# cita-cloud/consensus_overlord

Hardware: AMD Instinct MI355X
Metric: BLS12-381 vote verifications/sec (batch 4096) at 1/2/4/8 MI355X vs host blst (higher is better)
Workload: dtype u32; 1 GPU; config3: 4096 distinct-message precommit votes per GPU, RLC batch verify; batch_per_gpu=4096, global_batch=4096, parallelism=single GPU

## Files before the change

### consensus_overlord_amd/csrc/bls/fp.hpp

```cpp
#pragma once
#include <stdint.h>

#if defined(__HIPCC__)
#include <hip/hip_runtime.h>
#define OVH_HD __host__ __device__ __forceinline__
#define OVH_HDNI __host__ __device__ inline __attribute__((noinline))
#else
#define OVH_HD inline
#define OVH_HDNI inline
#endif

#include "consts.hpp"
#if defined(__HIP_DEVICE_COMPILE__)
#include "fp_mul_gfx950.hpp"
#include "fp_mul28.hpp"
#include "fp_mul28_gfx950.hpp"
#endif

namespace ovh {

#if defined(OVH_COUNT_MULS) && !defined(__HIP_DEVICE_COMPILE__)
extern unsigned long long g_fp_mul_count;
#define OVH_COUNT_MUL() (++::ovh::g_fp_mul_count)
#else
// ... 39 lines not shown
  for (int i = 0; i < 12; ++i) r.v[i] = 0;
}

OVH_HD void fp_one(Fp& r) { fp_load(r, ONE_M); }

OVH_HD bool fp_is_zero(const Fp& a) {
  uint32_t acc = 0;
#pragma unroll
  for (int i = 0; i < 12; ++i) acc |= a.v[i];
  return acc == 0;
}

OVH_HD bool fp_eq(const Fp& a, const Fp& b) {
  uint32_t acc = 0;
#pragma unroll
  for (int i = 0; i < 12; ++i) acc |= a.v[i] ^ b.v[i];
  return acc == 0;
}

OVH_HD bool fp_is_one(const Fp& a) { return fp_eq(a, fp_const(ONE_M)); }

OVH_HD void fp_select(Fp& r, bool cond, const Fp& a, const Fp& b) {
#pragma unroll
  for (int i = 0; i < 12; ++i) r.v[i] = cond ? b.v[i] : a.v[i];
}

OVH_HD void fp_add(Fp& r, const Fp& a, const Fp& b) {
  uint32_t s[12], d[12], c = 0, br = 0;
#pragma unroll
  for (int i = 0; i < 12; ++i) s[i] = addc32(a.v[i], b.v[i], c, &c);
#pragma unroll
  for (int i = 0; i < 12; ++i) d[i] = subc32(s[i], P_LIMBS[i], br, &br);
#pragma unroll
  for (int i = 0; i < 12; ++i) r.v[i] = br ? s[i] : d[i];
}

OVH_HD void fp_sub(Fp& r, const Fp& a, const Fp& b) {
  uint32_t d[12], br = 0, c = 0;
#pragma unroll
  for (int i = 0; i < 12; ++i) d[i] = subc32(a.v[i], b.v[i], br, &br);
  const uint32_t mask = 0u - br;
#pragma unroll
  for (int i = 0; i < 12; ++i) r.v[i] = addc32(d[i], P_LIMBS[i] & mask, c, &c);
}

OVH_HD void fp_dbl(Fp& r, const Fp& a) { fp_add(r, a, a); }

OVH_HD void fp_neg(Fp& r, const Fp& a) {
  Fp z;
  fp_zero(z);
  fp_sub(r, z, a);
}

OVH_HD void fp_mul(Fp& r, const Fp& a, const Fp& b) {
#if defined(__HIP_DEVICE_COMPILE__) && defined(OVH_FPMUL32)
  fp_mul_gfx950(r.v, a.v, b.v);
#elif defined(__HIP_DEVICE_COMPILE__)
  fp_mul28_gfx950(r.v, a.v, b.v);
#else
  OVH_COUNT_MUL();
  uint32_t t[12];
#pragma unroll
  for (int j = 0; j < 12; ++j) t[j] = 0;
#pragma unroll
  for (int i = 0; i < 12; ++i) {
    const uint32_t bi = b.v[i];
    uint64_t c = (uint64_t)a.v[0] * bi + t[0];
    t[0] = (uint32_t)c;
    const uint32_t m = t[0] * P_INV32;
    uint64_t c2 = (uint64_t)m * P_LIMBS[0] + t[0];
#pragma unroll
    for (int j = 1; j < 12; ++j) {
      c = (uint64_t)a.v[j] * bi + t[j] + (c >> 32);
      c2 = (uint64_t)m * P_LIMBS[j] + (uint32_t)c + (c2 >> 32);
      t[j - 1] = (uint32_t)c2;
    }
    t[11] = (uint32_t)(c >> 32) + (uint32_t)(c2 >> 32);
  }
  uint32_t d[12], br = 0;
#pragma unroll
  for (int i = 0; i < 12; ++i) d[i] = subc32(t[i], P_LIMBS[i], br, &br);
#pragma unroll
  for (int i = 0; i < 12; ++i) r.v[i] = br ? t[i] : d[i];
#endif
}

OVH_HD void fp_sqr(Fp& r, const Fp& a) { fp_mul(r, a, a); }

OVH_HD void fp_mul_small(Fp& r, const Fp& a, uint32_t k) {
  Fp acc, base = a;
  fp_zero(acc);
  while (k) {
    if (k & 1) fp_add(acc, acc, base);
    fp_add(base, base, base);
    k >>= 1;
  }
  r = acc;
}

OVH_HDNI void fp_pow(Fp& r, const Fp& a, const uint32_t* e) {
  Fp acc;
  fp_one(acc);
  bool started = false;
#pragma unroll 1
  for (int i = 11; i >= 0; --i) {
    const uint32_t w = e[i];
#pragma unroll 1
    for (int b = 31; b >= 0; --b) {
      if (started) fp_sqr(acc, acc);
      if ((w >> b) & 1) {
        if (started) {
          fp_mul(acc, acc, a);
        } else {
          acc = a;
          started = true;
        }
      }
    }
  }
  r = acc;
}

namespace inv {
constexpr int NL = 13;
constexpr int32_t M30 = 0x3FFFFFFF;
constexpr int32_t PL[NL] = {0x3fffaaab, 0x27fbffff, 0x153ffffb, 0x2affffac, 0x30f6241e, 0x034a83da, 0x112bf673,
                            0x12e13ce1, 0x2cd76477, 0x1ed90d2e, 0x29a4b1ba, 0x3a8e5ff9, 0x001a0111};
constexpr uint32_t PINV30 = 0x30003;
struct Trans {
  int32_t u, v, q, r;
};

OVH_HD int ctz32(uint32_t x) { return __builtin_ctz(x); }

OVH_HD uint32_t neg_inv32(uint32_t f) {
  uint32_t x = f;
  x *= 2u - f * x;
  x *= 2u - f * x;
  x *= 2u - f * x;
  x *= 2u - f * x;
  return 0u - x;
}

OVH_HD int32_t divsteps30(int32_t eta, uint32_t f, uint32_t g, Trans& t) {
  uint32_t u = 1, v = 0, q = 0, r = 1, finv = neg_inv32(f);
  int i = 30;
#pragma unroll 1
  for (;;) {
    const int z = ctz32(g | (0xFFFFFFFFu << i));
    g >>= z;
    u <<= z;
    v <<= z;
    eta -= z;
    i -= z;
    if (i == 0) break;
    if (eta < 0) {
      eta = -eta;
      uint32_t x = f;
      f = g;
      g = 0u - x;
      x = u;
      u = q;
      q = 0u - x;
      x = v;
      v = r;
      r = 0u - x;
// ... 208 lines not shown
```

### consensus_overlord_amd/csrc/bls/fp_mul28.hpp

```cpp
#pragma once
#include <stdint.h>

#include "consts.hpp"

namespace ovh {

constexpr uint32_t M28 = 0x0FFFFFFFu;
constexpr uint32_t P28[14] = {0xfffaaabu, 0xfefffffu, 0x3ffffb9u, 0xfffeb15u, 0x6241eabu, 0xa0f6b0fu, 0xf6730d2u,
                              0xf38512bu, 0x4774b84u, 0x4bacd76u, 0xba7b643u, 0xe69a4b1u, 0x1ea397fu, 0x001a011u};
constexpr uint32_t PINV28 = 0xffcfffdu;

template <int SH>
__device__ __forceinline__ void split28(uint32_t* x, const uint32_t* a) {
#if defined(OVH_UBENCH_NOSPLIT)
#pragma unroll
  for (int k = 0; k < 14; ++k) x[k] = a[k % 12];
  return;
#endif
#pragma unroll
  for (int k = 0; k < 14; ++k) {
    const int lo = 28 * k - SH;
    uint32_t v;
    if (lo < 0) {
      v = a[0] << (-lo);
    } else {
      const int w = lo >> 5, s = lo & 31;
      v = a[w] >> s;
      if (s > 4 && w + 1 < 12) v |= a[w + 1] << (32 - s);
    }
    x[k] = v & M28;
  }
}

__device__ __forceinline__ void join28_reduce(uint32_t* r, const uint32_t* t) {
#if defined(OVH_UBENCH_NOSPLIT)
#pragma unroll
  for (int j = 0; j < 12; ++j) r[j] = t[j];
  return;
#endif
  uint32_t u[12];
#pragma unroll
  for (int j = 0; j < 12; ++j) {
    const int k = (32 * j) / 28, s = (32 * j) % 28;
    uint32_t v = (t[k] >> s) | (t[k + 1] << (28 - s));
    if (s > 24 && k + 2 < 14) v |= t[k + 2] << (56 - s);
    u[j] = v;
  }
  uint32_t d[12], br = 0;
#pragma unroll
  for (int j = 0; j < 12; ++j) d[j] = __builtin_subc(u[j], P_LIMBS[j], br, &br);
#pragma unroll
  for (int j = 0; j < 12; ++j) r[j] = br ? u[j] : d[j];
}

__device__ __forceinline__ void fp_mul28(uint32_t* r, const uint32_t* a, const uint32_t* b) {
  uint32_t x[14], y[14], m[14], t[14];
  split28<8>(x, a);
  split28<0>(y, b);
  uint64_t acc = 0;
#pragma unroll
  for (int k = 0; k < 27; ++k) {
#pragma unroll
    for (int i = 0; i < 14; ++i)
      if (k - i >= 0 && k - i < 14) acc += (uint64_t)x[i] * y[k - i];
#pragma unroll
    for (int i = 0; i < 14; ++i)
      if (i < k && k - i < 14) acc += (uint64_t)m[i] * P28[k - i];
    if (k < 14) {
      m[k] = ((uint32_t)acc * PINV28) & M28;
      acc += (uint64_t)m[k] * P28[0];
    } else {
      t[k - 14] = (uint32_t)acc & M28;
    }
    acc >>= 28;
  }
  t[13] = (uint32_t)acc;
  join28_reduce(r, t);
}

}
```

### consensus_overlord_amd/csrc/bls/fp_mul28_gfx950.hpp

```cpp
#pragma once
#include <stdint.h>
#include "fp_mul28.hpp"
namespace ovh {
__device__ __forceinline__ void fp_mul28_gfx950_1acc(uint32_t* __restrict__ r, const uint32_t* __restrict__ a,
                                             const uint32_t* __restrict__ b) {
  uint32_t x[14], y[14], m[14], t[14];
  split28<8>(x, a);
  split28<0>(y, b);
  asm volatile(
      "v_mad_u64_u32 v[252:253], vcc, %[x0], %[y0], 0\n\tv_mul_lo_u32 %[m0], v252, %[pinv]\n\tv_and_b32_e32 %[m0], %[mask], %[m0]\n\tv_mad_u64_u32 v[252:253], vcc, %[m0], %[p0], v[252:253]\n\tv_lshrrev_b64 v[252:253], 28, v[252:253]\n\tv_mad_u64_u32 v[252:253], vcc, %[x0], %[y1], v[252:253]\n\tv_mad_u64_u32 v[252:253], vcc, %[x1], %[y0], v[252:253]\n\tv_mad_u64_u32 v[252:253], vcc, %[m0], %[p1], v[252:253]\n\t"
      "v_mul_lo_u32 %[m1], v252, %[pinv]\n\tv_and_b32_e32 %[m1], %[mask], %[m1]\n\tv_mad_u64_u32 v[252:253], vcc, %[m1], %[p0], v[252:253]\n\tv_lshrrev_b64 v[252:253], 28, v[252:253]\n\tv_mad_u64_u32 v[252:253], vcc, %[x0], %[y2], v[252:253]\n\tv_mad_u64_u32 v[252:253], vcc, %[x1], %[y1], v[252:253]\n\tv_mad_u64_u32 v[252:253], vcc, %[x2], %[y0], v[252:253]\n\tv_mad_u64_u32 v[252:253], vcc, %[m0], %[p2], v[252:253]\n\t"
      "v_mad_u64_u32 v[252:253], vcc, %[m1], %[p1], v[252:253]\n\tv_mul_lo_u32 %[m2], v252, %[pinv]\n\tv_and_b32_e32 %[m2], %[mask], %[m2]\n\tv_mad_u64_u32 v[252:253], vcc, %[m2], %[p0], v[252:253]\n\tv_lshrrev_b64 v[252:253], 28, v[252:253]\n\tv_mad_u64_u32 v[252:253], vcc, %[x0], %[y3], v[252:253]\n\tv_mad_u64_u32 v[252:253], vcc, %[x1], %[y2], v[252:253]\n\tv_mad_u64_u32 v[252:253], vcc, %[x2], %[y1], v[252:253]\n\t"
      "v_mad_u64_u32 v[252:253], vcc, %[x3], %[y0], v[252:253]\n\tv_mad_u64_u32 v[252:253], vcc, %[m0], %[p3], v[252:253]\n\tv_mad_u64_u32 v[252:253], vcc, %[m1], %[p2], v[252:253]\n\tv_mad_u64_u32 v[252:253], vcc, %[m2], %[p1], v[252:253]\n\tv_mul_lo_u32 %[m3], v252, %[pinv]\n\tv_and_b32_e32 %[m3], %[mask], %[m3]\n\tv_mad_u64_u32 v[252:253], vcc, %[m3], %[p0], v[252:253]\n\tv_lshrrev_b64 v[252:253], 28, v[252:253]\n\t"
      "v_mad_u64_u32 v[252:253], vcc, %[x0], %[y4], v[252:253]\n\tv_mad_u64_u32 v[252:253], vcc, %[x1], %[y3], v[252:253]\n\tv_mad_u64_u32 v[252:253], vcc, %[x2], %[y2], v[252:253]\n\tv_mad_u64_u32 v[252:253], vcc, %[x3], %[y1], v[252:253]\n\tv_mad_u64_u32 v[252:253], vcc, %[x4], %[y0], v[252:253]\n\tv_mad_u64_u32 v[252:253], vcc, %[m0], %[p4], v[252:253]\n\tv_mad_u64_u32 v[252:253], vcc, %[m1], %[p3], v[252:253]\n\tv_mad_u64_u32 v[252:253], vcc, %[m2], %[p2], v[252:253]\n\t"
      "v_mad_u64_u32 v[252:253], vcc, %[m3], %[p1], v[252:253]\n\tv_mul_lo_u32 %[m4], v252, %[pinv]\n\tv_and_b32_e32 %[m4], %[mask], %[m4]\n\tv_mad_u64_u32 v[252:253], vcc, %[m4], %[p0], v[252:253]\n\tv_lshrrev_b64 v[252:253], 28, v[252:253]\n\tv_mad_u64_u32 v[252:253], vcc, %[x0], %[y5], v[252:253]\n\tv_mad_u64_u32 v[252:253], vcc, %[x1], %[y4], v[252:253]\n\tv_mad_u64_u32 v[252:253], vcc, %[x2], %[y3], v[252:253]\n\t"
      "v_mad_u64_u32 v[252:253], vcc, %[x3], %[y2], v[252:253]\n\tv_mad_u64_u32 v[252:253], vcc, %[x4], %[y1], v[252:253]\n\tv_mad_u64_u32 v[252:253], vcc, %[x5], %[y0], v[252:253]\n\tv_mad_u64_u32 v[252:253], vcc, %[m0], %[p5], v[252:253]\n\tv_mad_u64_u32 v[252:253], vcc, %[m1], %[p4], v[252:253]\n\tv_mad_u64_u32 v[252:253], vcc, %[m2], %[p3], v[252:253]\n\tv_mad_u64_u32 v[252:253], vcc, %[m3], %[p2], v[252:253]\n\tv_mad_u64_u32 v[252:253], vcc, %[m4], %[p1], v[252:253]\n\t"
      "v_mul_lo_u32 %[m5], v252, %[pinv]\n\tv_and_b32_e32 %[m5], %[mask], %[m5]\n\tv_mad_u64_u32 v[252:253], vcc, %[m5], %[p0], v[252:253]\n\tv_lshrrev_b64 v[252:253], 28, v[252:253]\n\tv_mad_u64_u32 v[252:253], vcc, %[x0], %[y6], v[252:253]\n\tv_mad_u64_u32 v[252:253], vcc, %[x1], %[y5], v[252:253]\n\tv_mad_u64_u32 v[252:253], vcc, %[x2], %[y4], v[252:253]\n\tv_mad_u64_u32 v[252:253], vcc, %[x3], %[y3], v[252:253]\n\t"
      "v_mad_u64_u32 v[252:253], vcc, %[x4], %[y2], v[252:253]\n\tv_mad_u64_u32 v[252:253], vcc, %[x5], %[y1], v[252:253]\n\tv_mad_u64_u32 v[252:253], vcc, %[x6], %[y0], v[252:253]\n\tv_mad_u64_u32 v[252:253], vcc, %[m0], %[p6], v[252:253]\n\tv_mad_u64_u32 v[252:253], vcc, %[m1], %[p5], v[252:253]\n\tv_mad_u64_u32 v[252:253], vcc, %[m2], %[p4], v[252:253]\n\tv_mad_u64_u32 v[252:253], vcc, %[m3], %[p3], v[252:253]\n\tv_mad_u64_u32 v[252:253], vcc, %[m4], %[p2], v[252:253]\n\t"
      "v_mad_u64_u32 v[252:253], vcc, %[m5], %[p1], v[252:253]\n\tv_mul_lo_u32 %[m6], v252, %[pinv]\n\tv_and_b32_e32 %[m6], %[mask], %[m6]\n\tv_mad_u64_u32 v[252:253], vcc, %[m6], %[p0], v[252:253]\n\tv_lshrrev_b64 v[252:253], 28, v[252:253]\n\tv_mad_u64_u32 v[252:253], vcc, %[x0], %[y7], v[252:253]\n\tv_mad_u64_u32 v[252:253], vcc, %[x1], %[y6], v[252:253]\n\tv_mad_u64_u32 v[252:253], vcc, %[x2], %[y5], v[252:253]\n\t"
      "v_mad_u64_u32 v[252:253], vcc, %[x3], %[y4], v[252:253]\n\tv_mad_u64_u32 v[252:253], vcc, %[x4], %[y3], v[252:253]\n\tv_mad_u64_u32 v[252:253], vcc, %[x5], %[y2], v[252:253]\n\tv_mad_u64_u32 v[252:253], vcc, %[x6], %[y1], v[252:253]\n\tv_mad_u64_u32 v[252:253], vcc, %[x7], %[y0], v[252:253]\n\tv_mad_u64_u32 v[252:253], vcc, %[m0], %[p7], v[252:253]\n\tv_mad_u64_u32 v[252:253], vcc, %[m1], %[p6], v[252:253]\n\tv_mad_u64_u32 v[252:253], vcc, %[m2], %[p5], v[252:253]\n\t"
      "v_mad_u64_u32 v[252:253], vcc, %[m3], %[p4], v[252:253]\n\tv_mad_u64_u32 v[252:253], vcc, %[m4], %[p3], v[252:253]\n\tv_mad_u64_u32 v[252:253], vcc, %[m5], %[p2], v[252:253]\n\tv_mad_u64_u32 v[252:253], vcc, %[m6], %[p1], v[252:253]\n\tv_mul_lo_u32 %[m7], v252, %[pinv]\n\tv_and_b32_e32 %[m7], %[mask], %[m7]\n\tv_mad_u64_u32 v[252:253], vcc, %[m7], %[p0], v[252:253]\n\tv_lshrrev_b64 v[252:253], 28, v[252:253]\n\t"
      "v_mad_u64_u32 v[252:253], vcc, %[x0], %[y8], v[252:253]\n\tv_mad_u64_u32 v[252:253], vcc, %[x1], %[y7], v[252:253]\n\tv_mad_u64_u32 v[252:253], vcc, %[x2], %[y6], v[252:253]\n\tv_mad_u64_u32 v[252:253], vcc, %[x3], %[y5], v[252:253]\n\tv_mad_u64_u32 v[252:253], vcc, %[x4], %[y4], v[252:253]\n\tv_mad_u64_u32 v[252:253], vcc, %[x5], %[y3], v[252:253]\n\tv_mad_u64_u32 v[252:253], vcc, %[x6], %[y2], v[252:253]\n\tv_mad_u64_u32 v[252:253], vcc, %[x7], %[y1], v[252:253]\n\t"
      "v_mad_u64_u32 v[252:253], vcc, %[x8], %[y0], v[252:253]\n\tv_mad_u64_u32 v[252:253], vcc, %[m0], %[p8], v[252:253]\n\tv_mad_u64_u32 v[252:253], vcc, %[m1], %[p7], v[252:253]\n\tv_mad_u64_u32 v[252:253], vcc, %[m2], %[p6], v[252:253]\n\tv_mad_u64_u32 v[252:253], vcc, %[m3], %[p5], v[252:253]\n\tv_mad_u64_u32 v[252:253], vcc, %[m4], %[p4], v[252:253]\n\tv_mad_u64_u32 v[252:253], vcc, %[m5], %[p3], v[252:253]\n\tv_mad_u64_u32 v[252:253], vcc, %[m6], %[p2], v[252:253]\n\t"
      "v_mad_u64_u32 v[252:253], vcc, %[m7], %[p1], v[252:253]\n\tv_mul_lo_u32 %[m8], v252, %[pinv]\n\tv_and_b32_e32 %[m8], %[mask], %[m8]\n\tv_mad_u64_u32 v[252:253], vcc, %[m8], %[p0], v[252:253]\n\tv_lshrrev_b64 v[252:253], 28, v[252:253]\n\tv_mad_u64_u32 v[252:253], vcc, %[x0], %[y9], v[252:253]\n\tv_mad_u64_u32 v[252:253], vcc, %[x1], %[y8], v[252:253]\n\tv_mad_u64_u32 v[252:253], vcc, %[x2], %[y7], v[252:253]\n\t"
// ... 39 lines not shown
      "v_mad_u64_u32 v[252:253], vcc, %[x10], %[y13], v[252:253]\n\tv_mad_u64_u32 v[252:253], vcc, %[x11], %[y12], v[252:253]\n\tv_mad_u64_u32 v[252:253], vcc, %[x12], %[y11], v[252:253]\n\tv_mad_u64_u32 v[252:253], vcc, %[x13], %[y10], v[252:253]\n\tv_mad_u64_u32 v[252:253], vcc, %[m10], %[p13], v[252:253]\n\tv_mad_u64_u32 v[252:253], vcc, %[m11], %[p12], v[252:253]\n\tv_mad_u64_u32 v[252:253], vcc, %[m12], %[p11], v[252:253]\n\tv_mad_u64_u32 v[252:253], vcc, %[m13], %[p10], v[252:253]\n\t"
      "v_and_b32_e32 %[t9], %[mask], v252\n\tv_lshrrev_b64 v[252:253], 28, v[252:253]\n\tv_mad_u64_u32 v[252:253], vcc, %[x11], %[y13], v[252:253]\n\tv_mad_u64_u32 v[252:253], vcc, %[x12], %[y12], v[252:253]\n\tv_mad_u64_u32 v[252:253], vcc, %[x13], %[y11], v[252:253]\n\tv_mad_u64_u32 v[252:253], vcc, %[m11], %[p13], v[252:253]\n\tv_mad_u64_u32 v[252:253], vcc, %[m12], %[p12], v[252:253]\n\tv_mad_u64_u32 v[252:253], vcc, %[m13], %[p11], v[252:253]\n\t"
      "v_and_b32_e32 %[t10], %[mask], v252\n\tv_lshrrev_b64 v[252:253], 28, v[252:253]\n\tv_mad_u64_u32 v[252:253], vcc, %[x12], %[y13], v[252:253]\n\tv_mad_u64_u32 v[252:253], vcc, %[x13], %[y12], v[252:253]\n\tv_mad_u64_u32 v[252:253], vcc, %[m12], %[p13], v[252:253]\n\tv_mad_u64_u32 v[252:253], vcc, %[m13], %[p12], v[252:253]\n\tv_and_b32_e32 %[t11], %[mask], v252\n\tv_lshrrev_b64 v[252:253], 28, v[252:253]\n\t"
      "v_mad_u64_u32 v[252:253], vcc, %[x13], %[y13], v[252:253]\n\tv_mad_u64_u32 v[252:253], vcc, %[m13], %[p13], v[252:253]\n\tv_and_b32_e32 %[t12], %[mask], v252\n\tv_lshrrev_b64 v[252:253], 28, v[252:253]\n\tv_mov_b32 %[t13], v252\n\t"
      : [m0] "=&v"(m[0]), [m1] "=&v"(m[1]), [m2] "=&v"(m[2]), [m3] "=&v"(m[3]), [m4] "=&v"(m[4]), [m5] "=&v"(m[5]), [m6] "=&v"(m[6]), [m7] "=&v"(m[7]), [m8] "=&v"(m[8]), [m9] "=&v"(m[9]), [m10] "=&v"(m[10]), [m11] "=&v"(m[11]), [m12] "=&v"(m[12]), [m13] "=&v"(m[13]), [t0] "=&v"(t[0]), [t1] "=&v"(t[1]), [t2] "=&v"(t[2]), [t3] "=&v"(t[3]), [t4] "=&v"(t[4]), [t5] "=&v"(t[5]), [t6] "=&v"(t[6]), [t7] "=&v"(t[7]), [t8] "=&v"(t[8]), [t9] "=&v"(t[9]), [t10] "=&v"(t[10]), [t11] "=&v"(t[11]), [t12] "=&v"(t[12]), [t13] "=&v"(t[13])
      : [x0] "v"(x[0]), [x1] "v"(x[1]), [x2] "v"(x[2]), [x3] "v"(x[3]), [x4] "v"(x[4]), [x5] "v"(x[5]), [x6] "v"(x[6]), [x7] "v"(x[7]), [x8] "v"(x[8]), [x9] "v"(x[9]), [x10] "v"(x[10]), [x11] "v"(x[11]), [x12] "v"(x[12]), [x13] "v"(x[13]), [y0] "v"(y[0]), [y1] "v"(y[1]), [y2] "v"(y[2]), [y3] "v"(y[3]), [y4] "v"(y[4]), [y5] "v"(y[5]), [y6] "v"(y[6]), [y7] "v"(y[7]), [y8] "v"(y[8]), [y9] "v"(y[9]), [y10] "v"(y[10]), [y11] "v"(y[11]), [y12] "v"(y[12]), [y13] "v"(y[13]), [p0] "s"(P28[0]), [p1] "s"(P28[1]), [p2] "s"(P28[2]), [p3] "s"(P28[3]), [p4] "s"(P28[4]), [p5] "s"(P28[5]), [p6] "s"(P28[6]), [p7] "s"(P28[7]), [p8] "s"(P28[8]), [p9] "s"(P28[9]), [p10] "s"(P28[10]), [p11] "s"(P28[11]), [p12] "s"(P28[12]), [p13] "s"(P28[13]), [pinv] "s"(PINV28), [mask] "v"(M28)
      : "vcc", "v252", "v253");
  (void)m;
  join28_reduce(r, t);
}
__device__ __forceinline__ void fp_mul28_gfx950_2acc(uint32_t* __restrict__ r, const uint32_t* __restrict__ a,
                                             const uint32_t* __restrict__ b) {
  uint32_t x[14], y[14], m[14], t[14];
  split28<8>(x, a);
  split28<0>(y, b);
  asm volatile(
      "v_mad_u64_u32 v[252:253], vcc, %[x0], %[y0], 0\n\tv_mul_lo_u32 %[m0], v252, %[pinv]\n\tv_mad_u64_u32 v[250:251], vcc, %[x0], %[y1], 0\n\tv_and_b32_e32 %[m0], %[mask], %[m0]\n\tv_mad_u64_u32 v[250:251], vcc, %[x1], %[y0], v[250:251]\n\tv_mad_u64_u32 v[252:253], vcc, %[m0], %[p0], v[252:253]\n\tv_lshrrev_b64 v[252:253], 28, v[252:253]\n\tv_mad_u64_u32 v[252:253], vcc, %[m0], %[p1], v[252:253]\n\t"
      "v_lshl_add_u64 v[252:253], v[250:251], 0, v[252:253]\n\tv_mul_lo_u32 %[m1], v252, %[pinv]\n\tv_mad_u64_u32 v[250:251], vcc, %[x0], %[y2], 0\n\tv_and_b32_e32 %[m1], %[mask], %[m1]\n\tv_mad_u64_u32 v[250:251], vcc, %[x1], %[y1], v[250:251]\n\tv_mad_u64_u32 v[252:253], vcc, %[m1], %[p0], v[252:253]\n\tv_mad_u64_u32 v[250:251], vcc, %[x2], %[y0], v[250:251]\n\tv_lshrrev_b64 v[252:253], 28, v[252:253]\n\t"
      "v_mad_u64_u32 v[250:251], vcc, %[m0], %[p2], v[250:251]\n\tv_mad_u64_u32 v[252:253], vcc, %[m1], %[p1], v[252:253]\n\tv_lshl_add_u64 v[252:253], v[250:251], 0, v[252:253]\n\tv_mul_lo_u32 %[m2], v252, %[pinv]\n\tv_mad_u64_u32 v[250:251], vcc, %[x0], %[y3], 0\n\tv_and_b32_e32 %[m2], %[mask], %[m2]\n\tv_mad_u64_u32 v[250:251], vcc, %[x1], %[y2], v[250:251]\n\tv_mad_u64_u32 v[252:253], vcc, %[m2], %[p0], v[252:253]\n\t"
      "v_mad_u64_u32 v[250:251], vcc, %[x2], %[y1], v[250:251]\n\tv_lshrrev_b64 v[252:253], 28, v[252:253]\n\tv_mad_u64_u32 v[250:251], vcc, %[x3], %[y0], v[250:251]\n\tv_mad_u64_u32 v[252:253], vcc, %[m0], %[p3], v[252:253]\n\tv_mad_u64_u32 v[250:251], vcc, %[m1], %[p2], v[250:251]\n\tv_mad_u64_u32 v[252:253], vcc, %[m2], %[p1], v[252:253]\n\tv_lshl_add_u64 v[252:253], v[250:251], 0, v[252:253]\n\tv_mul_lo_u32 %[m3], v252, %[pinv]\n\t"
      "v_mad_u64_u32 v[250:251], vcc, %[x0], %[y4], 0\n\tv_and_b32_e32 %[m3], %[mask], %[m3]\n\tv_mad_u64_u32 v[250:251], vcc, %[x1], %[y3], v[250:251]\n\tv_mad_u64_u32 v[252:253], vcc, %[m3], %[p0], v[252:253]\n\tv_mad_u64_u32 v[250:251], vcc, %[x2], %[y2], v[250:251]\n\tv_lshrrev_b64 v[252:253], 28, v[252:253]\n\tv_mad_u64_u32 v[250:251], vcc, %[x3], %[y1], v[250:251]\n\tv_mad_u64_u32 v[252:253], vcc, %[x4], %[y0], v[252:253]\n\t"
      "v_mad_u64_u32 v[250:251], vcc, %[m0], %[p4], v[250:251]\n\tv_mad_u64_u32 v[252:253], vcc, %[m1], %[p3], v[252:253]\n\tv_mad_u64_u32 v[250:251], vcc, %[m2], %[p2], v[250:251]\n\tv_mad_u64_u32 v[252:253], vcc, %[m3], %[p1], v[252:253]\n\tv_lshl_add_u64 v[252:253], v[250:251], 0, v[252:253]\n\tv_mul_lo_u32 %[m4], v252, %[pinv]\n\tv_mad_u64_u32 v[250:251], vcc, %[x0], %[y5], 0\n\tv_and_b32_e32 %[m4], %[mask], %[m4]\n\t"
      "v_mad_u64_u32 v[250:251], vcc, %[x1], %[y4], v[250:251]\n\tv_mad_u64_u32 v[252:253], vcc, %[m4], %[p0], v[252:253]\n\tv_mad_u64_u32 v[250:251], vcc, %[x2], %[y3], v[250:251]\n\tv_lshrrev_b64 v[252:253], 28, v[252:253]\n\tv_mad_u64_u32 v[250:251], vcc, %[x3], %[y2], v[250:251]\n\tv_mad_u64_u32 v[252:253], vcc, %[x4], %[y1], v[252:253]\n\tv_mad_u64_u32 v[250:251], vcc, %[x5], %[y0], v[250:251]\n\tv_mad_u64_u32 v[252:253], vcc, %[m0], %[p5], v[252:253]\n\t"
      "v_mad_u64_u32 v[250:251], vcc, %[m1], %[p4], v[250:251]\n\tv_mad_u64_u32 v[252:253], vcc, %[m2], %[p3], v[252:253]\n\tv_mad_u64_u32 v[250:251], vcc, %[m3], %[p2], v[250:251]\n\tv_mad_u64_u32 v[252:253], vcc, %[m4], %[p1], v[252:253]\n\tv_lshl_add_u64 v[252:253], v[250:251], 0, v[252:253]\n\tv_mul_lo_u32 %[m5], v252, %[pinv]\n\tv_mad_u64_u32 v[250:251], vcc, %[x0], %[y6], 0\n\tv_and_b32_e32 %[m5], %[mask], %[m5]\n\t"
      "v_mad_u64_u32 v[250:251], vcc, %[x1], %[y5], v[250:251]\n\tv_mad_u64_u32 v[252:253], vcc, %[m5], %[p0], v[252:253]\n\tv_mad_u64_u32 v[250:251], vcc, %[x2], %[y4], v[250:251]\n\tv_lshrrev_b64 v[252:253], 28, v[252:253]\n\tv_mad_u64_u32 v[250:251], vcc, %[x3], %[y3], v[250:251]\n\tv_mad_u64_u32 v[252:253], vcc, %[x4], %[y2], v[252:253]\n\tv_mad_u64_u32 v[250:251], vcc, %[x5], %[y1], v[250:251]\n\tv_mad_u64_u32 v[252:253], vcc, %[x6], %[y0], v[252:253]\n\t"
      "v_mad_u64_u32 v[250:251], vcc, %[m0], %[p6], v[250:251]\n\tv_mad_u64_u32 v[252:253], vcc, %[m1], %[p5], v[252:253]\n\tv_mad_u64_u32 v[250:251], vcc, %[m2], %[p4], v[250:251]\n\tv_mad_u64_u32 v[252:253], vcc, %[m3], %[p3], v[252:253]\n\tv_mad_u64_u32 v[250:251], vcc, %[m4], %[p2], v[250:251]\n\tv_mad_u64_u32 v[252:253], vcc, %[m5], %[p1], v[252:253]\n\tv_lshl_add_u64 v[252:253], v[250:251], 0, v[252:253]\n\tv_mul_lo_u32 %[m6], v252, %[pinv]\n\t"
      "v_mad_u64_u32 v[250:251], vcc, %[x0], %[y7], 0\n\tv_and_b32_e32 %[m6], %[mask], %[m6]\n\tv_mad_u64_u32 v[250:251], vcc, %[x1], %[y6], v[250:251]\n\tv_mad_u64_u32 v[252:253], vcc, %[m6], %[p0], v[252:253]\n\tv_mad_u64_u32 v[250:251], vcc, %[x2], %[y5], v[250:251]\n\tv_lshrrev_b64 v[252:253], 28, v[252:253]\n\tv_mad_u64_u32 v[250:251], vcc, %[x3], %[y4], v[250:251]\n\tv_mad_u64_u32 v[252:253], vcc, %[x4], %[y3], v[252:253]\n\t"
      "v_mad_u64_u32 v[250:251], vcc, %[x5], %[y2], v[250:251]\n\tv_mad_u64_u32 v[252:253], vcc, %[x6], %[y1], v[252:253]\n\tv_mad_u64_u32 v[250:251], vcc, %[x7], %[y0], v[250:251]\n\tv_mad_u64_u32 v[252:253], vcc, %[m0], %[p7], v[252:253]\n\tv_mad_u64_u32 v[250:251], vcc, %[m1], %[p6], v[250:251]\n\tv_mad_u64_u32 v[252:253], vcc, %[m2], %[p5], v[252:253]\n\tv_mad_u64_u32 v[250:251], vcc, %[m3], %[p4], v[250:251]\n\tv_mad_u64_u32 v[252:253], vcc, %[m4], %[p3], v[252:253]\n\t"
      "v_mad_u64_u32 v[250:251], vcc, %[m5], %[p2], v[250:251]\n\tv_mad_u64_u32 v[252:253], vcc, %[m6], %[p1], v[252:253]\n\tv_lshl_add_u64 v[252:253], v[250:251], 0, v[252:253]\n\tv_mul_lo_u32 %[m7], v252, %[pinv]\n\tv_mad_u64_u32 v[250:251], vcc, %[x0], %[y8], 0\n\tv_and_b32_e32 %[m7], %[mask], %[m7]\n\tv_mad_u64_u32 v[250:251], vcc, %[x1], %[y7], v[250:251]\n\tv_mad_u64_u32 v[252:253], vcc, %[m7], %[p0], v[252:253]\n\t"
      "v_mad_u64_u32 v[250:251], vcc, %[x2], %[y6], v[250:251]\n\tv_lshrrev_b64 v[252:253], 28, v[252:253]\n\tv_mad_u64_u32 v[250:251], vcc, %[x3], %[y5], v[250:251]\n\tv_mad_u64_u32 v[252:253], vcc, %[x4], %[y4], v[252:253]\n\tv_mad_u64_u32 v[250:251], vcc, %[x5], %[y3], v[250:251]\n\tv_mad_u64_u32 v[252:253], vcc, %[x6], %[y2], v[252:253]\n\tv_mad_u64_u32 v[250:251], vcc, %[x7], %[y1], v[250:251]\n\tv_mad_u64_u32 v[252:253], vcc, %[x8], %[y0], v[252:253]\n\t"
      "v_mad_u64_u32 v[250:251], vcc, %[m0], %[p8], v[250:251]\n\tv_mad_u64_u32 v[252:253], vcc, %[m1], %[p7], v[252:253]\n\tv_mad_u64_u32 v[250:251], vcc, %[m2], %[p6], v[250:251]\n\tv_mad_u64_u32 v[252:253], vcc, %[m3], %[p5], v[252:253]\n\tv_mad_u64_u32 v[250:251], vcc, %[m4], %[p4], v[250:251]\n\tv_mad_u64_u32 v[252:253], vcc, %[m5], %[p3], v[252:253]\n\tv_mad_u64_u32 v[250:251], vcc, %[m6], %[p2], v[250:251]\n\tv_mad_u64_u32 v[252:253], vcc, %[m7], %[p1], v[252:253]\n\t"
      "v_lshl_add_u64 v[252:253], v[250:251], 0, v[252:253]\n\tv_mul_lo_u32 %[m8], v252, %[pinv]\n\tv_mad_u64_u32 v[250:251], vcc, %[x0], %[y9], 0\n\tv_and_b32_e32 %[m8], %[mask], %[m8]\n\tv_mad_u64_u32 v[250:251], vcc, %[x1], %[y8], v[250:251]\n\tv_mad_u64_u32 v[252:253], vcc, %[m8], %[p0], v[252:253]\n\tv_mad_u64_u32 v[250:251], vcc, %[x2], %[y7], v[250:251]\n\tv_lshrrev_b64 v[252:253], 28, v[252:253]\n\t"
      "v_mad_u64_u32 v[250:251], vcc, %[x3], %[y6], v[250:251]\n\tv_mad_u64_u32 v[252:253], vcc, %[x4], %[y5], v[252:253]\n\tv_mad_u64_u32 v[250:251], vcc, %[x5], %[y4], v[250:251]\n\tv_mad_u64_u32 v[252:253], vcc, %[x6], %[y3], v[252:253]\n\tv_mad_u64_u32 v[250:251], vcc, %[x7], %[y2], v[250:251]\n\tv_mad_u64_u32 v[252:253], vcc, %[x8], %[y1], v[252:253]\n\tv_mad_u64_u32 v[250:251], vcc, %[x9], %[y0], v[250:251]\n\tv_mad_u64_u32 v[252:253], vcc, %[m0], %[p9], v[252:253]\n\t"
      "v_mad_u64_u32 v[250:251], vcc, %[m1], %[p8], v[250:251]\n\tv_mad_u64_u32 v[252:253], vcc, %[m2], %[p7], v[252:253]\n\tv_mad_u64_u32 v[250:251], vcc, %[m3], %[p6], v[250:251]\n\tv_mad_u64_u32 v[252:253], vcc, %[m4], %[p5], v[252:253]\n\tv_mad_u64_u32 v[250:251], vcc, %[m5], %[p4], v[250:251]\n\tv_mad_u64_u32 v[252:253], vcc, %[m6], %[p3], v[252:253]\n\tv_mad_u64_u32 v[250:251], vcc, %[m7], %[p2], v[250:251]\n\tv_mad_u64_u32 v[252:253], vcc, %[m8], %[p1], v[252:253]\n\t"
      "v_lshl_add_u64 v[252:253], v[250:251], 0, v[252:253]\n\tv_mul_lo_u32 %[m9], v252, %[pinv]\n\tv_mad_u64_u32 v[250:251], vcc, %[x0], %[y10], 0\n\tv_and_b32_e32 %[m9], %[mask], %[m9]\n\tv_mad_u64_u32 v[250:251], vcc, %[x1], %[y9], v[250:251]\n\tv_mad_u64_u32 v[252:253], vcc, %[m9], %[p0], v[252:253]\n\tv_mad_u64_u32 v[250:251], vcc, %[x2], %[y8], v[250:251]\n\tv_lshrrev_b64 v[252:253], 28, v[252:253]\n\t"
      "v_mad_u64_u32 v[250:251], vcc, %[x3], %[y7], v[250:251]\n\tv_mad_u64_u32 v[252:253], vcc, %[x4], %[y6], v[252:253]\n\tv_mad_u64_u32 v[250:251], vcc, %[x5], %[y5], v[250:251]\n\tv_mad_u64_u32 v[252:253], vcc, %[x6], %[y4], v[252:253]\n\tv_mad_u64_u32 v[250:251], vcc, %[x7], %[y3], v[250:251]\n\tv_mad_u64_u32 v[252:253], vcc, %[x8], %[y2], v[252:253]\n\tv_mad_u64_u32 v[250:251], vcc, %[x9], %[y1], v[250:251]\n\tv_mad_u64_u32 v[252:253], vcc, %[x10], %[y0], v[252:253]\n\t"
      "v_mad_u64_u32 v[250:251], vcc, %[m0], %[p10], v[250:251]\n\tv_mad_u64_u32 v[252:253], vcc, %[m1], %[p9], v[252:253]\n\tv_mad_u64_u32 v[250:251], vcc, %[m2], %[p8], v[250:251]\n\tv_mad_u64_u32 v[252:253], vcc, %[m3], %[p7], v[252:253]\n\tv_mad_u64_u32 v[250:251], vcc, %[m4], %[p6], v[250:251]\n\tv_mad_u64_u32 v[252:253], vcc, %[m5], %[p5], v[252:253]\n\tv_mad_u64_u32 v[250:251], vcc, %[m6], %[p4], v[250:251]\n\tv_mad_u64_u32 v[252:253], vcc, %[m7], %[p3], v[252:253]\n\t"
      "v_mad_u64_u32 v[250:251], vcc, %[m8], %[p2], v[250:251]\n\tv_mad_u64_u32 v[252:253], vcc, %[m9], %[p1], v[252:253]\n\tv_lshl_add_u64 v[252:253], v[250:251], 0, v[252:253]\n\tv_mul_lo_u32 %[m10], v252, %[pinv]\n\tv_mad_u64_u32 v[250:251], vcc, %[x0], %[y11], 0\n\tv_and_b32_e32 %[m10], %[mask], %[m10]\n\tv_mad_u64_u32 v[250:251], vcc, %[x1], %[y10], v[250:251]\n\tv_mad_u64_u32 v[252:253], vcc, %[m10], %[p0], v[252:253]\n\t"
      "v_mad_u64_u32 v[250:251], vcc, %[x2], %[y9], v[250:251]\n\tv_lshrrev_b64 v[252:253], 28, v[252:253]\n\tv_mad_u64_u32 v[250:251], vcc, %[x3], %[y8], v[250:251]\n\tv_mad_u64_u32 v[252:253], vcc, %[x4], %[y7], v[252:253]\n\tv_mad_u64_u32 v[250:251], vcc, %[x5], %[y6], v[250:251]\n\tv_mad_u64_u32 v[252:253], vcc, %[x6], %[y5], v[252:253]\n\tv_mad_u64_u32 v[250:251], vcc, %[x7], %[y4], v[250:251]\n\tv_mad_u64_u32 v[252:253], vcc, %[x8], %[y3], v[252:253]\n\t"
      "v_mad_u64_u32 v[250:251], vcc, %[x9], %[y2], v[250:251]\n\tv_mad_u64_u32 v[252:253], vcc, %[x10], %[y1], v[252:253]\n\tv_mad_u64_u32 v[250:251], vcc, %[x11], %[y0], v[250:251]\n\tv_mad_u64_u32 v[252:253], vcc, %[m0], %[p11], v[252:253]\n\tv_mad_u64_u32 v[250:251], vcc, %[m1], %[p10], v[250:251]\n\tv_mad_u64_u32 v[252:253], vcc, %[m2], %[p9], v[252:253]\n\tv_mad_u64_u32 v[250:251], vcc, %[m3], %[p8], v[250:251]\n\tv_mad_u64_u32 v[252:253], vcc, %[m4], %[p7], v[252:253]\n\t"
      "v_mad_u64_u32 v[250:251], vcc, %[m5], %[p6], v[250:251]\n\tv_mad_u64_u32 v[252:253], vcc, %[m6], %[p5], v[252:253]\n\tv_mad_u64_u32 v[250:251], vcc, %[m7], %[p4], v[250:251]\n\tv_mad_u64_u32 v[252:253], vcc, %[m8], %[p3], v[252:253]\n\tv_mad_u64_u32 v[250:251], vcc, %[m9], %[p2], v[250:251]\n\tv_mad_u64_u32 v[252:253], vcc, %[m10], %[p1], v[252:253]\n\tv_lshl_add_u64 v[252:253], v[250:251], 0, v[252:253]\n\tv_mul_lo_u32 %[m11], v252, %[pinv]\n\t"
      "v_mad_u64_u32 v[250:251], vcc, %[x0], %[y12], 0\n\tv_and_b32_e32 %[m11], %[mask], %[m11]\n\tv_mad_u64_u32 v[250:251], vcc, %[x1], %[y11], v[250:251]\n\tv_mad_u64_u32 v[252:253], vcc, %[m11], %[p0], v[252:253]\n\tv_mad_u64_u32 v[250:251], vcc, %[x2], %[y10], v[250:251]\n\tv_lshrrev_b64 v[252:253], 28, v[252:253]\n\tv_mad_u64_u32 v[250:251], vcc, %[x3], %[y9], v[250:251]\n\tv_mad_u64_u32 v[252:253], vcc, %[x4], %[y8], v[252:253]\n\t"
      "v_mad_u64_u32 v[250:251], vcc, %[x5], %[y7], v[250:251]\n\tv_mad_u64_u32 v[252:253], vcc, %[x6], %[y6], v[252:253]\n\tv_mad_u64_u32 v[250:251], vcc, %[x7], %[y5], v[250:251]\n\tv_mad_u64_u32 v[252:253], vcc, %[x8], %[y4], v[252:253]\n\tv_mad_u64_u32 v[250:251], vcc, %[x9], %[y3], v[250:251]\n\tv_mad_u64_u32 v[252:253], vcc, %[x10], %[y2], v[252:253]\n\tv_mad_u64_u32 v[250:251], vcc, %[x11], %[y1], v[250:251]\n\tv_mad_u64_u32 v[252:253], vcc, %[x12], %[y0], v[252:253]\n\t"
      "v_mad_u64_u32 v[250:251], vcc, %[m0], %[p12], v[250:251]\n\tv_mad_u64_u32 v[252:253], vcc, %[m1], %[p11], v[252:253]\n\tv_mad_u64_u32 v[250:251], vcc, %[m2], %[p10], v[250:251]\n\tv_mad_u64_u32 v[252:253], vcc, %[m3], %[p9], v[252:253]\n\tv_mad_u64_u32 v[250:251], vcc, %[m4], %[p8], v[250:251]\n\tv_mad_u64_u32 v[252:253], vcc, %[m5], %[p7], v[252:253]\n\tv_mad_u64_u32 v[250:251], vcc, %[m6], %[p6], v[250:251]\n\tv_mad_u64_u32 v[252:253], vcc, %[m7], %[p5], v[252:253]\n\t"
      "v_mad_u64_u32 v[250:251], vcc, %[m8], %[p4], v[250:251]\n\tv_mad_u64_u32 v[252:253], vcc, %[m9], %[p3], v[252:253]\n\tv_mad_u64_u32 v[250:251], vcc, %[m10], %[p2], v[250:251]\n\tv_mad_u64_u32 v[252:253], vcc, %[m11], %[p1], v[252:253]\n\tv_lshl_add_u64 v[252:253], v[250:251], 0, v[252:253]\n\tv_mul_lo_u32 %[m12], v252, %[pinv]\n\tv_mad_u64_u32 v[250:251], vcc, %[x0], %[y13], 0\n\tv_and_b32_e32 %[m12], %[mask], %[m12]\n\t"
      "v_mad_u64_u32 v[250:251], vcc, %[x1], %[y12], v[250:251]\n\tv_mad_u64_u32 v[252:253], vcc, %[m12], %[p0], v[252:253]\n\tv_mad_u64_u32 v[250:251], vcc, %[x2], %[y11], v[250:251]\n\tv_lshrrev_b64 v[252:253], 28, v[252:253]\n\tv_mad_u64_u32 v[250:251], vcc, %[x3], %[y10], v[250:251]\n\tv_mad_u64_u32 v[252:253], vcc, %[x4], %[y9], v[252:253]\n\tv_mad_u64_u32 v[250:251], vcc, %[x5], %[y8], v[250:251]\n\tv_mad_u64_u32 v[252:253], vcc, %[x6], %[y7], v[252:253]\n\t"
      "v_mad_u64_u32 v[250:251], vcc, %[x7], %[y6], v[250:251]\n\tv_mad_u64_u32 v[252:253], vcc, %[x8], %[y5], v[252:253]\n\tv_mad_u64_u32 v[250:251], vcc, %[x9], %[y4], v[250:251]\n\tv_mad_u64_u32 v[252:253], vcc, %[x10], %[y3], v[252:253]\n\tv_mad_u64_u32 v[250:251], vcc, %[x11], %[y2], v[250:251]\n\tv_mad_u64_u32 v[252:253], vcc, %[x12], %[y1], v[252:253]\n\tv_mad_u64_u32 v[250:251], vcc, %[x13], %[y0], v[250:251]\n\tv_mad_u64_u32 v[252:253], vcc, %[m0], %[p13], v[252:253]\n\t"
      "v_mad_u64_u32 v[250:251], vcc, %[m1], %[p12], v[250:251]\n\tv_mad_u64_u32 v[252:253], vcc, %[m2], %[p11], v[252:253]\n\tv_mad_u64_u32 v[250:251], vcc, %[m3], %[p10], v[250:251]\n\tv_mad_u64_u32 v[252:253], vcc, %[m4], %[p9], v[252:253]\n\tv_mad_u64_u32 v[250:251], vcc, %[m5], %[p8], v[250:251]\n\tv_mad_u64_u32 v[252:253], vcc, %[m6], %[p7], v[252:253]\n\tv_mad_u64_u32 v[250:251], vcc, %[m7], %[p6], v[250:251]\n\tv_mad_u64_u32 v[252:253], vcc, %[m8], %[p5], v[252:253]\n\t"
      "v_mad_u64_u32 v[250:251], vcc, %[m9], %[p4], v[250:251]\n\tv_mad_u64_u32 v[252:253], vcc, %[m10], %[p3], v[252:253]\n\tv_mad_u64_u32 v[250:251], vcc, %[m11], %[p2], v[250:251]\n\tv_mad_u64_u32 v[252:253], vcc, %[m12], %[p1], v[252:253]\n\tv_lshl_add_u64 v[252:253], v[250:251], 0, v[252:253]\n\tv_mul_lo_u32 %[m13], v252, %[pinv]\n\tv_mad_u64_u32 v[250:251], vcc, %[x1], %[y13], 0\n\tv_and_b32_e32 %[m13], %[mask], %[m13]\n\t"
      "v_mad_u64_u32 v[250:251], vcc, %[x2], %[y12], v[250:251]\n\tv_mad_u64_u32 v[252:253], vcc, %[m13], %[p0], v[252:253]\n\tv_mad_u64_u32 v[250:251], vcc, %[x3], %[y11], v[250:251]\n\tv_lshrrev_b64 v[252:253], 28, v[252:253]\n\tv_mad_u64_u32 v[250:251], vcc, %[x4], %[y10], v[250:251]\n\tv_mad_u64_u32 v[252:253], vcc, %[x5], %[y9], v[252:253]\n\tv_mad_u64_u32 v[250:251], vcc, %[x6], %[y8], v[250:251]\n\tv_mad_u64_u32 v[252:253], vcc, %[x7], %[y7], v[252:253]\n\t"
      "v_mad_u64_u32 v[250:251], vcc, %[x8], %[y6], v[250:251]\n\tv_mad_u64_u32 v[252:253], vcc, %[x9], %[y5], v[252:253]\n\tv_mad_u64_u32 v[250:251], vcc, %[x10], %[y4], v[250:251]\n\tv_mad_u64_u32 v[252:253], vcc, %[x11], %[y3], v[252:253]\n\tv_mad_u64_u32 v[250:251], vcc, %[x12], %[y2], v[250:251]\n\tv_mad_u64_u32 v[252:253], vcc, %[x13], %[y1], v[252:253]\n\tv_mad_u64_u32 v[250:251], vcc, %[m1], %[p13], v[250:251]\n\tv_mad_u64_u32 v[252:253], vcc, %[m2], %[p12], v[252:253]\n\t"
      "v_mad_u64_u32 v[250:251], vcc, %[m3], %[p11], v[250:251]\n\tv_mad_u64_u32 v[252:253], vcc, %[m4], %[p10], v[252:253]\n\tv_mad_u64_u32 v[250:251], vcc, %[m5], %[p9], v[250:251]\n\tv_mad_u64_u32 v[252:253], vcc, %[m6], %[p8], v[252:253]\n\tv_mad_u64_u32 v[250:251], vcc, %[m7], %[p7], v[250:251]\n\tv_mad_u64_u32 v[252:253], vcc, %[m8], %[p6], v[252:253]\n\tv_mad_u64_u32 v[250:251], vcc, %[m9], %[p5], v[250:251]\n\tv_mad_u64_u32 v[252:253], vcc, %[m10], %[p4], v[252:253]\n\t"
      "v_mad_u64_u32 v[250:251], vcc, %[m11], %[p3], v[250:251]\n\tv_mad_u64_u32 v[252:253], vcc, %[m12], %[p2], v[252:253]\n\tv_mad_u64_u32 v[250:251], vcc, %[m13], %[p1], v[250:251]\n\tv_lshl_add_u64 v[252:253], v[250:251], 0, v[252:253]\n\tv_and_b32_e32 %[t0], %[mask], v252\n\tv_mad_u64_u32 v[250:251], vcc, %[x2], %[y13], 0\n\tv_lshrrev_b64 v[252:253], 28, v[252:253]\n\tv_mad_u64_u32 v[250:251], vcc, %[x3], %[y12], v[250:251]\n\t"
      "v_mad_u64_u32 v[252:253], vcc, %[x4], %[y11], v[252:253]\n\tv_mad_u64_u32 v[250:251], vcc, %[x5], %[y10], v[250:251]\n\tv_mad_u64_u32 v[252:253], vcc, %[x6], %[y9], v[252:253]\n\tv_mad_u64_u32 v[250:251], vcc, %[x7], %[y8], v[250:251]\n\tv_mad_u64_u32 v[252:253], vcc, %[x8], %[y7], v[252:253]\n\tv_mad_u64_u32 v[250:251], vcc, %[x9], %[y6], v[250:251]\n\tv_mad_u64_u32 v[252:253], vcc, %[x10], %[y5], v[252:253]\n\tv_mad_u64_u32 v[250:251], vcc, %[x11], %[y4], v[250:251]\n\t"
      "v_mad_u64_u32 v[252:253], vcc, %[x12], %[y3], v[252:253]\n\tv_mad_u64_u32 v[250:251], vcc, %[x13], %[y2], v[250:251]\n\tv_mad_u64_u32 v[252:253], vcc, %[m2], %[p13], v[252:253]\n\tv_mad_u64_u32 v[250:251], vcc, %[m3], %[p12], v[250:251]\n\tv_mad_u64_u32 v[252:253], vcc, %[m4], %[p11], v[252:253]\n\tv_mad_u64_u32 v[250:251], vcc, %[m5], %[p10], v[250:251]\n\tv_mad_u64_u32 v[252:253], vcc, %[m6], %[p9], v[252:253]\n\tv_mad_u64_u32 v[250:251], vcc, %[m7], %[p8], v[250:251]\n\t"
      "v_mad_u64_u32 v[252:253], vcc, %[m8], %[p7], v[252:253]\n\tv_mad_u64_u32 v[250:251], vcc, %[m9], %[p6], v[250:251]\n\tv_mad_u64_u32 v[252:253], vcc, %[m10], %[p5], v[252:253]\n\tv_mad_u64_u32 v[250:251], vcc, %[m11], %[p4], v[250:251]\n\tv_mad_u64_u32 v[252:253], vcc, %[m12], %[p3], v[252:253]\n\tv_mad_u64_u32 v[250:251], vcc, %[m13], %[p2], v[250:251]\n\tv_lshl_add_u64 v[252:253], v[250:251], 0, v[252:253]\n\tv_and_b32_e32 %[t1], %[mask], v252\n\t"
      "v_mad_u64_u32 v[250:251], vcc, %[x3], %[y13], 0\n\tv_lshrrev_b64 v[252:253], 28, v[252:253]\n\tv_mad_u64_u32 v[250:251], vcc, %[x4], %[y12], v[250:251]\n\tv_mad_u64_u32 v[252:253], vcc, %[x5], %[y11], v[252:253]\n\tv_mad_u64_u32 v[250:251], vcc, %[x6], %[y10], v[250:251]\n\tv_mad_u64_u32 v[252:253], vcc, %[x7], %[y9], v[252:253]\n\tv_mad_u64_u32 v[250:251], vcc, %[x8], %[y8], v[250:251]\n\tv_mad_u64_u32 v[252:253], vcc, %[x9], %[y7], v[252:253]\n\t"
      "v_mad_u64_u32 v[250:251], vcc, %[x10], %[y6], v[250:251]\n\tv_mad_u64_u32 v[252:253], vcc, %[x11], %[y5], v[252:253]\n\tv_mad_u64_u32 v[250:251], vcc, %[x12], %[y4], v[250:251]\n\tv_mad_u64_u32 v[252:253], vcc, %[x13], %[y3], v[252:253]\n\tv_mad_u64_u32 v[250:251], vcc, %[m3], %[p13], v[250:251]\n\tv_mad_u64_u32 v[252:253], vcc, %[m4], %[p12], v[252:253]\n\tv_mad_u64_u32 v[250:251], vcc, %[m5], %[p11], v[250:251]\n\tv_mad_u64_u32 v[252:253], vcc, %[m6], %[p10], v[252:253]\n\t"
      "v_mad_u64_u32 v[250:251], vcc, %[m7], %[p9], v[250:251]\n\tv_mad_u64_u32 v[252:253], vcc, %[m8], %[p8], v[252:253]\n\tv_mad_u64_u32 v[250:251], vcc, %[m9], %[p7], v[250:251]\n\tv_mad_u64_u32 v[252:253], vcc, %[m10], %[p6], v[252:253]\n\tv_mad_u64_u32 v[250:251], vcc, %[m11], %[p5], v[250:251]\n\tv_mad_u64_u32 v[252:253], vcc, %[m12], %[p4], v[252:253]\n\tv_mad_u64_u32 v[250:251], vcc, %[m13], %[p3], v[250:251]\n\tv_lshl_add_u64 v[252:253], v[250:251], 0, v[252:253]\n\t"
      "v_and_b32_e32 %[t2], %[mask], v252\n\tv_mad_u64_u32 v[250:251], vcc, %[x4], %[y13], 0\n\tv_lshrrev_b64 v[252:253], 28, v[252:253]\n\tv_mad_u64_u32 v[250:251], vcc, %[x5], %[y12], v[250:251]\n\tv_mad_u64_u32 v[252:253], vcc, %[x6], %[y11], v[252:253]\n\tv_mad_u64_u32 v[250:251], vcc, %[x7], %[y10], v[250:251]\n\tv_mad_u64_u32 v[252:253], vcc, %[x8], %[y9], v[252:253]\n\tv_mad_u64_u32 v[250:251], vcc, %[x9], %[y8], v[250:251]\n\t"
      "v_mad_u64_u32 v[252:253], vcc, %[x10], %[y7], v[252:253]\n\tv_mad_u64_u32 v[250:251], vcc, %[x11], %[y6], v[250:251]\n\tv_mad_u64_u32 v[252:253], vcc, %[x12], %[y5], v[252:253]\n\tv_mad_u64_u32 v[250:251], vcc, %[x13], %[y4], v[250:251]\n\tv_mad_u64_u32 v[252:253], vcc, %[m4], %[p13], v[252:253]\n\tv_mad_u64_u32 v[250:251], vcc, %[m5], %[p12], v[250:251]\n\tv_mad_u64_u32 v[252:253], vcc, %[m6], %[p11], v[252:253]\n\tv_mad_u64_u32 v[250:251], vcc, %[m7], %[p10], v[250:251]\n\t"
      "v_mad_u64_u32 v[252:253], vcc, %[m8], %[p9], v[252:253]\n\tv_mad_u64_u32 v[250:251], vcc, %[m9], %[p8], v[250:251]\n\tv_mad_u64_u32 v[252:253], vcc, %[m10], %[p7], v[252:253]\n\tv_mad_u64_u32 v[250:251], vcc, %[m11], %[p6], v[250:251]\n\tv_mad_u64_u32 v[252:253], vcc, %[m12], %[p5], v[252:253]\n\tv_mad_u64_u32 v[250:251], vcc, %[m13], %[p4], v[250:251]\n\tv_lshl_add_u64 v[252:253], v[250:251], 0, v[252:253]\n\tv_and_b32_e32 %[t3], %[mask], v252\n\t"
      "v_mad_u64_u32 v[250:251], vcc, %[x5], %[y13], 0\n\tv_lshrrev_b64 v[252:253], 28, v[252:253]\n\tv_mad_u64_u32 v[250:251], vcc, %[x6], %[y12], v[250:251]\n\tv_mad_u64_u32 v[252:253], vcc, %[x7], %[y11], v[252:253]\n\tv_mad_u64_u32 v[250:251], vcc, %[x8], %[y10], v[250:251]\n\tv_mad_u64_u32 v[252:253], vcc, %[x9], %[y9], v[252:253]\n\tv_mad_u64_u32 v[250:251], vcc, %[x10], %[y8], v[250:251]\n\tv_mad_u64_u32 v[252:253], vcc, %[x11], %[y7], v[252:253]\n\t"
      "v_mad_u64_u32 v[250:251], vcc, %[x12], %[y6], v[250:251]\n\tv_mad_u64_u32 v[252:253], vcc, %[x13], %[y5], v[252:253]\n\tv_mad_u64_u32 v[250:251], vcc, %[m5], %[p13], v[250:251]\n\tv_mad_u64_u32 v[252:253], vcc, %[m6], %[p12], v[252:253]\n\tv_mad_u64_u32 v[250:251], vcc, %[m7], %[p11], v[250:251]\n\tv_mad_u64_u32 v[252:253], vcc, %[m8], %[p10], v[252:253]\n\tv_mad_u64_u32 v[250:251], vcc, %[m9], %[p9], v[250:251]\n\tv_mad_u64_u32 v[252:253], vcc, %[m10], %[p8], v[252:253]\n\t"
      "v_mad_u64_u32 v[250:251], vcc, %[m11], %[p7], v[250:251]\n\tv_mad_u64_u32 v[252:253], vcc, %[m12], %[p6], v[252:253]\n\tv_mad_u64_u32 v[250:251], vcc, %[m13], %[p5], v[250:251]\n\tv_lshl_add_u64 v[252:253], v[250:251], 0, v[252:253]\n\tv_and_b32_e32 %[t4], %[mask], v252\n\tv_mad_u64_u32 v[250:251], vcc, %[x6], %[y13], 0\n\tv_lshrrev_b64 v[252:253], 28, v[252:253]\n\tv_mad_u64_u32 v[250:251], vcc, %[x7], %[y12], v[250:251]\n\t"
      "v_mad_u64_u32 v[252:253], vcc, %[x8], %[y11], v[252:253]\n\tv_mad_u64_u32 v[250:251], vcc, %[x9], %[y10], v[250:251]\n\tv_mad_u64_u32 v[252:253], vcc, %[x10], %[y9], v[252:253]\n\tv_mad_u64_u32 v[250:251], vcc, %[x11], %[y8], v[250:251]\n\tv_mad_u64_u32 v[252:253], vcc, %[x12], %[y7], v[252:253]\n\tv_mad_u64_u32 v[250:251], vcc, %[x13], %[y6], v[250:251]\n\tv_mad_u64_u32 v[252:253], vcc, %[m6], %[p13], v[252:253]\n\tv_mad_u64_u32 v[250:251], vcc, %[m7], %[p12], v[250:251]\n\t"
      "v_mad_u64_u32 v[252:253], vcc, %[m8], %[p11], v[252:253]\n\tv_mad_u64_u32 v[250:251], vcc, %[m9], %[p10], v[250:251]\n\tv_mad_u64_u32 v[252:253], vcc, %[m10], %[p9], v[252:253]\n\tv_mad_u64_u32 v[250:251], vcc, %[m11], %[p8], v[250:251]\n\tv_mad_u64_u32 v[252:253], vcc, %[m12], %[p7], v[252:253]\n\tv_mad_u64_u32 v[250:251], vcc, %[m13], %[p6], v[250:251]\n\tv_lshl_add_u64 v[252:253], v[250:251], 0, v[252:253]\n\tv_and_b32_e32 %[t5], %[mask], v252\n\t"
      "v_mad_u64_u32 v[250:251], vcc, %[x7], %[y13], 0\n\tv_lshrrev_b64 v[252:253], 28, v[252:253]\n\tv_mad_u64_u32 v[250:251], vcc, %[x8], %[y12], v[250:251]\n\tv_mad_u64_u32 v[252:253], vcc, %[x9], %[y11], v[252:253]\n\tv_mad_u64_u32 v[250:251], vcc, %[x10], %[y10], v[250:251]\n\tv_mad_u64_u32 v[252:253], vcc, %[x11], %[y9], v[252:253]\n\tv_mad_u64_u32 v[250:251], vcc, %[x12], %[y8], v[250:251]\n\tv_mad_u64_u32 v[252:253], vcc, %[x13], %[y7], v[252:253]\n\t"
      "v_mad_u64_u32 v[250:251], vcc, %[m7], %[p13], v[250:251]\n\tv_mad_u64_u32 v[252:253], vcc, %[m8], %[p12], v[252:253]\n\tv_mad_u64_u32 v[250:251], vcc, %[m9], %[p11], v[250:251]\n\tv_mad_u64_u32 v[252:253], vcc, %[m10], %[p10], v[252:253]\n\tv_mad_u64_u32 v[250:251], vcc, %[m11], %[p9], v[250:251]\n\tv_mad_u64_u32 v[252:253], vcc, %[m12], %[p8], v[252:253]\n\tv_mad_u64_u32 v[250:251], vcc, %[m13], %[p7], v[250:251]\n\tv_lshl_add_u64 v[252:253], v[250:251], 0, v[252:253]\n\t"
      "v_and_b32_e32 %[t6], %[mask], v252\n\tv_mad_u64_u32 v[250:251], vcc, %[x8], %[y13], 0\n\tv_lshrrev_b64 v[252:253], 28, v[252:253]\n\tv_mad_u64_u32 v[250:251], vcc, %[x9], %[y12], v[250:251]\n\tv_mad_u64_u32 v[252:253], vcc, %[x10], %[y11], v[252:253]\n\tv_mad_u64_u32 v[250:251], vcc, %[x11], %[y10], v[250:251]\n\tv_mad_u64_u32 v[252:253], vcc, %[x12], %[y9], v[252:253]\n\tv_mad_u64_u32 v[250:251], vcc, %[x13], %[y8], v[250:251]\n\t"
      "v_mad_u64_u32 v[252:253], vcc, %[m8], %[p13], v[252:253]\n\tv_mad_u64_u32 v[250:251], vcc, %[m9], %[p12], v[250:251]\n\tv_mad_u64_u32 v[252:253], vcc, %[m10], %[p11], v[252:253]\n\tv_mad_u64_u32 v[250:251], vcc, %[m11], %[p10], v[250:251]\n\tv_mad_u64_u32 v[252:253], vcc, %[m12], %[p9], v[252:253]\n\tv_mad_u64_u32 v[250:251], vcc, %[m13], %[p8], v[250:251]\n\tv_lshl_add_u64 v[252:253], v[250:251], 0, v[252:253]\n\tv_and_b32_e32 %[t7], %[mask], v252\n\t"
      "v_mad_u64_u32 v[250:251], vcc, %[x9], %[y13], 0\n\tv_lshrrev_b64 v[252:253], 28, v[252:253]\n\tv_mad_u64_u32 v[250:251], vcc, %[x10], %[y12], v[250:251]\n\tv_mad_u64_u32 v[252:253], vcc, %[x11], %[y11], v[252:253]\n\tv_mad_u64_u32 v[250:251], vcc, %[x12], %[y10], v[250:251]\n\tv_mad_u64_u32 v[252:253], vcc, %[x13], %[y9], v[252:253]\n\tv_mad_u64_u32 v[250:251], vcc, %[m9], %[p13], v[250:251]\n\tv_mad_u64_u32 v[252:253], vcc, %[m10], %[p12], v[252:253]\n\t"
      "v_mad_u64_u32 v[250:251], vcc, %[m11], %[p11], v[250:251]\n\tv_mad_u64_u32 v[252:253], vcc, %[m12], %[p10], v[252:253]\n\tv_mad_u64_u32 v[250:251], vcc, %[m13], %[p9], v[250:251]\n\tv_lshl_add_u64 v[252:253], v[250:251], 0, v[252:253]\n\tv_and_b32_e32 %[t8], %[mask], v252\n\tv_mad_u64_u32 v[250:251], vcc, %[x10], %[y13], 0\n\tv_lshrrev_b64 v[252:253], 28, v[252:253]\n\tv_mad_u64_u32 v[250:251], vcc, %[x11], %[y12], v[250:251]\n\t"
      "v_mad_u64_u32 v[252:253], vcc, %[x12], %[y11], v[252:253]\n\tv_mad_u64_u32 v[250:251], vcc, %[x13], %[y10], v[250:251]\n\tv_mad_u64_u32 v[252:253], vcc, %[m10], %[p13], v[252:253]\n\tv_mad_u64_u32 v[250:251], vcc, %[m11], %[p12], v[250:251]\n\tv_mad_u64_u32 v[252:253], vcc, %[m12], %[p11], v[252:253]\n\tv_mad_u64_u32 v[250:251], vcc, %[m13], %[p10], v[250:251]\n\tv_lshl_add_u64 v[252:253], v[250:251], 0, v[252:253]\n\tv_and_b32_e32 %[t9], %[mask], v252\n\t"
      "v_mad_u64_u32 v[250:251], vcc, %[x11], %[y13], 0\n\tv_lshrrev_b64 v[252:253], 28, v[252:253]\n\tv_mad_u64_u32 v[250:251], vcc, %[x12], %[y12], v[250:251]\n\tv_mad_u64_u32 v[252:253], vcc, %[x13], %[y11], v[252:253]\n\tv_mad_u64_u32 v[250:251], vcc, %[m11], %[p13], v[250:251]\n\tv_mad_u64_u32 v[252:253], vcc, %[m12], %[p12], v[252:253]\n\tv_mad_u64_u32 v[250:251], vcc, %[m13], %[p11], v[250:251]\n\tv_lshl_add_u64 v[252:253], v[250:251], 0, v[252:253]\n\t"
      "v_and_b32_e32 %[t10], %[mask], v252\n\tv_mad_u64_u32 v[250:251], vcc, %[x12], %[y13], 0\n\tv_lshrrev_b64 v[252:253], 28, v[252:253]\n\tv_mad_u64_u32 v[250:251], vcc, %[x13], %[y12], v[250:251]\n\tv_mad_u64_u32 v[252:253], vcc, %[m12], %[p13], v[252:253]\n\tv_mad_u64_u32 v[250:251], vcc, %[m13], %[p12], v[250:251]\n\tv_lshl_add_u64 v[252:253], v[250:251], 0, v[252:253]\n\tv_and_b32_e32 %[t11], %[mask], v252\n\t"
      "v_mad_u64_u32 v[250:251], vcc, %[x13], %[y13], 0\n\tv_lshrrev_b64 v[252:253], 28, v[252:253]\n\tv_mad_u64_u32 v[250:251], vcc, %[m13], %[p13], v[250:251]\n\tv_lshl_add_u64 v[252:253], v[250:251], 0, v[252:253]\n\tv_and_b32_e32 %[t12], %[mask], v252\n\tv_lshrrev_b64 v[252:253], 28, v[252:253]\n\tv_mov_b32 %[t13], v252\n\t"
      : [m0] "=&v"(m[0]), [m1] "=&v"(m[1]), [m2] "=&v"(m[2]), [m3] "=&v"(m[3]), [m4] "=&v"(m[4]), [m5] "=&v"(m[5]), [m6] "=&v"(m[6]), [m7] "=&v"(m[7]), [m8] "=&v"(m[8]), [m9] "=&v"(m[9]), [m10] "=&v"(m[10]), [m11] "=&v"(m[11]), [m12] "=&v"(m[12]), [m13] "=&v"(m[13]), [t0] "=&v"(t[0]), [t1] "=&v"(t[1]), [t2] "=&v"(t[2]), [t3] "=&v"(t[3]), [t4] "=&v"(t[4]), [t5] "=&v"(t[5]), [t6] "=&v"(t[6]), [t7] "=&v"(t[7]), [t8] "=&v"(t[8]), [t9] "=&v"(t[9]), [t10] "=&v"(t[10]), [t11] "=&v"(t[11]), [t12] "=&v"(t[12]), [t13] "=&v"(t[13])
      : [x0] "v"(x[0]), [x1] "v"(x[1]), [x2] "v"(x[2]), [x3] "v"(x[3]), [x4] "v"(x[4]), [x5] "v"(x[5]), [x6] "v"(x[6]), [x7] "v"(x[7]), [x8] "v"(x[8]), [x9] "v"(x[9]), [x10] "v"(x[10]), [x11] "v"(x[11]), [x12] "v"(x[12]), [x13] "v"(x[13]), [y0] "v"(y[0]), [y1] "v"(y[1]), [y2] "v"(y[2]), [y3] "v"(y[3]), [y4] "v"(y[4]), [y5] "v"(y[5]), [y6] "v"(y[6]), [y7] "v"(y[7]), [y8] "v"(y[8]), [y9] "v"(y[9]), [y10] "v"(y[10]), [y11] "v"(y[11]), [y12] "v"(y[12]), [y13] "v"(y[13]), [p0] "s"(P28[0]), [p1] "s"(P28[1]), [p2] "s"(P28[2]), [p3] "s"(P28[3]), [p4] "s"(P28[4]), [p5] "s"(P28[5]), [p6] "s"(P28[6]), [p7] "s"(P28[7]), [p8] "s"(P28[8]), [p9] "s"(P28[9]), [p10] "s"(P28[10]), [p11] "s"(P28[11]), [p12] "s"(P28[12]), [p13] "s"(P28[13]), [pinv] "s"(PINV28), [mask] "v"(M28)
      : "vcc", "v250", "v251", "v252", "v253");
  (void)m;
  join28_reduce(r, t);
}
#if defined(OVH_FPMUL28_2ACC)
__device__ __forceinline__ void fp_mul28_gfx950(uint32_t* r, const uint32_t* a, const uint32_t* b) {
  fp_mul28_gfx950_2acc(r, a, b);
}
#else
__device__ __forceinline__ void fp_mul28_gfx950(uint32_t* r, const uint32_t* a, const uint32_t* b) {
  fp_mul28_gfx950_1acc(r, a, b);
}
#endif
}
```

### consensus_overlord_amd/csrc/fpvm.hpp

```cpp
#pragma once
#include "bls/fp.hpp"

#if defined(__HIPCC__)
#define VM_FN __device__ __forceinline__
#else
#define VM_FN inline
struct uint4 {
  uint32_t x, y, z, w;
};
inline uint4 make_uint4(uint32_t a, uint32_t b, uint32_t c, uint32_t d) { return uint4{a, b, c, d}; }
#endif

namespace ovh {
namespace vm {

enum : uint32_t {
  OP_NOP = 0, OP_MULS = 1, OP_SGN0 = 2, OP_LEX = 3, OP_INV = 4, OP_LIN = 5, OP_SEL = 6, OP_EQ = 7,
  OP_AND = 8, OP_OR = 9, OP_XOR = 10, OP_ST = 11, OP_SELB = 12,
};

constexpr uint32_t PREFETCH = 6;

struct Out {
  uint32_t* base;
// ... 105 lines not shown

VM_FN void canon(Fp& r, const Fp& a) {
  uint32_t d[12], br = 0;
#pragma unroll
  for (int j = 0; j < 12; ++j) d[j] = subc32(a.v[j], P_LIMBS[j], br, &br);
#pragma unroll
  for (int j = 0; j < 12; ++j) r.v[j] = br ? a.v[j] : d[j];
}

constexpr uint32_t NP_LIMBS[12] = {
    0u - P_LIMBS[0], ~P_LIMBS[1], ~P_LIMBS[2], ~P_LIMBS[3], ~P_LIMBS[4], ~P_LIMBS[5],
    ~P_LIMBS[6], ~P_LIMBS[7], ~P_LIMBS[8], ~P_LIMBS[9], ~P_LIMBS[10], ~P_LIMBS[11]};
static_assert(P_LIMBS[0] != 0, "NP_LIMBS: no borrow out of limb 0");

VM_FN uint32_t quot_est(uint32_t t) {
  constexpr float QS = (float)((1.0 - 0x1p-20) / (double)((P_LIMBS[11] >> 7) + 1));
  return (uint32_t)((float)t * QS);
}

VM_FN void scale_reduce(Fp& r, const uint32_t* s, uint32_t k) {
  const uint32_t q = quot_est(k * (uint32_t)((((uint64_t)s[12] << 32) | s[11]) >> 7));
  uint64_t acc = 0;
#pragma unroll
  for (int j = 0; j < 12; ++j) {
    acc = (uint64_t)k * s[j] + (acc >> 32);
    acc = (uint64_t)q * NP_LIMBS[j] + acc;
    r.v[j] = (uint32_t)acc;
  }
}

constexpr uint32_t P2P1_LIMBS[12] = {
    P2_LIMBS[0] + 1, P2_LIMBS[1], P2_LIMBS[2], P2_LIMBS[3], P2_LIMBS[4], P2_LIMBS[5],
    P2_LIMBS[6], P2_LIMBS[7], P2_LIMBS[8], P2_LIMBS[9], P2_LIMBS[10], P2_LIMBS[11]};

VM_FN void lin_mad(Fp& r, const Fp& A, const Fp& B, const Fp& C, const Fp& D, int ca, int cb, int cc, int cd) {
  const Fp* X[4] = {&A, &B, &C, &D};
  const int cf[4] = {ca, cb, cc, cd};
  uint64_t acc[12];
#pragma unroll
  for (int j = 0; j < 12; ++j) acc[j] = 0;
  uint32_t nw = 0;
#pragma unroll
  for (int t = 0; t < 4; ++t) {
    const uint32_t a = cf[t] < 0 ? (uint32_t)(-cf[t]) : (uint32_t)cf[t];
    const uint32_t m = cf[t] < 0 ? ~0u : 0u;
    nw += a & m;
#pragma unroll
    for (int j = 0; j < 12; ++j) acc[j] = (uint64_t)a * (X[t]->v[j] ^ m) + acc[j];
  }
#pragma unroll
  for (int j = 0; j < 12; ++j) acc[j] = (uint64_t)nw * P2P1_LIMBS[j] + acc[j];
  const int64_t top = (int64_t)(acc[11] >> 7) - ((int64_t)nw << 25);
  const uint32_t q = top > 0 ? quot_est((uint32_t)top) : 0u;
  uint64_t cy = 0;
#pragma unroll
  for (int j = 0; j < 12; ++j) {
    const uint64_t v = (uint64_t)q * NP_LIMBS[j] + (acc[j] + cy);
    r.v[j] = (uint32_t)v;
    cy = v >> 32;
  }
}

VM_FN void pre_add2(Fp& x, const Fp& A, const Fp& B, Fp& y, const Fp& C, const Fp& D, bool ny, bool any_neg) {
  uint32_t c1 = 0, c2 = 0;
  if (any_neg) {
    uint32_t nd[12], b2 = 0;
#pragma unroll
    for (int j = 0; j < 13; ++j) {
      if (j < 12) {
        nd[j] = subc32(P2_LIMBS[j], D.v[j], b2, &b2);
        x.v[j] = addc32(A.v[j], B.v[j], c1, &c1);
      }
      if (j >= 1) y.v[j - 1] = addc32(C.v[j - 1], ny ? nd[j - 1] : D.v[j - 1], c2, &c2);
    }
  } else {
#pragma unroll
    for (int j = 0; j < 12; ++j) {
      x.v[j] = addc32(A.v[j], B.v[j], c1, &c1);
      y.v[j] = addc32(C.v[j], D.v[j], c2, &c2);
    }
  }
}

constexpr uint32_t H_MUL = 1u << 22, H_MULNEG = 1u << 23, H_FLAG = 1u << 24, H_LIN = 1u << 25,
                   H_LINNEG = 1u << 26, H_ACC = 1u << 27, H_RARE = 1u << 28, H_SELB = 1u << 29,
                   H_LINNEG2 = 1u << 30, H_LINNEG3 = 1u << 31;
constexpr uint32_t H_ANY = H_MUL | H_LIN | H_ACC | H_RARE;

template <bool XB, bool XC>
VM_FN void lin_chain_neg(uint32_t* s, const Fp& A, const Fp& B, const Fp& C, const Fp& D, uint32_t mb, uint32_t mc,
                         uint32_t md, const Fp& K) {
  uint32_t u[12], v[12], w[12], c1 = 0, c2 = 0, c3 = 0, c4 = 0;
#pragma unroll
  for (int j = 0; j < 14; ++j) {
    if (j < 12) {
      u[j] = addc32(A.v[j], XB ? B.v[j] ^ mb : B.v[j], c1, &c1);
      v[j] = addc32(XC ? C.v[j] ^ mc : C.v[j], D.v[j] ^ md, c2, &c2);
    }
    if (j >= 1 && j <= 12) w[j - 1] = addc32(u[j - 1], v[j - 1], c3, &c3);
    if (j >= 2) s[j - 2] = addc32(w[j - 2], K.v[j - 2], c4, &c4);
  }
}

VM_FN void lin_sum(uint32_t* s, const Fp& A, const Fp& B, const Fp& C, const Fp& D, uint32_t mb, uint32_t mc,
                   uint32_t md, uint32_t hdr, const uint32_t* __restrict__ cst) {
  if (hdr & H_LINNEG) {
    const uint32_t n = (mb & 1u) + (mc & 1u) + (md & 1u);
    Fp K;
    ld_slot(K, nullptr, cst, CONST_BASE + KTAB + n);
    if (hdr & H_LINNEG3) {
      lin_chain_neg<true, true>(s, A, B, C, D, mb, mc, md, K);
    } else if (hdr & H_LINNEG2) {
#if defined(__HIP_DEVICE_COMPILE__)
      __asm__ volatile("");
#endif
      lin_chain_neg<false, true>(s, A, B, C, D, mb, mc, md, K);
    } else {
#if defined(__HIP_DEVICE_COMPILE__)
      __asm__ volatile("");
#endif
      lin_chain_neg<false, false>(s, A, B, C, D, mb, mc, md, K);
    }
  } else {
    uint32_t u[12], v[12], c1 = 0, c2 = 0, c3 = 0;
#pragma unroll
    for (int j = 0; j < 13; ++j) {
      if (j < 12) {
        u[j] = addc32(A.v[j], B.v[j], c1, &c1);
        v[j] = addc32(C.v[j], D.v[j], c2, &c2);
      }
      if (j >= 1) s[j - 1] = addc32(u[j - 1], v[j - 1], c3, &c3);
    }
  }
  s[12] = 0;
}

VM_FN void fp_inv(Fp& r, const Fp& a, const Fp& r3) { fp_inv_divsteps(r, a, r3); }

#if defined(__HIPCC__)
VM_FN uint32_t uniform(uint32_t w0) { return __builtin_amdgcn_readfirstlane(w0); }
#else
inline uint32_t uniform(uint32_t w0) { return w0; }
#endif

VM_FN uint32_t sign_mask(uint32_t w, int bit) { return (uint32_t)((int32_t)(w << (31 - bit)) >> 31); }
VM_FN int coef5(uint32_t w, int lo) { return ((int)(w << (27 - lo))) >> 27; }

template <bool INV = true>
VM_FN void exec(const uint4 in, bool active, uint32_t* __restrict__ slots, const uint32_t* __restrict__ cst,
                uint64_t scalar, const Out& out) {
  const uint32_t hdr = uniform(in.x);
  if (!(hdr & H_ANY)) return;
  const uint32_t op = active ? (in.x & 31) : (uint32_t)OP_NOP;
  uint32_t ra = in.y & 0xFFFF, rb = in.y >> 16, rc = in.z & 0xFFFF;
  bool selb = false;
  if (hdr & H_SELB) {
#if defined(__HIP_DEVICE_COMPILE__)
    __asm__ volatile("");
#endif
    selb = op == OP_SELB;
    const bool bit = ((scalar >> ((in.x >> 16) & 63)) & 1) != 0;
    ra = selb ? (bit ? rc : rb) : ra;
    rb = selb ? CONST_BASE + KZERO : rb;
    rc = selb ? CONST_BASE + KZERO : rc;
  }
  Fp A, B, C, D;
  ld_slots4(A, B, C, D, slots, cst, ra, rb, rc, in.z >> 16);
  const uint32_t dst = (in.x >> 5) & 0x7FF;
  const bool force_acc = (in.w & (1u << 24)) != 0;
  if (hdr & H_MUL) {
    const bool is_mul = op == OP_MULS || op == OP_SGN0 || op == OP_LEX || op == OP_EQ;
    Fp x, y, m;
    pre_add2(x, A, B, y, C, D, sign_mask(in.w, 19) != 0, (hdr & H_MULNEG) != 0);
    fp_mul(m, x, y);
    if (hdr & H_FLAG) {
      const bool flag = is_mul && op != OP_MULS;
      uint32_t f = 0;
      if (op == OP_SGN0) f = m.v[0] & 1u;
      if (op == OP_LEX) f = limbs_gt(m.v, HALF_P) ? 1u : 0u;
      if (op == OP_EQ) f = fp_is_zero(m) ? 1u : 0u;
#pragma unroll
      for (int j = 0; j < 12; ++j) m.v[j] = flag ? (j == 0 ? f : 0u) : m.v[j];
    }
    if (is_mul) st_slot(slots, dst, m);
  }
  if (hdr & H_LIN) {
    uint32_t s[13];
    lin_sum(s, A, B, C, D, sign_mask(in.w, 9), sign_mask(in.w, 14), sign_mask(in.w, 19), hdr, cst);
    const uint32_t k = (in.w >> 20) & 15;
    Fp l;
    scale_reduce(l, s, k > 1 ? k : 1u);
    if ((op == OP_LIN && !force_acc) || selb) st_slot(slots, dst, l);
  }
  if (hdr & H_ACC) {
    Fp l;
    lin_mad(l, A, B, C, D, coef5(in.w, 0), coef5(in.w, 5), coef5(in.w, 10), coef5(in.w, 15));
    if (op == OP_LIN && force_acc) st_slot(slots, dst, l);
  }
  if (hdr & H_RARE) {
    const bool rare = op != OP_NOP && op != OP_LIN && !selb && op != OP_MULS && op != OP_SGN0 && op != OP_LEX &&
                      op != OP_EQ;
    const uint32_t imm = (in.x >> 16) & 63;
    Fp z = A;
    if (op == OP_ST) {
      canon(z, A);
      uint32_t* b = out.base + (size_t)imm * 12 * out.cap + out.unit;
#pragma unroll
      for (int k = 0; k < 12; ++k) b[(size_t)k * out.cap] = z.v[k];
    } else if (op == OP_SEL) {
      z = A.v[0] ? C : B;
    } else if (op >= OP_AND && op <= OP_XOR) {
      set_flag(z, op == OP_AND ? (A.v[0] & C.v[0]) : op == OP_OR ? (A.v[0] | C.v[0]) : (A.v[0] ^ C.v[0]));
    } else if (INV && op == OP_INV) {
      Fp a;
      canon(a, A);
      fp_inv(z, a, C);
    }
    if (rare && op != OP_ST) st_slot(slots, dst, z);
  }
#if defined(__HIP_DEVICE_COMPILE__)
  __asm__ volatile("" ::"v"(A.v[11]), "v"(B.v[11]), "v"(C.v[11]), "v"(D.v[11]));
#endif
}

#if defined(__HIPCC__)
constexpr uint32_t SIDE_VALID = 1u << 31, SIDE_FILL = 1u << 30;

__device__ __forceinline__ void side_spill(uint32_t sw, uint32_t* __restrict__ slots, uint32_t* __restrict__ scr) {
  if ((sw & (SIDE_VALID | SIDE_FILL)) == SIDE_VALID) {
    const u32x4* s = reinterpret_cast<const u32x4*>(slots + (sw & 0x7FF) * 12);
    const u32x4 a = s[0], b = s[1], c = s[2];
    u32x4* d = reinterpret_cast<u32x4*>(scr + ((sw >> 11) & 0xFFF) * 12);
    d[0] = a;
    d[1] = b;
    d[2] = c;
  }
}

#ifndef OVH_VM_UNROLL
#define OVH_VM_UNROLL 1
#endif

template <bool SIDE = false, bool INV = true, int UNROLL = OVH_VM_UNROLL>
__device__ __forceinline__ void run(const uint4* __restrict__ code, uint32_t nphases, uint32_t W, uint32_t lane,
                                    bool active, uint32_t* __restrict__ slots, const uint32_t* __restrict__ cst,
                                    uint64_t scalar, const Out& out, uint64_t* __restrict__ trace = nullptr,
                                    const uint32_t* __restrict__ side = nullptr, uint32_t* __restrict__ scr = nullptr) {
  static_assert(PREFETCH >= 5, "the unrolled loops below read up to 4 phases past the end");
  static_assert(UNROLL == 1 || UNROLL == 3, "loop shapes: 1 (rotated by moves) or 3 (unrolled over the rings)");
  if constexpr (SIDE) {
    uint4 qa = code[lane], qb, qc;
    uint32_t sa = side[lane], sb = side[W + lane], sc;
    if constexpr (UNROLL == 3) qb = code[W + lane];
    if (!active) sa = sb = 0;
    __builtin_amdgcn_s_waitcnt(0x0F70);
    auto step = [&](const uint4& q, uint4& q2, const uint32_t s, const uint32_t sn, uint32_t& s2,
                    const uint32_t ph) __attribute__((always_inline)) {
      constexpr uint32_t QD = UNROLL == 3 ? 2 : 1;
      const bool fill = (sn & (SIDE_VALID | SIDE_FILL)) == (SIDE_VALID | SIDE_FILL);
      u32x4 f0, f1, f2;
      if (fill) {
        const u32x4* src = reinterpret_cast<const u32x4*>(scr + ((sn >> 11) & 0xFFF) * 12);
        f0 = __builtin_nontemporal_load(src);
        f1 = __builtin_nontemporal_load(src + 1);
        f2 = __builtin_nontemporal_load(src + 2);
      }
      q2 = code[(size_t)(ph + QD) * W + lane];
      s2 = active ? side[(size_t)(ph + 2) * W + lane] : 0u;
      exec<INV>(q, active, slots, cst, scalar, out);
      side_spill(s, slots, scr);
      if (fill) {
        u32x4* d = reinterpret_cast<u32x4*>(slots + (sn & 0x7FF) * 12);
        d[0] = f0;
        d[1] = f1;
        d[2] = f2;
      }
    };
    if constexpr (UNROLL == 3) {
#pragma unroll 1
      for (uint32_t ph = 0; ph < nphases; ph += 3) {
        step(qa, qc, sa, sb, sc, ph);
        step(qb, qa, sb, sc, sa, ph + 1);
        step(qc, qb, sc, sa, sb, ph + 2);
      }
    } else {
#pragma unroll 1
      for (uint32_t ph = 0; ph < nphases; ++ph) {
        step(qa, qb, sa, sb, sc, ph);
        qa = qb;
        sa = sb;
        sb = sc;
      }
    }
    __asm__ volatile("s_waitcnt lgkmcnt(0)\n\ts_barrier" ::: "memory");
    return;
  }
  if (trace && threadIdx.x == 0) trace[0] = wall_clock64();
  uint4 qa = code[lane], qb, qc;
  if constexpr (UNROLL == 3) qb = code[W + lane];
  __builtin_amdgcn_s_waitcnt(0x0F70);
  auto step = [&](const uint4& q, uint4& q2, const uint32_t ph) __attribute__((always_inline)) {
    q2 = code[(size_t)(ph + (UNROLL == 3 ? 2 : 1)) * W + lane];
    exec<INV>(q, active, slots, cst, scalar, out);
    if (trace && ph < nphases) {
      __asm__ volatile("s_waitcnt lgkmcnt(0)" ::: "memory");
      if (threadIdx.x == 0) trace[ph + 1] = wall_clock64();
    }
  };
  if constexpr (UNROLL == 3) {
#pragma unroll 1
    for (uint32_t ph = 0; ph < nphases; ph += 3) {
      step(qa, qc, ph);
      step(qb, qa, ph + 1);
      step(qc, qb, ph + 2);
    }
  } else {
#pragma unroll 1
    for (uint32_t ph = 0; ph < nphases; ++ph) {
      step(qa, qb, ph);
      qa = qb;
    }
  }
  __asm__ volatile("s_waitcnt lgkmcnt(0)\n\ts_barrier" ::: "memory");
}

#endif

}
}
```

### consensus_overlord_amd/csrc/ovhip.hip

```cpp
#include <hip/hip_runtime.h>

#include <errno.h>
#include <stdlib.h>
#include <sys/random.h>
#include <sys/types.h>

#include <algorithm>
#include <atomic>
#include <deque>
#include <mutex>
#include <new>
#include <string>
#include <string.h>
#include <unordered_map>
#include <vector>

#include "../../include/ovhip.h"
#include "bls/verify.hpp"
#include "fpvm.hpp"
#include "keygen.hpp"
#include "proof.hpp"
#include "qc_round_groups.hpp"
#include "qc_segments.hpp"
#include "rlp.hpp"
#include "sm3.hpp"
#include "sm3_bulk.hpp"
#ifdef OVH_VM_PROGS
#include OVH_VM_PROGS
#else
#include <vm_progs.inc>
#endif
static_assert(VM_KZERO == ovh::vm::KZERO && VM_KTAB == ovh::vm::KTAB, "fixed constants (tools/fpvm/gen.py)");
#define VM_ASSERT_NO_INV(P) static_assert(!VM_##P##_HAS_INV, #P " has an inv op: it needs vm::run<SIDE, true>")
#define VM_ASSERT_INV(P) static_assert(VM_##P##_HAS_INV, #P " has no inv op: bind it to vm::run<SIDE, false>")
VM_ASSERT_NO_INV(MADD); VM_ASSERT_NO_INV(PADD); VM_ASSERT_NO_INV(G1PADD);
VM_ASSERT_NO_INV(HDBL1); VM_ASSERT_NO_INV(HDBL2); VM_ASSERT_NO_INV(HDBL4); VM_ASSERT_NO_INV(HDBL8); VM_ASSERT_NO_INV(HDBL16);
VM_ASSERT_NO_INV(VOTE1); VM_ASSERT_NO_INV(VOTE_T1); VM_ASSERT_NO_INV(VOTE1H); VM_ASSERT_NO_INV(VOTE_T1H);
VM_ASSERT_NO_INV(VOTEW); VM_ASSERT_NO_INV(VOTEW_T);
VM_ASSERT_NO_INV(VSAME); VM_ASSERT_NO_INV(VSAME_T); VM_ASSERT_NO_INV(VSAME8); VM_ASSERT_NO_INV(VSAME8_T);

using namespace ovh;

#define WG 64

#include "ovhip/common.hpp"

#include "ovhip/pool.hpp"

template <int SLICES>
__global__ __launch_bounds__(64) void k_vm_fold(uint32_t m, VmDev prog, const uint32_t* __restrict__ cst_g, Slab inF,
                                                Slab inS, Slab out, const int32_t* __restrict__ codes,
                                                const int32_t* __restrict__ gate = nullptr) {
  if (gate && *gate == 1) return;
  __builtin_amdgcn_s_setprio(2);
  const uint32_t slice = threadIdx.x / VM_FOLD_W, lane = threadIdx.x % VM_FOLD_W;
  const uint32_t sl = slice < SLICES ? slice : 0;
  auto [cst, slots] = vm_lds(cst_g, sl * FOLD_STRIDE_W);
  const uint32_t t = blockIdx.x * SLICES + slice;
  const bool active = slice < SLICES && 4 * t < m;
  fold_unit(t, m, prog, cst, slots, lane, active, inF, inS, out, codes);
}

__global__ __launch_bounds__(64) void k_vm_final(uint32_t m, VmDev prog, const uint32_t* __restrict__ cst_g, Slab inF,
                                                 Slab inS, Slab xS, int32_t* __restrict__ result) {
  __builtin_amdgcn_s_setprio(3);
  auto [cst, slots] = vm_lds(cst_g);
  const uint32_t lane = threadIdx.x;
  for (uint32_t k = lane; k < 4 * PART_PLANES; k += 64) {
    const uint32_t q = k / PART_PLANES, j = k % PART_PLANES;
    Fp v;
    if (q == 0 && j >= 12 && xS.p) {
      xS.ld(v, j - 12, 0);
    } else if (q < m) {
      if (j < 12) inF.ld(v, j, q);
      else inS.ld(v, j - 12, q);
    } else if (j == 0 || j == 12 + 2) {
      fp_one(v);
    } else {
      fp_zero(v);
    }
    slot_put(slots, VM_FINAL_IN[k], v.v);
  }
  __syncthreads();
  VM_ASSERT_INV(FINAL);
  vm::run<false, true, 3>(prog.code, VM_FINAL_NPHASES, VM_FINAL_W, lane, true, slots, cst, 0, vm::Out{nullptr, 0, 0},
                          blockIdx.x == 0 ? prog.trace : nullptr);
  if (lane == 0) *result = slot_flag_get(slots, VM_FINAL_OUT[0]) ? 1 : 0;
}

static_assert(VM_VOTEW_NIN == VM_VOTE1_NIN && VM_VOTEW_T_NIN == VM_VOTE_T1_NIN && VM_VOTEW_W == 64 &&
                  VM_VOTEW_T_W == 64 && VM_VOTE1_W == 64 && VM_VOTE_T1_W == 64,
              "one-vote-per-wave programs share the vote1 / vote_t1 layouts");
static_assert(VM_VOTE1H_IN_H0 == VM_VOTE1_IN_U00 && VM_VOTE_T1H_IN_H0 == VM_VOTE_T1_IN_U00 &&
                  VM_VOTE1H_OUT_SIG_GRP == VM_VOTE1_OUT_SIG_GRP && VM_VOTE_T1H_OUT_SIG_GRP == VM_VOTE_T1_OUT_SIG_GRP,
              "vote1h / vote_t1h share vote1 / vote_t1's layouts, H in place of the u's");
template <bool TABLE, bool HIN = false>
__device__ __forceinline__ void vote_wave(const VmDev& prog, uint32_t nph, uint32_t ns, const uint16_t* IN,
                                          const uint16_t* OUT, const uint32_t* __restrict__ cst_g,
                                          const uint8_t* __restrict__ pk_bytes, PkSrc pk, uint32_t e,
                                          const uint8_t* __restrict__ sig, Slab s, uint32_t i, uint64_t scalar,
                                          int32_t* __restrict__ code, Slab hc = Slab{nullptr, 0}, uint32_t he = 0,
                                          const uint32_t* __restrict__ hinf_in = nullptr,
                                          uint32_t* __restrict__ hinf_out = nullptr) {
  auto [cst, slots] = vm_lds(cst_g);
  uint32_t* hdr = slots + ns * 12;
  const uint32_t lane = threadIdx.x;
  if (lane == 0) {
    uint32_t x1[12], x0[12], bad, inf, sort, xz;
    parse_hdr(sig, 96, x1, x0, bad, inf, sort, xz);
    if constexpr (TABLE) {
      slot_put(slots, IN[VM_VOTE_T1_IN_SIG_X1], x1);
      slot_put(slots, IN[VM_VOTE_T1_IN_SIG_X0], x0);
      slot_flag(slots, IN[VM_VOTE_T1_IN_SIG_SORT], sort);
    } else {
      slot_put(slots, IN[VM_VOTE1_IN_SIG_X1], x1);
      slot_put(slots, IN[VM_VOTE1_IN_SIG_X0], x0);
      slot_flag(slots, IN[VM_VOTE1_IN_SIG_SORT], sort);
// ... 1301 lines not shown
    size_t d, lo, cnt;
    std::vector<uint32_t> perm;
  };
  std::vector<Dev> dev;
};

#define NFIN_STREAMS 4u
struct ovh_ctx {
  int device = 0;
  uint32_t flags = 0;
  hipStream_t stream = nullptr;
  hipStream_t fstream[NFIN_STREAMS] = {};
  uint32_t nfin = NFIN_STREAMS;
  hipStream_t xstream = nullptr;
  hipStream_t vstream[3] = {};
  hipStream_t hstream[4] = {};
  hipStream_t pool_st[3] = {};
  uint64_t* pool_q = nullptr;
  void* pool_desc = nullptr;
  uint32_t* pool_scr = nullptr;
  uint32_t pool_wgs = 0;
  uint32_t pool_grid0 = 0;
  uint32_t ncu = 256;
  uint32_t pool_rsv = 0;
  uint32_t pool_ncu = 256;
  uint64_t pool_seq = 0;
  uint32_t* pool_err = nullptr;
  uint64_t* plog = nullptr;
  uint64_t plog_seq[OVH_BATCH_SLOTS] = {};
  uint64_t plog_grids = 0;
  hipStream_t fs[OVH_BATCH_SLOTS] = {};
  hipEvent_t ev_front[OVH_BATCH_SLOTS] = {}, ev_back[OVH_BATCH_SLOTS] = {};
  hipEvent_t ev_x[4] = {};
  uint32_t* state_slot[OVH_BATCH_SLOTS] = {};
  uint32_t* red_slot[OVH_BATCH_SLOTS] = {};
  uint32_t *state_all = nullptr, *red_all = nullptr;
  uint8_t* pstage_all = nullptr;
  size_t state_w = 0, red_w = 0, pstage_b = 0;
  int32_t* grp_ok[OVH_BATCH_SLOTS] = {};
  uint32_t slot_n[OVH_BATCH_SLOTS] = {};
  uint32_t* fin = nullptr;
  uint32_t pipe_k = 0;
  int last_slot = 0;
  uint32_t small_max = SMALL_MAX;
  XmdTemplates xmd;
  std::mutex mu;
  uint32_t cap = 0, red_cap = 0;
  uint8_t* in_buf = nullptr;
  size_t in_cap = 0;
  uint32_t* scr = nullptr;
  int32_t *scr_pk = nullptr, *scr_sig = nullptr;
  uint32_t scr_cap = 0;
  uint32_t* comb = nullptr;
  uint32_t comb_cap = 0;
  uint32_t* part_out = nullptr;
  int32_t* result = nullptr;
  uint32_t last_n = 0;
  uint64_t test_seed = 0, test_base = 0;
  ValidatorTable tab;
  std::vector<QcRound> rounds;
  uint64_t round_next = 1;
  uint32_t* rsig = nullptr;
  uint32_t rsig_cap = 0;
  uint32_t* qc_buf = nullptr;
  uint32_t qc_cap = 0;
  uint32_t* qt_buf = nullptr;
  uint32_t qt_cap = 0;
  VerdictCache cache;
  std::vector<ovh_ctx*> sub;
  std::atomic<uint32_t> rr{0};
  std::vector<uint8_t> peer;
  std::vector<int> fin_devs;
  uint8_t* gather = nullptr;
  uint32_t* mfin = nullptr;
  uint32_t* msm_buf[OVH_BATCH_SLOTS] = {};
  uint64_t slot_seed[OVH_BATCH_SLOTS] = {}, slot_base[OVH_BATCH_SLOTS] = {};
  uint8_t* hst_h[OVH_BATCH_SLOTS] = {};
  uint8_t* hst_d[OVH_BATCH_SLOTS] = {};
  size_t hst_cap[OVH_BATCH_SLOTS] = {};
  hipEvent_t ev_m[OVH_BATCH_SLOTS][4] = {};
  uint8_t* mg = nullptr;
  std::deque<HostBatch> hq;
  uint64_t hb_k = 0;
  VmDev vm_vote{}, vm_vote_t{}, vm_fold{}, vm_final{}, vm_rs{}, vm_sigchk{}, vm_pkchk{}, vm_vote1{}, vm_vote_t1{},
      vm_signg0{}, vm_signg1{}, vm_pkgen{}, vm_vote1h{}, vm_vote_t1h{}, vm_qcpre{}, vm_qcmil{}, vm_votew{}, vm_votew_t{},
      vm_votewh{}, vm_votewh_t{}, vm_signg0h{}, vm_final1{}, vm_vsame{}, vm_vsame_t{}, vm_vsame8{}, vm_vsame8_t{},
      vm_h2g{}, vm_gfin{}, vm_g1grp{}, vm_pkdec{}, vm_gmil{}, vm_g1padd{}, vm_madd{}, vm_padd{}, vm_hdbl[5]{};
  uint32_t* vm_consts = nullptr;
  std::vector<void*> vm_bufs;
  uint32_t* gslab[OVH_BATCH_SLOTS] = {};
  uint32_t gcap[OVH_BATCH_SLOTS] = {};
  int samemsg = 1;
  uint32_t shard_span = 0;
  uint32_t shard_streams = 2;
  uint8_t* pstage[OVH_BATCH_SLOTS] = {};
  uint64_t sm_batches = 0, sm_votes = 0, sm_hashes = 0;
  uint32_t* sm1_plan = nullptr;
  size_t sm1_n = 0;
  std::vector<uint32_t> sm1_lo;
  uint8_t* sm1_hash = nullptr;
  uint32_t* hc_planes = nullptr;
  uint32_t* hc_inf = nullptr;
  std::unordered_map<std::string, uint32_t> hc_index;
  std::vector<std::string> hc_keys;
  uint32_t hc_next = 0;
  uint64_t hc_hits = 0, hc_misses = 0;
  hipStream_t prime_st = nullptr;
  uint32_t* prime_slab = nullptr;
  hipEvent_t prime_ev0 = nullptr, prime_ev = nullptr;
  bool prime_pending = false;
  uint64_t prime_enq = 0, prime_skip = 0, prime_signs = 0, prime_parts = 0;
  bool prime_sign = true, prime_batch = true;
  uint32_t clk_wgs = 0;
  bool clk_table = false;
  std::vector<uint32_t> blind_h;
  hipEvent_t ev0[OVH_NSTAGES] = {}, ev1[OVH_NSTAGES] = {};
  static constexpr uint32_t VEV_CAP = 256;
  hipEvent_t vev0[VEV_CAP] = {}, vev1[VEV_CAP] = {};
  uint32_t vev_n = 0;
  uint32_t ev_mask = 0;
};

#define HIPCHK(x)                                  \
  do {                                             \
    if ((x) != hipSuccess) return OVH_ERR_DEVICE;  \
  } while (0)
#define CHK(x)                \
  do {                              \
    const int e_ = (x);             \
    if (e_) return e_;              \
  } while (0)

static const char* const STAGE_NAMES[OVH_NSTAGES] = {"hash_to_field", "vote", "fold", "final", "bisect", "msm"};

constexpr size_t lds_bytes(uint32_t units, uint32_t stride_w, uint32_t extra_w = 0) {
  return ((size_t)SLOT_BASE_W + (size_t)units * stride_w + extra_w) * 4;
}
static constexpr size_t LDS_VOTE = lds_bytes(VM_SLICES, VOTE_STRIDE_W);
static constexpr size_t LDS_VOTE_T = lds_bytes(VM_SLICES, VOTE_T_STRIDE_W);
static constexpr size_t LDS_FOLD = lds_bytes(VM_FOLD_UNITS, FOLD_STRIDE_W);
static constexpr size_t LDS_FINAL = lds_bytes(1, VM_FINAL_NSLOTS * 12);
static_assert(VM_VOTE_W * VM_SLICES == 64 && VM_VOTE_T_W * VM_SLICES == 64 && VM_FOLD_W * VM_FOLD_UNITS == 64 &&
                  VM_FINAL_W == 64, "VM slice widths");
static constexpr size_t LDS_FOLD1 = lds_bytes(1, FOLD_STRIDE_W);
static constexpr size_t LDS_RS = lds_bytes(64 / VM_RS_W, RS_STRIDE_W);
constexpr uint32_t cmax(uint32_t a, uint32_t b) { return a > b ? a : b; }
static constexpr uint32_t MSM8_STRIDE_W = align128w(cmax(VM_MADD_NSLOTS, VM_PADD_NSLOTS) * 12);
static constexpr uint32_t HDBL_STRIDE_W =
    align128w(cmax(cmax(cmax(VM_HDBL1_NSLOTS, VM_HDBL2_NSLOTS), cmax(VM_HDBL4_NSLOTS, VM_HDBL8_NSLOTS)), VM_HDBL16_NSLOTS) * 12);
static constexpr size_t LDS_MSM8 = lds_bytes(64 / VM_MADD_W, MSM8_STRIDE_W);
static constexpr size_t LDS_HDBL = lds_bytes(64 / VM_HDBL1_W, HDBL_STRIDE_W);
static_assert(VM_MADD_W == VM_PADD_W && VM_HDBL1_W == VM_HDBL2_W && VM_HDBL1_W == VM_HDBL4_W && VM_HDBL1_W == VM_HDBL8_W &&
                  VM_HDBL1_W == VM_HDBL16_W && VM_MADD_NIN == 10 && VM_PADD_NIN == 12 && VM_HDBL1_NIN == 12,
              "MSM program shapes (tools/fpvm/progs.py)");
static constexpr size_t LDS_SIGCHK = lds_bytes(64 / VM_SIGCHK_W, SIGCHK_STRIDE_W);
static constexpr uint32_t VOTE1_NSLOTS = cmax(VM_VOTE1_NSLOTS, VM_VOTE_T1_NSLOTS);
static constexpr size_t LDS_VOTE1 = lds_bytes(1, VOTE1_NSLOTS * 12, 4);
static constexpr uint32_t VOTE1H_NSLOTS = cmax(VM_VOTE1H_NSLOTS, VM_VOTE_T1H_NSLOTS);
static constexpr size_t LDS_VOTE1H = lds_bytes(1, VOTE1H_NSLOTS * 12, 4);
static constexpr uint32_t VOTEW_NSLOTS = cmax(VM_VOTEW_NSLOTS, VM_VOTEW_T_NSLOTS);
static constexpr size_t LDS_VOTEW = lds_bytes(1, VOTEW_NSLOTS * 12, 4);
static constexpr uint32_t VOTEWH_NSLOTS = cmax(VM_VOTEWH_NSLOTS, VM_VOTEWH_T_NSLOTS);
static constexpr size_t LDS_VOTEWH = lds_bytes(1, VOTEWH_NSLOTS * 12, 4);
static constexpr size_t LDS_QCPRE = lds_bytes(1, VM_QCPRE_NSLOTS * 12, 4);
static constexpr size_t LDS_QCMIL = lds_bytes(1, VM_QCMIL_NSLOTS * 12);
static constexpr size_t LDS_FINAL1 = lds_bytes(1, VM_FINAL1_NSLOTS * 12);
static constexpr size_t LDS_SIGNG = lds_bytes(64 / VM_SIGNG0_W, SIGNG_STRIDE_W);
static_assert(LDS_SIGNG <= 80 * 1024, "signg LDS (raised limit, ovh_create)");
static constexpr size_t LDS_PKGEN = lds_bytes(64 / VM_PKGEN_W, PKGEN_STRIDE_W);
static constexpr size_t LDS_PKCHK = lds_bytes(64 / VM_PKCHK_W, PKCHK_STRIDE_W);
static constexpr uint32_t G1PADD_STRIDE_W = align128w(VM_G1PADD_NSLOTS * 12);
static constexpr size_t LDS_G1PADD = lds_bytes(64 / VM_G1PADD_W, G1PADD_STRIDE_W);
static_assert(LDS_RS <= 64 * 1024 && LDS_MSM8 <= 64 * 1024 && LDS_HDBL <= 64 * 1024 && LDS_SIGCHK <= 64 * 1024 &&
                  LDS_PKCHK <= 64 * 1024 && LDS_G1PADD <= 64 * 1024 && LDS_PKGEN <= 64 * 1024 &&
                  LDS_VOTE1 <= 64 * 1024 && LDS_FINAL1 <= 64 * 1024 && LDS_VOTEW <= 64 * 1024 && LDS_QCPRE <= 64 * 1024 && LDS_VOTE1H <= 64 * 1024 &&
                  LDS_QCMIL <= 64 * 1024 && VM_G1PADD_NIN == 6,
              "default LDS limit");
static_assert(LDS_VOTE <= 160 * 1024 && LDS_VOTE_T <= 160 * 1024 && LDS_FINAL <= 160 * 1024, "VM LDS budget");
static constexpr size_t LDS_VSAME = lds_bytes(VM_SLICES, VSAME_STRIDE_W);
static constexpr size_t LDS_VSAME8 = lds_bytes(8, VSAME8_STRIDE_W);
static_assert(LDS_VSAME8 <= 64 * 1024, "vsame8 LDS (default limit)");
static constexpr size_t LDS_H2G = lds_bytes(VM_SLICES, H2G_STRIDE_W);
static constexpr size_t LDS_GMIL = lds_bytes(1, VM_GMIL_NSLOTS * 12);
static_assert(LDS_VSAME <= 64 * 1024 && LDS_H2G <= 64 * 1024 && LDS_GMIL + 16 <= 64 * 1024, "same-message LDS");
static constexpr size_t LDS_PKDEC = lds_bytes(64 / VM_PKDEC_W, PKDEC_STRIDE_W);
static_assert(LDS_PKDEC <= 64 * 1024 && VM_PKDEC_NIN == 2, "pkdec LDS / shape");
static constexpr size_t LDS_G1GRP = lds_bytes(1, G1GRP_STRIDE_W);
static_assert(LDS_G1GRP <= 64 * 1024 && VM_G1GRP_NIN == 3, "g1grp LDS / shape");
static constexpr size_t LDS_GFIN = lds_bytes(1, VM_GFIN_NSLOTS * 12);
static_assert(LDS_GFIN + 16 <= 64 * 1024, "gfin LDS");
constexpr size_t lds_granule(size_t b) { return (b + 1023) / 1024 * 1024; }
static constexpr size_t LDS_POOL = LDS_VOTE > LDS_VOTE_T ? LDS_VOTE : LDS_VOTE_T;
static_assert(8 * lds_granule(LDS_POOL) <= 160 * 1024, "eight pool workgroups per CU");
static_assert(4 * lds_granule(LDS_VOTEW) <= 160 * 1024, "four votew workgroups per CU: a small batch is one round");
static constexpr uint32_t VOTEWH_PER_CU = (uint32_t)(160 * 1024 / lds_granule(LDS_VOTEWH));
static constexpr uint32_t VOTEWH_MAX = 256 * VOTEWH_PER_CU < SMALL_MAX ? 256 * VOTEWH_PER_CU : SMALL_MAX;
static_assert(LDS_VOTEWH <= 64 * 1024 && VOTEWH_PER_CU >= 4, "votewh LDS (default limit; four per CU: 1,024 waves)");
static_assert(VOTE_NSCR <= 4096 && VM_VOTE_NSLOTS <= 2048 && VM_VOTE_T_NSLOTS <= 2048,
              "side words: 12-bit scratch entries, 11-bit slots (fpvm.hpp side_spill)");
#ifndef POOL_HOLES_PER_8CU
#define POOL_HOLES_PER_8CU 8u
#endif
#define POOL_MAX_WGS 4096u
static_assert(FOLD_STRIDE_W <= VM_SLICES * VOTE_STRIDE_W && FOLD_STRIDE_W <= VM_SLICES * VOTE_T_STRIDE_W,
              "fused fold reuses the vote slots");

struct VmProg {
  const uint32_t* code;
  uint32_t nphases, W, NW;
  const uint16_t* in; uint32_t nin; const uint16_t* out; uint32_t nout;
  const uint32_t* side;
};
#define VM_PROG(P, ...) \
  VmProg { VM_##P##_CODE, VM_##P##_NPHASES, VM_##P##_W, VM_##P##_NW, VM_##P##_IN, VM_##P##_NIN, VM_##P##_OUT, VM_##P##_NOUT, __VA_ARGS__ }
#if VM_VOTE_NSCR == 0
#define VM_VOTE_SIDE nullptr
#endif
#if VM_VOTE_T_NSCR == 0
#define VM_VOTE_T_SIDE nullptr
#endif
struct VmRow {
  VmDev* (*dev)(ovh_ctx*);
  VmProg prog;
};
#define VM_ROW(member, ...) \
  VmRow { [](ovh_ctx* c) { return &c->member; }, VM_PROG(__VA_ARGS__) }
static const VmRow VM_TABLE[] = {
    VM_ROW(vm_vote, VOTE, VM_VOTE_SIDE),
    VM_ROW(vm_vote_t, VOTE_T, VM_VOTE_T_SIDE),
    VM_ROW(vm_fold, FOLD),
    VM_ROW(vm_final, FINAL),
    VM_ROW(vm_rs, RS),
    VM_ROW(vm_sigchk, SIGCHK),
    VM_ROW(vm_pkchk, PKCHK),
    VM_ROW(vm_vote1, VOTE1),
    VM_ROW(vm_vote_t1, VOTE_T1),
    VM_ROW(vm_signg0, SIGNG0),
    VM_ROW(vm_signg1, SIGNG1),
    VM_ROW(vm_pkgen, PKGEN),
    VM_ROW(vm_vote1h, VOTE1H),
    VM_ROW(vm_vote_t1h, VOTE_T1H),
    VM_ROW(vm_qcpre, QCPRE),
    VM_ROW(vm_qcmil, QCMIL),
    VM_ROW(vm_votew, VOTEW),
    VM_ROW(vm_votew_t, VOTEW_T),
    VM_ROW(vm_votewh, VOTEWH),
    VM_ROW(vm_votewh_t, VOTEWH_T),
    VM_ROW(vm_signg0h, SIGNG0H),
    VM_ROW(vm_final1, FINAL1),
    VM_ROW(vm_vsame, VSAME),
    VM_ROW(vm_vsame_t, VSAME_T),
    VM_ROW(vm_vsame8, VSAME8),
    VM_ROW(vm_vsame8_t, VSAME8_T),
    VM_ROW(vm_h2g, H2G),
    VM_ROW(vm_gfin, GFIN),
    VM_ROW(vm_g1grp, G1GRP),
    VM_ROW(vm_pkdec, PKDEC),
    VM_ROW(vm_gmil, GMIL),
    VM_ROW(vm_g1padd, G1PADD),
    VM_ROW(vm_madd, MADD),
    VM_ROW(vm_padd, PADD),
    VM_ROW(vm_hdbl[0], HDBL1),
    VM_ROW(vm_hdbl[1], HDBL2),
    VM_ROW(vm_hdbl[2], HDBL4),
    VM_ROW(vm_hdbl[3], HDBL8),
    VM_ROW(vm_hdbl[4], HDBL16),
};
static_assert(VM_RS_NOUT == 0 && VM_GMIL_NOUT == 0, "rs / gmil: no slot outputs (tools/fpvm/progs.py)");

static int vm_upload(ovh_ctx* c, VmDev& d, const VmProg& p) {
  const size_t words = (size_t)p.nphases * p.W * p.NW, pad = (size_t)vm::PREFETCH * p.W * p.NW;
  void *dc = nullptr, *di = nullptr, *dout = nullptr;
  HIPCHK(hipMalloc(&dc, (words + pad) * 4));
  c->vm_bufs.push_back(dc);
  HIPCHK(hipMemcpy(dc, p.code, words * 4, hipMemcpyHostToDevice));
  HIPCHK(hipMemset((uint32_t*)dc + words, 0, pad * 4));
  HIPCHK(hipMalloc(&di, p.nin * 2 + 2));
  c->vm_bufs.push_back(di);
  HIPCHK(hipMemcpy(di, p.in, p.nin * 2, hipMemcpyHostToDevice));
  HIPCHK(hipMalloc(&dout, p.nout * 2 + 2));
  c->vm_bufs.push_back(dout);
  HIPCHK(hipMemcpy(dout, p.out, p.nout * 2, hipMemcpyHostToDevice));
  d.code = (const uint4*)dc;
  d.nphases = p.nphases;
  d.in = (const uint16_t*)di;
  d.out = (const uint16_t*)dout;
  d.trace = nullptr;
  d.clk = nullptr;
  d.side = nullptr;
  if (p.side) {
    const size_t sw = (size_t)p.nphases * p.W;
    void* ds = nullptr;
    HIPCHK(hipMalloc(&ds, (sw + (size_t)vm::PREFETCH * p.W) * 4));
    c->vm_bufs.push_back(ds);
    HIPCHK(hipMemcpy(ds, p.side, sw * 4, hipMemcpyHostToDevice));
    HIPCHK(hipMemset((uint32_t*)ds + sw, 0, (size_t)vm::PREFETCH * p.W * 4));
    d.side = (const uint32_t*)ds;
  }
  if ((c->flags & OVH_FLAG_VM_CLOCK) && (p.code == VM_VOTE_CODE || p.code == VM_VOTE_T_CODE)) {
    void* dk = nullptr;
    HIPCHK(hipMalloc(&dk, (size_t)2 * VM_CLOCK_WGS * 8));
    c->vm_bufs.push_back(dk);
    HIPCHK(hipMemset(dk, 0, (size_t)2 * VM_CLOCK_WGS * 8));
    d.clk = (uint64_t*)dk;
  }
  if (c->flags & OVH_FLAG_VM_TRACE) {
    void* dt = nullptr;
    HIPCHK(hipMalloc(&dt, ((size_t)p.nphases + 1) * 8));
    c->vm_bufs.push_back(dt);
    HIPCHK(hipMemset(dt, 0, ((size_t)p.nphases + 1) * 8));
    d.trace = (uint64_t*)dt;
  }
  return 0;
}

static int vm_init(ovh_ctx* c) {
  HIPCHK(hipMalloc(&c->vm_consts, sizeof(VM_CONST_WORDS)));
  HIPCHK(hipMemcpy(c->vm_consts, VM_CONST_WORDS, sizeof(VM_CONST_WORDS), hipMemcpyHostToDevice));
  for (const VmRow& r : VM_TABLE) CHK(vm_upload(c, *r.dev(c), r.prog));
  HIPCHK(hipFuncSetAttribute((const void*)k_vm_pool, hipFuncAttributeMaxDynamicSharedMemorySize, (int)LDS_POOL));
  HIPCHK(hipFuncSetAttribute((const void*)k_vm_signg, hipFuncAttributeMaxDynamicSharedMemorySize, (int)LDS_SIGNG));
  HIPCHK(hipFuncSetAttribute((const void*)k_vm_fold<VM_FOLD_UNITS>, hipFuncAttributeMaxDynamicSharedMemorySize,
                             (int)LDS_FOLD));
  HIPCHK(hipFuncSetAttribute((const void*)k_vm_fold<1>, hipFuncAttributeMaxDynamicSharedMemorySize, (int)LDS_FOLD1));
  for (const void* k : {(const void*)k_vm_final, (const void*)k_vm_group, (const void*)k_vm_votechk})
    HIPCHK(hipFuncSetAttribute(k, hipFuncAttributeMaxDynamicSharedMemorySize, (int)LDS_FINAL));
  return 0;
}

struct StageScope {
  ovh_ctx* c;
  int k;
  hipStream_t st;
  StageScope(ovh_ctx* c_, int k_, hipStream_t st_ = nullptr) : c(c_), k(k_), st(st_ ? st_ : c_->stream) {
    if (c->flags & OVH_FLAG_PROFILE) (void)hipEventRecord(c->ev0[k], st);
  }
  ~StageScope() {
    if (c->flags & OVH_FLAG_PROFILE) {
      (void)hipEventRecord(c->ev1[k], st);
      c->ev_mask |= 1u << k;
    }
  }
};

static const uint8_t DEFAULT_DST[] = "BLS_SIG_BLS12381G2_XMD:SHA-256_SSWU_RO_NUL_";

static uint32_t nblk(size_t n) { return (uint32_t)((n + WG - 1) / WG); }

static Slab region_F(ovh_ctx* c, int slot, int r) {
  return Slab{c->red_slot[slot] + (size_t)r * PART_PLANES * 12 * c->red_cap, c->red_cap};
}
static Slab region_S(ovh_ctx* c, int slot, int r) {
  return Slab{c->red_slot[slot] + (size_t)r * PART_PLANES * 12 * c->red_cap + (size_t)12 * 12 * c->red_cap,
              c->red_cap};
}

namespace {
struct ParkedStream {
  int device;
  int prio;
  hipStream_t s;
};
std::mutex g_park_mu;
std::vector<ParkedStream> g_parked;
}

static hipError_t stream_new(hipStream_t* s, int prio) {
  int dev = 0;
  const hipError_t e = hipGetDevice(&dev);
  if (e != hipSuccess) return e;
  {
    std::lock_guard<std::mutex> g(g_park_mu);
    for (size_t k = 0; k < g_parked.size(); ++k)
      if (g_parked[k].device == dev && g_parked[k].prio == prio) {
        *s = g_parked[k].s;
        g_parked.erase(g_parked.begin() + (ptrdiff_t)k);
        return hipSuccess;
      }
  }
  return hipStreamCreateWithPriority(s, hipStreamNonBlocking, prio);
}

static void stream_park(int device, hipStream_t s) {
  if (!s) return;
  (void)hipStreamSynchronize(s);
  int prio = 0;
  if (hipStreamGetPriority(s, &prio) != hipSuccess) return;
  std::lock_guard<std::mutex> g(g_park_mu);
  g_parked.push_back(ParkedStream{device, prio, s});
}

template <class F>
static void each_stream(const ovh_ctx* c, F f) {
  for (hipStream_t s : {c->stream, c->fstream[0], c->fstream[1], c->fstream[2], c->fstream[3], c->xstream, c->vstream[0],
                        c->vstream[1], c->vstream[2], c->pool_st[0], c->pool_st[1], c->pool_st[2], c->hstream[1],
                        c->hstream[2], c->hstream[3], c->prime_st})
    if (s) f(s);
}
static_assert(NFIN_STREAMS == 4, "each_stream names the final streams");

static int pool_failed(const ovh_ctx* c) {
// ... 130 lines not shown
    *base = c->test_base;
    return 0;
  }
  uint8_t b[8];
  size_t got = 0;
  while (got < sizeof b) {
    const ssize_t r = getrandom(b + got, sizeof b - got, 0);
    if (r < 0) {
      if (errno == EINTR) continue;
      return OVH_ERR_RNG;
    }
    got += (size_t)r;
  }
  memcpy(seed, b, 8);
  *base = 0;
  return 0;
}

struct KeySrc {
  const uint8_t* bytes;
  PkSrc pts;
};

static uint32_t groups_of(uint32_t n) { return (n + GROUP_VOTES - 1) / GROUP_VOTES; }

static int batch_front(ovh_ctx* c, int slot, uint32_t n, const uint8_t* d_sigs, const uint8_t* d_hashes, KeySrc key,
                       int32_t* d_codes, bool alone = false, bool launch = true, bool shard = false) {
  Slab s{c->state_slot[slot], c->cap};
  c->ev_mask = 0;
  uint64_t seed, base;
  CHK(draw_seed(c, &seed, &base));
  if (n == 1 && alone) base = UNIT_BASE;
  c->slot_seed[slot] = seed;
  c->slot_base[slot] = base;
  uint8_t* ps = c->pstage[slot];
  const bool table = key.bytes == nullptr;
  const uint64_t seq = c->pool_seq++;
  {
    StageScope p(c, ST_H2F, c->stream);
    const uint32_t bytes = n * (table ? 96u : 144u) + (table && key.pts.idx ? n * 4u : 0u);
    k_pool_stage<<<std::min(1024u, (bytes + 16 * WG - 1) / (16 * WG)), WG, 0, c->stream>>>(
        n, d_sigs, key.bytes, table ? key.pts.idx : nullptr, ps);
    k_h2f<<<nblk(n), WG, 0, c->stream>>>(n, d_hashes, c->xmd, s);
  }
  PoolBatch b{};
  b.n = n;
  b.nq = (n + VM_SLICES - 1) / VM_SLICES;
  b.table = table;
  b.has_idx = table && key.pts.idx;
  b.seed = seed;
  b.base = base;
  b.codes = d_codes;
  b.planes = key.pts.planes;
  b.flags = key.pts.flags;
  b.pcap = key.pts.cap;
  b.state = s.p;
  b.cap = s.cap;
  const Slab r0 = region_F(c, slot, 0);
  b.part0 = r0.p;
  b.part_cap = r0.cap;
  b.stage = ps;
  b.clk = table ? c->vm_vote_t.clk : c->vm_vote.clk;
  b.plog = c->plog ? c->plog + (size_t)(seq % PLOG_RING) * PLOG_WORDS : nullptr;
  c->plog_seq[slot] = seq;
  k_pool_publish<<<1, 64, 0, c->stream>>>(b, (uint32_t)slot, seq, c->pool_q, (PoolBatch*)c->pool_desc);
  if (b.plog) k_stamp<<<1, 64, 0, c->stream>>>(b.plog + PLOG_EV_PUB, seq);
  HIPCHK(hipEventRecord(c->ev_front[slot], c->stream));
  c->slot_n[slot] = n;
  c->last_n = n;
  const bool vev = (c->flags & OVH_FLAG_PROFILE) != 0;
  const uint32_t vk = c->vev_n % ovh_ctx::VEV_CAP;
  const uint32_t wgs = c->pool_wgs;
  PoolArgs pa;
  pa.only = ~0ull;
  pa.nsimd = 4 * c->pool_ncu;
  pa.skip_cu = c->pool_rsv / 8;
  shard = shard && !c->pool_rsv;
  pa.q = c->pool_q;
  pa.descs = (const PoolBatch*)c->pool_desc;
  pa.pv_code = c->vm_vote.code;
  pa.pv_side = c->vm_vote.side;
  pa.pt_code = c->vm_vote_t.code;
  pa.pt_side = c->vm_vote_t.side;
  pa.fold_code = c->vm_fold.code;
  pa.cst = c->vm_consts;
  for (uint32_t par = 0; launch && par < (shard ? c->shard_streams : 2u); ++par) {
    if (shard && par != (uint32_t)(seq % c->shard_streams)) continue;
    if (shard) pa.only = seq + c->shard_span;
    hipStream_t pst = c->pool_st[par];
    HIPCHK(hipStreamWaitEvent(pst, c->ev_front[slot], 0));
    if (par == 0 || shard) {
      if (c->flags & OVH_FLAG_PROFILE) HIPCHK(hipEventRecord(c->ev0[ST_VOTE], pst));
      if (vev) HIPCHK(hipEventRecord(c->vev0[vk], pst));
    }
    const uint32_t gw = shard ? 2 * wgs : par == 0 ? c->pool_grid0 : 2 * wgs - c->pool_grid0;
    pa.scr = c->pool_scr + (size_t)par * 2 * wgs * VM_SLICES * VOTE_NSCR * 12;
    pa.wlog = nullptr;
    if (c->plog) {
      uint64_t* g = c->plog + PLOG_GRID_BASE + (size_t)(c->plog_grids++ % PLOG_GRIDS) * (4 + PLOG_WGS * PLOG_WG_WORDS);
      k_grid_hdr<<<1, 64, 0, pst>>>(g, seq, par, gw);
      pa.wlog = g + 4;
    }
    k_vm_pool<<<gw, 64, LDS_POOL, pst>>>(pa);
    if (par == 1 || shard) {
      if (c->flags & OVH_FLAG_PROFILE) {
        HIPCHK(hipEventRecord(c->ev1[ST_VOTE], pst));
        c->ev_mask |= 1u << ST_VOTE;
      }
      if (vev) {
        HIPCHK(hipEventRecord(c->vev1[vk], pst));
        ++c->vev_n;
      }
    }
  }
  c->clk_table = table;
  c->clk_wgs = c->pool_wgs < VM_CLOCK_WGS ? c->pool_wgs : VM_CLOCK_WGS;
  HIPCHK(hipGetLastError());
  return 0;
}

static uint64_t pool_wait_ticks(uint32_t n) { return 100000000ull * 4 + (uint64_t)n * 100 * OVH_BATCH_SLOTS; }

static void plog_stamp(ovh_ctx* c, int slot, uint32_t ev, hipStream_t st) {
  if (c->plog)
    k_stamp<<<1, 64, 0, st>>>(c->plog + (size_t)(c->plog_seq[slot] % PLOG_RING) * PLOG_WORDS + ev, ~0ull);
}

static int pool_join(ovh_ctx* c, int slot, hipStream_t st, int* reg, uint32_t* m) {
  const uint32_t n = c->slot_n[slot], nq = (n + VM_SLICES - 1) / VM_SLICES;
  k_pool_wait<<<1, 64, 0, st>>>(c->pool_q, (uint32_t)slot, nq, pool_wait_ticks(n), c->pool_err);
  plog_stamp(c, slot, PLOG_EV_DONE, st);
  *m = groups_of(n);
  *reg = 1;
  StageScope p(c, ST_FOLD, st);
  k_vm_fold<1><<<*m, 64, LDS_FOLD1, st>>>(nq, c->vm_fold, c->vm_consts, region_F(c, slot, 0), region_S(c, slot, 0),
                                           region_F(c, slot, 1), nullptr);
  return hipGetLastError() == hipSuccess ? 0 : OVH_ERR_DEVICE;
}


static int fold_down(ovh_ctx* c, int slot, hipStream_t st, int slices, int* reg, uint32_t* m, uint32_t until) {
  StageScope p(c, ST_FOLD, st);
  while (*m > until) {
    const uint32_t mo = (*m + 3) / 4;
    const int ro = *reg == 2 ? 3 : 2;
    if (slices == 1)
      k_vm_fold<1><<<mo, 64, LDS_FOLD1, st>>>(*m, c->vm_fold, c->vm_consts, region_F(c, slot, *reg),
                                              region_S(c, slot, *reg), region_F(c, slot, ro), nullptr);
    else
      k_vm_fold<VM_FOLD_UNITS><<<(mo + VM_FOLD_UNITS - 1) / VM_FOLD_UNITS, 64, LDS_FOLD, st>>>(
          *m, c->vm_fold, c->vm_consts, region_F(c, slot, *reg), region_S(c, slot, *reg), region_F(c, slot, ro),
          nullptr);
    *reg = ro;
    *m = mo;
  }
  return hipGetLastError() == hipSuccess ? 0 : OVH_ERR_DEVICE;
}

enum { RES_WORDS = 32 };
enum { RES_BATCH = 4, RES_COMBINE = RES_BATCH + OVH_BATCH_SLOTS, RES_SYNC = RES_COMBINE + OVH_BATCH_SLOTS, RES_MULTI };
static_assert(RES_MULTI + 1 + OVH_BATCH_SLOTS <= RES_WORDS, "verdict words fit c->result");

static void enqueue_final(ovh_ctx* c, hipStream_t st, Slab F, Slab S, uint32_t m, int32_t* d_res,
                          Slab xS = Slab{nullptr, 0}) {
  StageScope p(c, ST_FINAL, st);
  k_vm_final<<<1, 64, LDS_FINAL, st>>>(m, c->vm_final, c->vm_consts, F, S, xS, d_res);
}

// ... 3263 lines not shown
```

### consensus_overlord_amd/csrc/ovhip/pool.hpp

```cpp

#define POOL_SEQR 16u
#define POOL_QW 16u
enum : uint32_t {
  PQ_CUR = 0,
  PQ_NPUB = POOL_QW,
  PQ_SLOTOF = 2 * POOL_QW,
  PQ_NANN = 3 * POOL_QW,
  PQ_DONE = 4 * POOL_QW,
  PQ_CLAIM = PQ_DONE + OVH_BATCH_SLOTS * POOL_QW,
  PQ_INFL = PQ_CLAIM + OVH_BATCH_SLOTS * POOL_QW,
  PQ_OCC = PQ_INFL + POOL_QW,
};
constexpr uint32_t POOL_OCC_N = 4096;
constexpr uint32_t PQ_WORDS = PQ_OCC + POOL_OCC_N / 2;
static_assert(POOL_SEQR > OVH_BATCH_SLOTS && POOL_SEQR / 2 <= POOL_QW, "pool queue layout");
#define POOL_IDLE_TICKS 2000ull
#define POOL_WAIT_TICKS 2000000ull

__device__ __forceinline__ uint32_t simd_key() {
  const uint32_t hw = __builtin_amdgcn_s_getreg((31 << 11) | 4);
  const uint32_t xcc = __builtin_amdgcn_s_getreg((3 << 11) | 20);
  return (xcc & 7u) << 9 | ((hw >> 13) & 3u) << 7 | ((hw >> 12) & 1u) << 6 | ((hw >> 8) & 15u) << 2 |
         ((hw >> 4) & 3u);
}
// ... 139 lines not shown
      continue;
    }
    const uint32_t slot = __builtin_amdgcn_readfirstlane(
        __hip_atomic_load(pq_slot_of(q) + s % POOL_SEQR, __ATOMIC_RELAXED, __HIP_MEMORY_SCOPE_AGENT));
    bool held = false;
    if (np == s + 1) {
      hw |= 1u;
      bool busy;
      if (tdef && __builtin_amdgcn_readfirstlane(__hip_atomic_load(occ, __ATOMIC_RELAXED, __HIP_MEMORY_SCOPE_AGENT))) {
        busy = true;
      } else {
        busy = lane0_fetch_add32(occ, 1u) != 0;
        held = true;
      }
      if (busy) {
        hw |= 2u;
        const uint64_t cw = qldu(pq_claim(q, slot));
        const uint32_t nq = __builtin_amdgcn_readfirstlane(
            __hip_atomic_load(&descs[slot].nq, __ATOMIC_RELAXED, __HIP_MEMORY_SCOPE_AGENT));
        const uint64_t infl = qldu(q + PQ_INFL);
        const uint32_t taken = (uint32_t)cw;
        if ((cw >> 32) == s && taken < nq && (uint64_t)(nq - taken) + infl <= nsimd + nsimd / 16) {
          const uint64_t now = wclock();
          if (!tdef) tdef = now;
          if (now - tdef < POOL_SPREAD_TICKS) {
            hw |= 4u;
            if (held) (void)lane0_fetch_add32(occ, ~0u);
            __builtin_amdgcn_s_sleep(32);
            continue;
          }
        }
        hw |= 8u;
      }
    }
    if (!held) (void)lane0_fetch_add32(occ, 1u);
    const uint64_t old = lane0_fetch_add(pq_claim(q, slot), 1ull);
    const uint64_t seq = old >> 32;
    const uint32_t idx = (uint32_t)old;
    const uint64_t tw = wclock();
    while (qldu(q + PQ_NPUB) <= seq && wclock() - tw < 100000000ull) __builtin_amdgcn_s_sleep(2);
    const uint32_t nq = __builtin_amdgcn_readfirstlane(
        __hip_atomic_load(&descs[slot].nq, __ATOMIC_RELAXED, __HIP_MEMORY_SCOPE_AGENT));
    asm volatile("s_waitcnt vmcnt(0)" ::: "memory");
    const uint64_t dseq = qldu(&descs[slot].seq);
    const bool mine = dseq == seq && idx < nq;
    if (seq != s || !mine) lane0_cas(q + PQ_CUR, s, s + 1);
    if (mine) {
      (void)lane0_fetch_add(q + PQ_INFL, 1ull);
      *slot_out = slot;
      *quad_out = idx;
      *how = hw;
      return 1;
    }
    (void)lane0_fetch_add32(occ, ~0u);
    tdef = 0;
    t0 = wclock();
  }
  return 0;
}

template <typename T>
__device__ __forceinline__ T dget(const T* p) {
  return __hip_atomic_load(p, __ATOMIC_RELAXED, __HIP_MEMORY_SCOPE_AGENT);
}
template <typename T>
__device__ __forceinline__ T* dgetp(T* const* p) {
  return reinterpret_cast<T*>(__hip_atomic_load(reinterpret_cast<const uint64_t*>(p), __ATOMIC_RELAXED,
                                                __HIP_MEMORY_SCOPE_AGENT));
}
__device__ __forceinline__ uint32_t uni(uint32_t v) { return __builtin_amdgcn_readfirstlane(v); }
__device__ __forceinline__ uint64_t uni64(uint64_t v) {
  return ((uint64_t)uni((uint32_t)(v >> 32)) << 32) | uni((uint32_t)v);
}
template <typename T>
__device__ __forceinline__ T* unip(T* p) {
  return reinterpret_cast<T*>(uni64(reinterpret_cast<uint64_t>(p)));
}

#ifndef OVH_POOL_UNROLL
#define OVH_POOL_UNROLL 3
#endif
__device__ __forceinline__ void vote_quad(const PoolArgs& a, uint32_t slot_in, uint32_t quad_in, uint32_t* lds,
                                          const bool TABLE) {
  VM_ASSERT_NO_INV(VOTE);
  VM_ASSERT_NO_INV(VOTE_T);
  const uint32_t NSLOTS = TABLE ? VM_VOTE_T_NSLOTS : VM_VOTE_NSLOTS;
  const uint32_t STRIDE = TABLE ? VOTE_T_STRIDE_W : VOTE_STRIDE_W;
  const uint32_t NPH = TABLE ? VM_VOTE_T_NPHASES : VM_VOTE_NPHASES;
  const uint16_t* IN = TABLE ? VM_VOTE_T_IN : VM_VOTE_IN;
  const uint16_t* OUT = TABLE ? VM_VOTE_T_OUT : VM_VOTE_OUT;
  uint32_t* cst = lds;
  const uint32_t slice = threadIdx.x / VM_VOTE_W, lane = threadIdx.x % VM_VOTE_W;
  uint32_t* slots = lds + SLOT_BASE_W + slice * STRIDE;
  uint32_t* hdr = slots + NSLOTS * 12;
  uint32_t* park = lds + SLOT_BASE_W + 2 * STRIDE + NSLOTS * 12 + 2;
  {
    const PoolBatch* bd = a.descs + slot_in;
    const uint32_t i = (quad_in & 0x0FFFFFFFu) * VM_SLICES + slice;
    const uint32_t n = uni(dget(&bd->n));
    const bool active = i < n;
    const uint8_t* sigs = unip(dgetp(&bd->stage));
    const Slab s{unip(dgetp(&bd->state)), uni(dget(&bd->cap))};
    if (active) {
      if (lane == 0) {
        uint32_t x1[12], x0[12], bad, inf, sort, xz;
        parse_hdr(sigs + (size_t)i * 96, 96, x1, x0, bad, inf, sort, xz);
        slot_put(slots, IN[TABLE ? VM_VOTE_T_IN_SIG_X1 : VM_VOTE_IN_SIG_X1], x1);
        slot_put(slots, IN[TABLE ? VM_VOTE_T_IN_SIG_X0 : VM_VOTE_IN_SIG_X0], x0);
        slot_flag(slots, IN[TABLE ? VM_VOTE_T_IN_SIG_SORT : VM_VOTE_IN_SIG_SORT], sort);
        hdr[0] = bad | inf << 1 | xz << 2;
      } else if (lane >= 2 && lane < 6) {
        Fp u;
        s.ld(u, S_U + (lane - 2), i);
        slot_put(slots, IN[(TABLE ? VM_VOTE_T_IN_U00 : VM_VOTE_IN_U00) + (lane - 2)], u.v);
      }
    }
    if (threadIdx.x == 0) {
      park[0] = slot_in;
      park[1] = quad_in;
      if (dgetp(&bd->plog)) {
        uint32_t* h3 = lds + SLOT_BASE_W + 3 * STRIDE + NSLOTS * 12 + 2;
        const uint64_t t = __builtin_amdgcn_s_memrealtime();
        h3[0] = (uint32_t)t;
        h3[1] = (uint32_t)(t >> 32);
      }
    }
    __syncthreads();
    if (active) {
      if (TABLE) {
        const int32_t* idx = reinterpret_cast<const int32_t*>(sigs + (size_t)n * 144);
        const uint32_t e = uni(dget(&bd->has_idx)) ? (uint32_t)idx[i] : i;
        if (lane == 1) {
          hdr[1] = unip(dgetp(&bd->flags))[e];
        } else if (lane >= 6 && lane < 9) {
          Fp v;
          Slab{const_cast<uint32_t*>(unip(dgetp(&bd->planes))), uni(dget(&bd->pcap))}.ld(v, lane - 6, e);
          slot_put(slots, IN[VM_VOTE_T_IN_PK_X + (lane - 6)], v.v);
        }
      } else {
        if (lane == 1) {
          uint32_t x[12], bad, inf, sort, xz;
          parse_hdr(sigs + (size_t)n * 96 + (size_t)i * 48, 48, x, x, bad, inf, sort, xz);
          slot_put(slots, IN[VM_VOTE_IN_PK_X], x);
          slot_flag(slots, IN[VM_VOTE_IN_PK_SORT], sort);
          hdr[1] = bad | inf << 1 | xz << 2;
        }
      }
    }
    if (threadIdx.x == 0 && dgetp(&bd->clk)) {
      const uint64_t t0 = __builtin_amdgcn_s_memtime(), r0 = __builtin_amdgcn_s_memrealtime();
      uint32_t* h0 = lds + SLOT_BASE_W + NSLOTS * 12 + 2;
      uint32_t* h1 = lds + SLOT_BASE_W + STRIDE + NSLOTS * 12 + 2;
      h0[0] = (uint32_t)t0;
      h0[1] = (uint32_t)(t0 >> 32);
      h1[0] = (uint32_t)r0;
      h1[1] = (uint32_t)(r0 >> 32);
    }
    __syncthreads();
    const uint64_t scalar = vote_scalar(uni64(dget(&bd->seed)), uni64(dget(&bd->base)), i);
    vm::run<true, false, OVH_POOL_UNROLL>(
        TABLE ? a.pt_code : a.pv_code, NPH, VM_VOTE_W, lane, active, slots, cst, scalar, vm::Out{s.p, s.cap, i},
        nullptr, TABLE ? a.pt_side : a.pv_side,
        a.scr + (size_t)blockIdx.x * VM_SLICES * VOTE_NSCR * 12 + slice * VOTE_NSCR * 12);
  }
  const uint32_t slot = uni(park[0]), quad = uni(park[1]) & 0x0FFFFFFFu, how = uni(park[1]) >> 28;
  const PoolBatch* bd = a.descs + slot;
  const uint32_t i = quad * VM_SLICES + slice;
  const uint32_t n = uni(dget(&bd->n));
  int32_t* codes = unip(dgetp(&bd->codes));
  if (uint64_t* clk = dgetp(&bd->clk); clk && threadIdx.x == 0 && blockIdx.x < VM_CLOCK_WGS) {
    const uint32_t* h0 = lds + SLOT_BASE_W + NSLOTS * 12 + 2;
    const uint32_t* h1 = lds + SLOT_BASE_W + STRIDE + NSLOTS * 12 + 2;
    const uint64_t t0 = h0[0] | (uint64_t)h0[1] << 32, r0 = h1[0] | (uint64_t)h1[1] << 32;
    clk[2 * blockIdx.x] = __builtin_amdgcn_s_memtime() - t0;
    clk[2 * blockIdx.x + 1] = __builtin_amdgcn_s_memrealtime() - r0;
  }
  if (i < n && lane == 0) {
    const uint32_t sf = hdr[0], pf = hdr[1];
    const uint32_t sg_bad = sf & 1, sg_inf = (sf >> 1) & 1, sg_xz = (sf >> 2) & 1;
    const uint32_t sg_ok = slot_flag_get(slots, OUT[TABLE ? VM_VOTE_T_OUT_SIG_OK : VM_VOTE_OUT_SIG_OK]);
    const uint32_t sg_grp = slot_flag_get(slots, OUT[TABLE ? VM_VOTE_T_OUT_SIG_GRP : VM_VOTE_OUT_SIG_GRP]);
    const uint32_t h_inf = slot_flag_get(slots, OUT[TABLE ? VM_VOTE_T_OUT_H_INF : VM_VOTE_OUT_H_INF]);
    uint32_t pk_parse, pk_inf, pk_grp;
    if (TABLE) {
      pk_parse = pf & PKF_PARSE;
      pk_inf = pf & PKF_INF;
      pk_grp = !(pf & PKF_GRP);
    } else {
      const uint32_t pk_bad = pf & 1, pk_xz = (pf >> 2) & 1;
      pk_inf = (pf >> 1) & 1;
      const uint32_t pk_ok = slot_flag_get(slots, OUT[VM_VOTE_OUT_PK_OK]);
      pk_grp = slot_flag_get(slots, OUT[VM_VOTE_OUT_PK_GRP]);
      pk_parse = pk_bad || (!pk_inf && (!pk_ok || pk_xz));
    }
    int32_t c;
    if (pk_parse) c = OVH_ERR_PUBKEY;
    else if (sg_bad) c = BLST_BAD_ENCODING;
    else if (!sg_inf && !sg_ok) c = BLST_POINT_NOT_ON_CURVE;
    else if (!sg_inf && (sg_xz || !sg_grp)) c = BLST_POINT_NOT_IN_GROUP;
    else if (pk_inf) c = BLST_PK_IS_INFINITY;
    else if (!pk_grp) c = BLST_POINT_NOT_IN_GROUP;
    else if (h_inf || sg_inf) c = BLST_VERIFY_FAIL;
    else c = 0;
    codes[i] = c;
  }
  __threadfence();
  __syncthreads();
  uint64_t* const pl = threadIdx.x == 0 && quad < PLOG_QUADS ? dgetp(&bd->plog) : nullptr;
  uint64_t pl_start = 0;
  if (pl) {
    const uint32_t* h3 = lds + SLOT_BASE_W + 3 * STRIDE + NSLOTS * 12 + 2;
    pl_start = (uint64_t)h3[0] | (uint64_t)(h3[1] & 0xFFFFu) << 32;
  }
  const Slab s{unip(dgetp(&bd->state)), uni(dget(&bd->cap))};
  VmDev fold{};
  fold.code = a.fold_code;
  fold_unit<1>(quad, n, fold, cst, lds + SLOT_BASE_W, threadIdx.x % VM_FOLD_W, threadIdx.x < VM_FOLD_W,
            Slab{s.p + (size_t)S_F * 12 * s.cap, s.cap}, Slab{nullptr, 0},
            Slab{unip(dgetp(&bd->part0)), uni(dget(&bd->part_cap))}, codes);
  if (pl) {
    pl[16 + 2 * quad] = pl_start | (uint64_t)simd_key() << 48 | (uint64_t)how << 60;
    pl[16 + 2 * quad + 1] = __builtin_amdgcn_s_memrealtime();
  }
  __builtin_amdgcn_fence(__ATOMIC_RELEASE, "agent");
  asm volatile("s_waitcnt vmcnt(0)" ::: "memory");
  if (threadIdx.x == 0) {
    __hip_atomic_fetch_add(pq_done(a.q, slot), 1ull, __ATOMIC_RELAXED, __HIP_MEMORY_SCOPE_AGENT);
    __hip_atomic_fetch_add(a.q + PQ_INFL, ~0ull, __ATOMIC_RELAXED, __HIP_MEMORY_SCOPE_AGENT);
    __hip_atomic_fetch_add(pq_occ(a.q) + simd_key(), ~0u, __ATOMIC_RELAXED, __HIP_MEMORY_SCOPE_AGENT);
  }
}

__global__ __launch_bounds__(64, 2) void k_vm_pool(PoolArgs a) {
  __builtin_amdgcn_s_setprio(2);
  extern __shared__ uint4 lds4[];
  if (a.skip_cu && ((simd_key() >> 2) & 0x7Fu) < a.skip_cu) return;
  uint32_t* lds = reinterpret_cast<uint32_t*>(lds4);
  load_consts(lds, a.cst, VM_NCONST);
  const uint64_t t_in = __builtin_amdgcn_s_memrealtime();
  vote_stagger();
  uint32_t nquads = 0, why = 0;
#pragma unroll 1
  for (;; ++nquads) {
    uint32_t slot = 0, quad = 0, how = 0;
    if (!pool_claim(a.q, a.descs, &slot, &quad, &why, a.only, a.nsimd, &how)) break;
    slot = uni(slot);
    quad = uni(quad) | uni(how) << 28;
    __builtin_amdgcn_fence(__ATOMIC_ACQUIRE, "agent");
    vote_quad(a, slot, quad, lds, uni(dget(&a.descs[slot].table)) != 0);
  }
  if (a.wlog && threadIdx.x == 0 && blockIdx.x < PLOG_WGS) {
    uint64_t* w = a.wlog + (size_t)blockIdx.x * PLOG_WG_WORDS;
    w[0] = t_in;
    w[1] = __builtin_amdgcn_s_memrealtime();
    w[2] = nquads;
    w[3] = why;
  }
}

__global__ __launch_bounds__(64) void k_pool_wait(uint64_t* q, uint32_t slot, uint32_t nq, uint64_t ticks,
                                                  uint32_t* err) {
  if (threadIdx.x) return;
  const uint64_t t0 = wall_clock64();
  while (__hip_atomic_load(pq_done(q, slot), __ATOMIC_RELAXED, __HIP_MEMORY_SCOPE_AGENT) < nq) {
    if (wall_clock64() - t0 > ticks) {
      __hip_atomic_store(err, 1u, __ATOMIC_RELAXED, __HIP_MEMORY_SCOPE_SYSTEM);
      return;
    }
    __builtin_amdgcn_s_sleep(32);
  }
}

__global__ __launch_bounds__(WG) void k_pool_stage(uint32_t n, const uint8_t* __restrict__ sigs,
                                                   const uint8_t* __restrict__ pks, const int32_t* __restrict__ idx,
                                                   uint8_t* __restrict__ dst) {
  const size_t nb = (size_t)n * 96 + (pks ? (size_t)n * 48 : 0);
  uint8_t* di = dst + (size_t)n * 144;
  for (size_t k = (size_t)blockIdx.x * WG + threadIdx.x; k < nb + (idx ? (size_t)n * 4 : 0);
       k += (size_t)gridDim.x * WG) {
    if (k < (size_t)n * 96) dst[k] = sigs[k];
    else if (k < nb) dst[k] = pks[k - (size_t)n * 96];
    else di[k - nb] = reinterpret_cast<const uint8_t*>(idx)[k - nb];
  }
}
```

Measured before the change: 1.804 million verifications/s.

## Run pool vote programs in Montgomery radix 2^392 with a compact constant table

```diff
diff --git a/consensus_overlord_amd/csrc/bls/fp.hpp b/consensus_overlord_amd/csrc/bls/fp.hpp
--- a/consensus_overlord_amd/csrc/bls/fp.hpp
+++ b/consensus_overlord_amd/csrc/bls/fp.hpp
@@ -145,6 +145,45 @@
   for (int i = 0; i < 12; ++i) d[i] = subc32(t[i], P_LIMBS[i], br, &br);
 #pragma unroll
   for (int i = 0; i < 12; ++i) r.v[i] = br ? t[i] : d[i];
+#endif
+}
+
+OVH_HD void fp_mul_wide(Fp& r, const Fp& a, const Fp& b) {
+#if defined(__HIP_DEVICE_COMPILE__)
+#if defined(OVH_FPMUL28_2ACC) || defined(OVH_FPMUL_2ACC)
+#error "the wide product (radix 2^392) has the one-accumulator 14 x 28 form only"
+#endif
+  fp_mul28w_gfx950(r.v, a.v, b.v);
+#else
+  OVH_COUNT_MUL();
+  uint32_t t[13];
+#pragma unroll
+  for (int j = 0; j < 13; ++j) t[j] = 0;
+#pragma unroll
+  for (int i = 0; i < 12; ++i) {
+    const uint32_t bi = b.v[i];
+    uint64_t c = (uint64_t)a.v[0] * bi + t[0];
+    t[0] = (uint32_t)c;
+    const uint32_t m = t[0] * P_INV32;
+    uint64_t c2 = (uint64_t)m * P_LIMBS[0] + t[0];
+#pragma unroll
+    for (int j = 1; j < 12; ++j) {
+      c = (uint64_t)a.v[j] * bi + t[j] + (c >> 32);
+      c2 = (uint64_t)m * P_LIMBS[j] + (uint32_t)c + (c2 >> 32);
+      t[j - 1] = (uint32_t)c2;
+    }
+    t[11] = (uint32_t)(c >> 32) + (uint32_t)(c2 >> 32);
+  }
+  const uint32_t m8 = (t[0] * P_INV32) & 0xFFu;
+  uint64_t cy = 0;
+#pragma unroll
+  for (int j = 0; j < 12; ++j) {
+    cy = (uint64_t)m8 * P_LIMBS[j] + t[j] + (cy >> 32);
+    t[j] = (uint32_t)cy;
+  }
+  t[12] = (uint32_t)(cy >> 32);
+#pragma unroll
+  for (int j = 0; j < 12; ++j) r.v[j] = (t[j] >> 8) | (t[j + 1] << 24);
 #endif
 }
 
diff --git a/consensus_overlord_amd/csrc/bls/fp_mul28.hpp b/consensus_overlord_amd/csrc/bls/fp_mul28.hpp
--- a/consensus_overlord_amd/csrc/bls/fp_mul28.hpp
+++ b/consensus_overlord_amd/csrc/bls/fp_mul28.hpp
@@ -29,6 +29,23 @@
       if (s > 4 && w + 1 < 12) v |= a[w + 1] << (32 - s);
     }
     x[k] = v & M28;
+  }
+}
+
+__device__ __forceinline__ void join28(uint32_t* u, const uint32_t* t) {
+#if defined(OVH_UBENCH_NOSPLIT)
+#pragma unroll
+  for (int j = 0; j < 12; ++j) u[j] = t[j];
+  return;
+#endif
+#pragma unroll
+  for (int j = 0; j < 12; ++j) {
+    const int k = (32 * j) / 28, s = (32 * j) % 28;
+    static_assert(28 % 4 == 0, "s <= 24: no third limb");
+    const uint32_t lo = s ? t[k] >> s : t[k];
+    uint32_t v;
+    asm("v_lshl_or_b32 %0, %1, %2, %3" : "=v"(v) : "v"(t[k + 1]), "n"(28 - s), "v"(lo));
+    u[j] = v;
   }
 }
 
diff --git a/consensus_overlord_amd/csrc/bls/fp_mul28_gfx950.hpp b/consensus_overlord_amd/csrc/bls/fp_mul28_gfx950.hpp
--- a/consensus_overlord_amd/csrc/bls/fp_mul28_gfx950.hpp
+++ b/consensus_overlord_amd/csrc/bls/fp_mul28_gfx950.hpp
@@ -145,6 +145,76 @@
   (void)m;
   join28_reduce(r, t);
 }
+__device__ __forceinline__ void fp_mul28w_gfx950(uint32_t* __restrict__ r, const uint32_t* __restrict__ a,
+                                         const uint32_t* __restrict__ b) {
+  uint32_t x[14], y[14], m[14], t[14];
+  split28<0>(x, a);
+  split28<0>(y, b);
+  asm volatile(
+      "v_mad_u64_u32 v[252:253], vcc, %[x0], %[y0], 0\n\tv_mul_lo_u32 %[m0], v252, %[pinv]\n\tv_and_b32_e32 %[m0], %[mask], %[m0]\n\tv_mad_u64_u32 v[252:253], vcc, %[m0], %[p0], v[252:253]\n\tv_lshrrev_b64 v[252:253], 28, v[252:253]\n\tv_mad_u64_u32 v[252:253], vcc, %[x0], %[y1], v[252:253]\n\tv_mad_u64_u32 v[252:253], vcc, %[x1], %[y0], v[252:253]\n\tv_mad_u64_u32 v[252:253], vcc, %[m0], %[p1], v[252:253]\n\t"
+      "v_mul_lo_u32 %[m1], v252, %[pinv]\n\tv_and_b32_e32 %[m1], %[mask], %[m1]\n\tv_mad_u64_u32 v[252:253], vcc, %[m1], %[p0], v[252:253]\n\tv_lshrrev_b64 v[252:253], 28, v[252:253]\n\tv_mad_u64_u32 v[252:253], vcc, %[x0], %[y2], v[252:253]\n\tv_mad_u64_u32 v[252:253], vcc, %[x1], %[y1], v[252:253]\n\tv_mad_u64_u32 v[252:253], vcc, %[x2], %[y0], v[252:253]\n\tv_mad_u64_u32 v[252:253], vcc, %[m0], %[p2], v[252:253]\n\t"
+      "v_mad_u64_u32 v[252:253], vcc, %[m1], %[p1], v[252:253]\n\tv_mul_lo_u32 %[m2], v252, %[pinv]\n\tv_and_b32_e32 %[m2], %[mask], %[m2]\n\tv_mad_u64_u32 v[252:253], vcc, %[m2], %[p0], v[252:253]\n\tv_lshrrev_b64 v[252:253], 28, v[252:253]\n\tv_mad_u64_u32 v[252:253], vcc, %[x0], %[y3], v[252:253]\n\tv_mad_u64_u32 v[252:253], vcc, %[x1], %[y2], v[252:253]\n\tv_mad_u64_u32 v[252:253], vcc, %[x2], %[y1], v[252:253]\n\t"
+      "v_mad_u64_u32 v[252:253], vcc, %[x3], %[y0], v[252:253]\n\tv_mad_u64_u32 v[252:253], vcc, %[m0], %[p3], v[252:253]\n\tv_mad_u64_u32 v[252:253], vcc, %[m1], %[p2], v[252:253]\n\tv_mad_u64_u32 v[252:253], vcc, %[m2], %[p1], v[252:253]\n\tv_mul_lo_u32 %[m3], v252, %[pinv]\n\tv_and_b32_e32 %[m3], %[mask], %[m3]\n\tv_mad_u64_u32 v[252:253], vcc, %[m3], %[p0], v[252:253]\n\tv_lshrrev_b64 v[252:253], 28, v[252:253]\n\t"
+      "v_mad_u64_u32 v[252:253], vcc, %[x0], %[y4], v[252:253]\n\tv_mad_u64_u32 v[252:253], vcc, %[x1], %[y3], v[252:253]\n\tv_mad_u64_u32 v[252:253], vcc, %[x2], %[y2], v[252:253]\n\tv_mad_u64_u32 v[252:253], vcc, %[x3], %[y1], v[252:253]\n\tv_mad_u64_u32 v[252:253], vcc, %[x4], %[y0], v[252:253]\n\tv_mad_u64_u32 v[252:253], vcc, %[m0], %[p4], v[252:253]\n\tv_mad_u64_u32 v[252:253], vcc, %[m1], %[p3], v[252:253]\n\tv_mad_u64_u32 v[252:253], vcc, %[m2], %[p2], v[252:253]\n\t"
+      "v_mad_u64_u32 v[252:253], vcc, %[m3], %[p1], v[252:253]\n\tv_mul_lo_u32 %[m4], v252, %[pinv]\n\tv_and_b32_e32 %[m4], %[mask], %[m4]\n\tv_mad_u64_u32 v[252:253], vcc, %[m4], %[p0], v[252:253]\n\tv_lshrrev_b64 v[252:253], 28, v[252:253]\n\tv_mad_u64_u32 v[252:253], vcc, %[x0], %[y5], v[252:253]\n\tv_mad_u64_u32 v[252:253], vcc, %[x1], %[y4], v[252:253]\n\tv_mad_u64_u32 v[252:253], vcc, %[x2], %[y3], v[252:253]\n\t"
+      "v_mad_u64_u32 v[252:253], vcc, %[x3], %[y2], v[252:253]\n\tv_mad_u64_u32 v[252:253], vcc, %[x4], %[y1], v[252:253]\n\tv_mad_u64_u32 v[252:253], vcc, %[x5], %[y0], v[252:253]\n\tv_mad_u64_u32 v[252:253], vcc, %[m0], %[p5], v[252:253]\n\tv_mad_u64_u32 v[252:253], vcc, %[m1], %[p4], v[252:253]\n\tv_mad_u64_u32 v[252:253], vcc, %[m2], %[p3], v[252:253]\n\tv_mad_u64_u32 v[252:253], vcc, %[m3], %[p2], v[252:253]\n\tv_mad_u64_u32 v[252:253], vcc, %[m4], %[p1], v[252:253]\n\t"
+      "v_mul_lo_u32 %[m5], v252, %[pinv]\n\tv_and_b32_e32 %[m5], %[mask], %[m5]\n\tv_mad_u64_u32 v[252:253], vcc, %[m5], %[p0], v[252:253]\n\tv_lshrrev_b64 v[252:253], 28, v[252:253]\n\tv_mad_u64_u32 v[252:253], vcc, %[x0], %[y6], v[252:253]\n\tv_mad_u64_u32 v[252:253], vcc, %[x1], %[y5], v[252:253]\n\tv_mad_u64_u32 v[252:253], vcc, %[x2], %[y4], v[252:253]\n\tv_mad_u64_u32 v[252:253], vcc, %[x3], %[y3], v[252:253]\n\t"
+      "v_mad_u64_u32 v[252:253], vcc, %[x4], %[y2], v[252:253]\n\tv_mad_u64_u32 v[252:253], vcc, %[x5], %[y1], v[252:253]\n\tv_mad_u64_u32 v[252:253], vcc, %[x6], %[y0], v[252:253]\n\tv_mad_u64_u32 v[252:253], vcc, %[m0], %[p6], v[252:253]\n\tv_mad_u64_u32 v[252:253], vcc, %[m1], %[p5], v[252:253]\n\tv_mad_u64_u32 v[252:253], vcc, %[m2], %[p4], v[252:253]\n\tv_mad_u64_u32 v[252:253], vcc, %[m3], %[p3], v[252:253]\n\tv_mad_u64_u32 v[252:253], vcc, %[m4], %[p2], v[252:253]\n\t"
+      "v_mad_u64_u32 v[252:253], vcc, %[m5], %[p1], v[252:253]\n\tv_mul_lo_u32 %[m6], v252, %[pinv]\n\tv_and_b32_e32 %[m6], %[mask], %[m6]\n\tv_mad_u64_u32 v[252:253], vcc, %[m6], %[p0], v[252:253]\n\tv_lshrrev_b64 v[252:253], 28, v[252:253]\n\tv_mad_u64_u32 v[252:253], vcc, %[x0], %[y7], v[252:253]\n\tv_mad_u64_u32 v[252:253], vcc, %[x1], %[y6], v[252:253]\n\tv_mad_u64_u32 v[252:253], vcc, %[x2], %[y5], v[252:253]\n\t"
+      "v_mad_u64_u32 v[252:253], vcc, %[x3], %[y4], v[252:253]\n\tv_mad_u64_u32 v[252:253], vcc, %[x4], %[y3], v[252:253]\n\tv_mad_u64_u32 v[252:253], vcc, %[x5], %[y2], v[252:253]\n\tv_mad_u64_u32 v[252:253], vcc, %[x6], %[y1], v[252:253]\n\tv_mad_u64_u32 v[252:253], vcc, %[x7], %[y0], v[252:253]\n\tv_mad_u64_u32 v[252:253], vcc, %[m0], %[p7], v[252:253]\n\tv_mad_u64_u32 v[252:253], vcc, %[m1], %[p6], v[252:253]\n\tv_mad_u64_u32 v[252:253], vcc, %[m2], %[p5], v[252:253]\n\t"
+      "v_mad_u64_u32 v[252:253], vcc, %[m3], %[p4], v[252:253]\n\tv_mad_u64_u32 v[252:253], vcc, %[m4], %[p3], v[252:253]\n\tv_mad_u64_u32 v[252:253], vcc, %[m5], %[p2], v[252:253]\n\tv_mad_u64_u32 v[252:253], vcc, %[m6], %[p1], v[252:253]\n\tv_mul_lo_u32 %[m7], v252, %[pinv]\n\tv_and_b32_e32 %[m7], %[mask], %[m7]\n\tv_mad_u64_u32 v[252:253], vcc, %[m7], %[p0], v[252:253]\n\tv_lshrrev_b64 v[252:253], 28, v[252:253]\n\t"
+      "v_mad_u64_u32 v[252:253], vcc, %[x0], %[y8], v[252:253]\n\tv_mad_u64_u32 v[252:253], vcc, %[x1], %[y7], v[252:253]\n\tv_mad_u64_u32 v[252:253], vcc, %[x2], %[y6], v[252:253]\n\tv_mad_u64_u32 v[252:253], vcc, %[x3], %[y5], v[252:253]\n\tv_mad_u64_u32 v[252:253], vcc, %[x4], %[y4], v[252:253]\n\tv_mad_u64_u32 v[252:253], vcc, %[x5], %[y3], v[252:253]\n\tv_mad_u64_u32 v[252:253], vcc, %[x6], %[y2], v[252:253]\n\tv_mad_u64_u32 v[252:253], vcc, %[x7], %[y1], v[252:253]\n\t"
+      "v_mad_u64_u32 v[252:253], vcc, %[x8], %[y0], v[252:253]\n\tv_mad_u64_u32 v[252:253], vcc, %[m0], %[p8], v[252:253]\n\tv_mad_u64_u32 v[252:253], vcc, %[m1], %[p7], v[252:253]\n\tv_mad_u64_u32 v[252:253], vcc, %[m2], %[p6], v[252:253]\n\tv_mad_u64_u32 v[252:253], vcc, %[m3], %[p5], v[252:253]\n\tv_mad_u64_u32 v[252:253], vcc, %[m4], %[p4], v[252:253]\n\tv_mad_u64_u32 v[252:253], vcc, %[m5], %[p3], v[252:253]\n\tv_mad_u64_u32 v[252:253], vcc, %[m6], %[p2], v[252:253]\n\t"
+      "v_mad_u64_u32 v[252:253], vcc, %[m7], %[p1], v[252:253]\n\tv_mul_lo_u32 %[m8], v252, %[pinv]\n\tv_and_b32_e32 %[m8], %[mask], %[m8]\n\tv_mad_u64_u32 v[252:253], vcc, %[m8], %[p0], v[252:253]\n\tv_lshrrev_b64 v[252:253], 28, v[252:253]\n\tv_mad_u64_u32 v[252:253], vcc, %[x0], %[y9], v[252:253]\n\tv_mad_u64_u32 v[252:253], vcc, %[x1], %[y8], v[252:253]\n\tv_mad_u64_u32 v[252:253], vcc, %[x2], %[y7], v[252:253]\n\t"
+      "v_mad_u64_u32 v[252:253], vcc, %[x3], %[y6], v[252:253]\n\tv_mad_u64_u32 v[252:253], vcc, %[x4], %[y5], v[252:253]\n\tv_mad_u64_u32 v[252:253], vcc, %[x5], %[y4], v[252:253]\n\tv_mad_u64_u32 v[252:253], vcc, %[x6], %[y3], v[252:253]\n\tv_mad_u64_u32 v[252:253], vcc, %[x7], %[y2], v[252:253]\n\tv_mad_u64_u32 v[252:253], vcc, %[x8], %[y1], v[252:253]\n\tv_mad_u64_u32 v[252:253], vcc, %[x9], %[y0], v[252:253]\n\tv_mad_u64_u32 v[252:253], vcc, %[m0], %[p9], v[252:253]\n\t"
+      "v_mad_u64_u32 v[252:253], vcc, %[m1], %[p8], v[252:253]\n\tv_mad_u64_u32 v[252:253], vcc, %[m2], %[p7], v[252:253]\n\tv_mad_u64_u32 v[252:253], vcc, %[m3], %[p6], v[252:253]\n\tv_mad_u64_u32 v[252:253], vcc, %[m4], %[p5], v[252:253]\n\tv_mad_u64_u32 v[252:253], vcc, %[m5], %[p4], v[252:253]\n\tv_mad_u64_u32 v[252:253], vcc, %[m6], %[p3], v[252:253]\n\tv_mad_u64_u32 v[252:253], vcc, %[m7], %[p2], v[252:253]\n\tv_mad_u64_u32 v[252:253], vcc, %[m8], %[p1], v[252:253]\n\t"
+      "v_mul_lo_u32 %[m9], v252, %[pinv]\n\tv_and_b32_e32 %[m9], %[mask], %[m9]\n\tv_mad_u64_u32 v[252:253], vcc, %[m9], %[p0], v[252:253]\n\tv_lshrrev_b64 v[252:253], 28, v[252:253]\n\tv_mad_u64_u32 v[252:253], vcc, %[x0], %[y10], v[252:253]\n\tv_mad_u64_u32 v[252:253], vcc, %[x1], %[y9], v[252:253]\n\tv_mad_u64_u32 v[252:253], vcc, %[x2], %[y8], v[252:253]\n\tv_mad_u64_u32 v[252:253], vcc, %[x3], %[y7], v[252:253]\n\t"
+      "v_mad_u64_u32 v[252:253], vcc, %[x4], %[y6], v[252:253]\n\tv_mad_u64_u32 v[252:253], vcc, %[x5], %[y5], v[252:253]\n\tv_mad_u64_u32 v[252:253], vcc, %[x6], %[y4], v[252:253]\n\tv_mad_u64_u32 v[252:253], vcc, %[x7], %[y3], v[252:253]\n\tv_mad_u64_u32 v[252:253], vcc, %[x8], %[y2], v[252:253]\n\tv_mad_u64_u32 v[252:253], vcc, %[x9], %[y1], v[252:253]\n\tv_mad_u64_u32 v[252:253], vcc, %[x10], %[y0], v[252:253]\n\tv_mad_u64_u32 v[252:253], vcc, %[m0], %[p10], v[252:253]\n\t"
+      "v_mad_u64_u32 v[252:253], vcc, %[m1], %[p9], v[252:253]\n\tv_mad_u64_u32 v[252:253], vcc, %[m2], %[p8], v[252:253]\n\tv_mad_u64_u32 v[252:253], vcc, %[m3], %[p7], v[252:253]\n\tv_mad_u64_u32 v[252:253], vcc, %[m4], %[p6], v[252:253]\n\tv_mad_u64_u32 v[252:253], vcc, %[m5], %[p5], v[252:253]\n\tv_mad_u64_u32 v[252:253], vcc, %[m6], %[p4], v[252:253]\n\tv_mad_u64_u32 v[252:253], vcc, %[m7], %[p3], v[252:253]\n\tv_mad_u64_u32 v[252:253], vcc, %[m8], %[p2], v[252:253]\n\t"
+      "v_mad_u64_u32 v[252:253], vcc, %[m9], %[p1], v[252:253]\n\tv_mul_lo_u32 %[m10], v252, %[pinv]\n\tv_and_b32_e32 %[m10], %[mask], %[m10]\n\tv_mad_u64_u32 v[252:253], vcc, %[m10], %[p0], v[252:253]\n\tv_lshrrev_b64 v[252:253], 28, v[252:253]\n\tv_mad_u64_u32 v[252:253], vcc, %[x0], %[y11], v[252:253]\n\tv_mad_u64_u32 v[252:253], vcc, %[x1], %[y10], v[252:253]\n\tv_mad_u64_u32 v[252:253], vcc, %[x2], %[y9], v[252:253]\n\t"
+      "v_mad_u64_u32 v[252:253], vcc, %[x3], %[y8], v[252:253]\n\tv_mad_u64_u32 v[252:253], vcc, %[x4], %[y7], v[252:253]\n\tv_mad_u64_u32 v[252:253], vcc, %[x5], %[y6], v[252:253]\n\tv_mad_u64_u32 v[252:253], vcc, %[x6], %[y5], v[252:253]\n\tv_mad_u64_u32 v[252:253], vcc, %[x7], %[y4], v[252:253]\n\tv_mad_u64_u32 v[252:253], vcc, %[x8], %[y3], v[252:253]\n\tv_mad_u64_u32 v[252:253], vcc, %[x9], %[y2], v[252:253]\n\tv_mad_u64_u32 v[252:253], vcc, %[x10], %[y1], v[252:253]\n\t"
+      "v_mad_u64_u32 v[252:253], vcc, %[x11], %[y0], v[252:253]\n\tv_mad_u64_u32 v[252:253], vcc, %[m0], %[p11], v[252:253]\n\tv_mad_u64_u32 v[252:253], vcc, %[m1], %[p10], v[252:253]\n\tv_mad_u64_u32 v[252:253], vcc, %[m2], %[p9], v[252:253]\n\tv_mad_u64_u32 v[252:253], vcc, %[m3], %[p8], v[252:253]\n\tv_mad_u64_u32 v[252:253], vcc, %[m4], %[p7], v[252:253]\n\tv_mad_u64_u32 v[252:253], vcc, %[m5], %[p6], v[252:253]\n\tv_mad_u64_u32 v[252:253], vcc, %[m6], %[p5], v[252:253]\n\t"
+      "v_mad_u64_u32 v[252:253], vcc, %[m7], %[p4], v[252:253]\n\tv_mad_u64_u32 v[252:253], vcc, %[m8], %[p3], v[252:253]\n\tv_mad_u64_u32 v[252:253], vcc, %[m9], %[p2], v[252:253]\n\tv_mad_u64_u32 v[252:253], vcc, %[m10], %[p1], v[252:253]\n\tv_mul_lo_u32 %[m11], v252, %[pinv]\n\tv_and_b32_e32 %[m11], %[mask], %[m11]\n\tv_mad_u64_u32 v[252:253], vcc, %[m11], %[p0], v[252:253]\n\tv_lshrrev_b64 v[252:253], 28, v[252:253]\n\t"
+      "v_mad_u64_u32 v[252:253], vcc, %[x0], %[y12], v[252:253]\n\tv_mad_u64_u32 v[252:253], vcc, %[x1], %[y11], v[252:253]\n\tv_mad_u64_u32 v[252:253], vcc, %[x2], %[y10], v[252:253]\n\tv_mad_u64_u32 v[252:253], vcc, %[x3], %[y9], v[252:253]\n\tv_mad_u64_u32 v[252:253], vcc, %[x4], %[y8], v[252:253]\n\tv_mad_u64_u32 v[252:253], vcc, %[x5], %[y7], v[252:253]\n\tv_mad_u64_u32 v[252:253], vcc, %[x6], %[y6], v[252:253]\n\tv_mad_u64_u32 v[252:253], vcc, %[x7], %[y5], v[252:253]\n\t"
+      "v_mad_u64_u32 v[252:253], vcc, %[x8], %[y4], v[252:253]\n\tv_mad_u64_u32 v[252:253], vcc, %[x9], %[y3], v[252:253]\n\tv_mad_u64_u32 v[252:253], vcc, %[x10], %[y2], v[252:253]\n\tv_mad_u64_u32 v[252:253], vcc, %[x11], %[y1], v[252:253]\n\tv_mad_u64_u32 v[252:253], vcc, %[x12], %[y0], v[252:253]\n\tv_mad_u64_u32 v[252:253], vcc, %[m0], %[p12], v[252:253]\n\tv_mad_u64_u32 v[252:253], vcc, %[m1], %[p11], v[252:253]\n\tv_mad_u64_u32 v[252:253], vcc, %[m2], %[p10], v[252:253]\n\t"
+      "v_mad_u64_u32 v[252:253], vcc, %[m3], %[p9], v[252:253]\n\tv_mad_u64_u32 v[252:253], vcc, %[m4], %[p8], v[252:253]\n\tv_mad_u64_u32 v[252:253], vcc, %[m5], %[p7], v[252:253]\n\tv_mad_u64_u32 v[252:253], vcc, %[m6], %[p6], v[252:253]\n\tv_mad_u64_u32 v[252:253], vcc, %[m7], %[p5], v[252:253]\n\tv_mad_u64_u32 v[252:253], vcc, %[m8], %[p4], v[252:253]\n\tv_mad_u64_u32 v[252:253], vcc, %[m9], %[p3], v[252:253]\n\tv_mad_u64_u32 v[252:253], vcc, %[m10], %[p2], v[252:253]\n\t"
+      "v_mad_u64_u32 v[252:253], vcc, %[m11], %[p1], v[252:253]\n\tv_mul_lo_u32 %[m12], v252, %[pinv]\n\tv_and_b32_e32 %[m12], %[mask], %[m12]\n\tv_mad_u64_u32 v[252:253], vcc, %[m12], %[p0], v[252:253]\n\tv_lshrrev_b64 v[252:253], 28, v[252:253]\n\tv_mad_u64_u32 v[252:253], vcc, %[x0], %[y13], v[252:253]\n\tv_mad_u64_u32 v[252:253], vcc, %[x1], %[y12], v[252:253]\n\tv_mad_u64_u32 v[252:253], vcc, %[x2], %[y11], v[252:253]\n\t"
+      "v_mad_u64_u32 v[252:253], vcc, %[x3], %[y10], v[252:253]\n\tv_mad_u64_u32 v[252:253], vcc, %[x4], %[y9], v[252:253]\n\tv_mad_u64_u32 v[252:253], vcc, %[x5], %[y8], v[252:253]\n\tv_mad_u64_u32 v[252:253], vcc, %[x6], %[y7], v[252:253]\n\tv_mad_u64_u32 v[252:253], vcc, %[x7], %[y6], v[252:253]\n\tv_mad_u64_u32 v[252:253], vcc, %[x8], %[y5], v[252:253]\n\tv_mad_u64_u32 v[252:253], vcc, %[x9], %[y4], v[252:253]\n\tv_mad_u64_u32 v[252:253], vcc, %[x10], %[y3], v[252:253]\n\t"
+      "v_mad_u64_u32 v[252:253], vcc, %[x11], %[y2], v[252:253]\n\tv_mad_u64_u32 v[252:253], vcc, %[x12], %[y1], v[252:253]\n\tv_mad_u64_u32 v[252:253], vcc, %[x13], %[y0], v[252:253]\n\tv_mad_u64_u32 v[252:253], vcc, %[m0], %[p13], v[252:253]\n\tv_mad_u64_u32 v[252:253], vcc, %[m1], %[p12], v[252:253]\n\tv_mad_u64_u32 v[252:253], vcc, %[m2], %[p11], v[252:253]\n\tv_mad_u64_u32 v[252:253], vcc, %[m3], %[p10], v[252:253]\n\tv_mad_u64_u32 v[252:253], vcc, %[m4], %[p9], v[252:253]\n\t"
+      "v_mad_u64_u32 v[252:253], vcc, %[m5], %[p8], v[252:253]\n\tv_mad_u64_u32 v[252:253], vcc, %[m6], %[p7], v[252:253]\n\tv_mad_u64_u32 v[252:253], vcc, %[m7], %[p6], v[252:253]\n\tv_mad_u64_u32 v[252:253], vcc, %[m8], %[p5], v[252:253]\n\tv_mad_u64_u32 v[252:253], vcc, %[m9], %[p4], v[252:253]\n\tv_mad_u64_u32 v[252:253], vcc, %[m10], %[p3], v[252:253]\n\tv_mad_u64_u32 v[252:253], vcc, %[m11], %[p2], v[252:253]\n\tv_mad_u64_u32 v[252:253], vcc, %[m12], %[p1], v[252:253]\n\t"
+      "v_mul_lo_u32 %[m13], v252, %[pinv]\n\tv_and_b32_e32 %[m13], %[mask], %[m13]\n\tv_mad_u64_u32 v[252:253], vcc, %[m13], %[p0], v[252:253]\n\tv_lshrrev_b64 v[252:253], 28, v[252:253]\n\tv_mad_u64_u32 v[252:253], vcc, %[x1], %[y13], v[252:253]\n\tv_mad_u64_u32 v[252:253], vcc, %[x2], %[y12], v[252:253]\n\tv_mad_u64_u32 v[252:253], vcc, %[x3], %[y11], v[252:253]\n\tv_mad_u64_u32 v[252:253], vcc, %[x4], %[y10], v[252:253]\n\t"
+      "v_mad_u64_u32 v[252:253], vcc, %[x5], %[y9], v[252:253]\n\tv_mad_u64_u32 v[252:253], vcc, %[x6], %[y8], v[252:253]\n\tv_mad_u64_u32 v[252:253], vcc, %[x7], %[y7], v[252:253]\n\tv_mad_u64_u32 v[252:253], vcc, %[x8], %[y6], v[252:253]\n\tv_mad_u64_u32 v[252:253], vcc, %[x9], %[y5], v[252:253]\n\tv_mad_u64_u32 v[252:253], vcc, %[x10], %[y4], v[252:253]\n\tv_mad_u64_u32 v[252:253], vcc, %[x11], %[y3], v[252:253]\n\tv_mad_u64_u32 v[252:253], vcc, %[x12], %[y2], v[252:253]\n\t"
+      "v_mad_u64_u32 v[252:253], vcc, %[x13], %[y1], v[252:253]\n\tv_mad_u64_u32 v[252:253], vcc, %[m1], %[p13], v[252:253]\n\tv_mad_u64_u32 v[252:253], vcc, %[m2], %[p12], v[252:253]\n\tv_mad_u64_u32 v[252:253], vcc, %[m3], %[p11], v[252:253]\n\tv_mad_u64_u32 v[252:253], vcc, %[m4], %[p10], v[252:253]\n\tv_mad_u64_u32 v[252:253], vcc, %[m5], %[p9], v[252:253]\n\tv_mad_u64_u32 v[252:253], vcc, %[m6], %[p8], v[252:253]\n\tv_mad_u64_u32 v[252:253], vcc, %[m7], %[p7], v[252:253]\n\t"
+      "v_mad_u64_u32 v[252:253], vcc, %[m8], %[p6], v[252:253]\n\tv_mad_u64_u32 v[252:253], vcc, %[m9], %[p5], v[252:253]\n\tv_mad_u64_u32 v[252:253], vcc, %[m10], %[p4], v[252:253]\n\tv_mad_u64_u32 v[252:253], vcc, %[m11], %[p3], v[252:253]\n\tv_mad_u64_u32 v[252:253], vcc, %[m12], %[p2], v[252:253]\n\tv_mad_u64_u32 v[252:253], vcc, %[m13], %[p1], v[252:253]\n\tv_and_b32_e32 %[t0], %[mask], v252\n\tv_lshrrev_b64 v[252:253], 28, v[252:253]\n\t"
+      "v_mad_u64_u32 v[252:253], vcc, %[x2], %[y13], v[252:253]\n\tv_mad_u64_u32 v[252:253], vcc, %[x3], %[y12], v[252:253]\n\tv_mad_u64_u32 v[252:253], vcc, %[x4], %[y11], v[252:253]\n\tv_mad_u64_u32 v[252:253], vcc, %[x5], %[y10], v[252:253]\n\tv_mad_u64_u32 v[252:253], vcc, %[x6], %[y9], v[252:253]\n\tv_mad_u64_u32 v[252:253], vcc, %[x7], %[y8], v[252:253]\n\tv_mad_u64_u32 v[252:253], vcc, %[x8], %[y7], v[252:253]\n\tv_mad_u64_u32 v[252:253], vcc, %[x9], %[y6], v[252:253]\n\t"
+      "v_mad_u64_u32 v[252:253], vcc, %[x10], %[y5], v[252:253]\n\tv_mad_u64_u32 v[252:253], vcc, %[x11], %[y4], v[252:253]\n\tv_mad_u64_u32 v[252:253], vcc, %[x12], %[y3], v[252:253]\n\tv_mad_u64_u32 v[252:253], vcc, %[x13], %[y2], v[252:253]\n\tv_mad_u64_u32 v[252:253], vcc, %[m2], %[p13], v[252:253]\n\tv_mad_u64_u32 v[252:253], vcc, %[m3], %[p12], v[252:253]\n\tv_mad_u64_u32 v[252:253], vcc, %[m4], %[p11], v[252:253]\n\tv_mad_u64_u32 v[252:253], vcc, %[m5], %[p10], v[252:253]\n\t"
+      "v_mad_u64_u32 v[252:253], vcc, %[m6], %[p9], v[252:253]\n\tv_mad_u64_u32 v[252:253], vcc, %[m7], %[p8], v[252:253]\n\tv_mad_u64_u32 v[252:253], vcc, %[m8], %[p7], v[252:253]\n\tv_mad_u64_u32 v[252:253], vcc, %[m9], %[p6], v[252:253]\n\tv_mad_u64_u32 v[252:253], vcc, %[m10], %[p5], v[252:253]\n\tv_mad_u64_u32 v[252:253], vcc, %[m11], %[p4], v[252:253]\n\tv_mad_u64_u32 v[252:253], vcc, %[m12], %[p3], v[252:253]\n\tv_mad_u64_u32 v[252:253], vcc, %[m13], %[p2], v[252:253]\n\t"
+      "v_and_b32_e32 %[t1], %[mask], v252\n\tv_lshrrev_b64 v[252:253], 28, v[252:253]\n\tv_mad_u64_u32 v[252:253], vcc, %[x3], %[y13], v[252:253]\n\tv_mad_u64_u32 v[252:253], vcc, %[x4], %[y12], v[252:253]\n\tv_mad_u64_u32 v[252:253], vcc, %[x5], %[y11], v[252:253]\n\tv_mad_u64_u32 v[252:253], vcc, %[x6], %[y10], v[252:253]\n\tv_mad_u64_u32 v[252:253], vcc, %[x7], %[y9], v[252:253]\n\tv_mad_u64_u32 v[252:253], vcc, %[x8], %[y8], v[252:253]\n\t"
+      "v_mad_u64_u32 v[252:253], vcc, %[x9], %[y7], v[252:253]\n\tv_mad_u64_u32 v[252:253], vcc, %[x10], %[y6], v[252:253]\n\tv_mad_u64_u32 v[252:253], vcc, %[x11], %[y5], v[252:253]\n\tv_mad_u64_u32 v[252:253], vcc, %[x12], %[y4], v[252:253]\n\tv_mad_u64_u32 v[252:253], vcc, %[x13], %[y3], v[252:253]\n\tv_mad_u64_u32 v[252:253], vcc, %[m3], %[p13], v[252:253]\n\tv_mad_u64_u32 v[252:253], vcc, %[m4], %[p12], v[252:253]\n\tv_mad_u64_u32 v[252:253], vcc, %[m5], %[p11], v[252:253]\n\t"
+      "v_mad_u64_u32 v[252:253], vcc, %[m6], %[p10], v[252:253]\n\tv_mad_u64_u32 v[252:253], vcc, %[m7], %[p9], v[252:253]\n\tv_mad_u64_u32 v[252:253], vcc, %[m8], %[p8], v[252:253]\n\tv_mad_u64_u32 v[252:253], vcc, %[m9], %[p7], v[252:253]\n\tv_mad_u64_u32 v[252:253], vcc, %[m10], %[p6], v[252:253]\n\tv_mad_u64_u32 v[252:253], vcc, %[m11], %[p5], v[252:253]\n\tv_mad_u64_u32 v[252:253], vcc, %[m12], %[p4], v[252:253]\n\tv_mad_u64_u32 v[252:253], vcc, %[m13], %[p3], v[252:253]\n\t"
+      "v_and_b32_e32 %[t2], %[mask], v252\n\tv_lshrrev_b64 v[252:253], 28, v[252:253]\n\tv_mad_u64_u32 v[252:253], vcc, %[x4], %[y13], v[252:253]\n\tv_mad_u64_u32 v[252:253], vcc, %[x5], %[y12], v[252:253]\n\tv_mad_u64_u32 v[252:253], vcc, %[x6], %[y11], v[252:253]\n\tv_mad_u64_u32 v[252:253], vcc, %[x7], %[y10], v[252:253]\n\tv_mad_u64_u32 v[252:253], vcc, %[x8], %[y9], v[252:253]\n\tv_mad_u64_u32 v[252:253], vcc, %[x9], %[y8], v[252:253]\n\t"
+      "v_mad_u64_u32 v[252:253], vcc, %[x10], %[y7], v[252:253]\n\tv_mad_u64_u32 v[252:253], vcc, %[x11], %[y6], v[252:253]\n\tv_mad_u64_u32 v[252:253], vcc, %[x12], %[y5], v[252:253]\n\tv_mad_u64_u32 v[252:253], vcc, %[x13], %[y4], v[252:253]\n\tv_mad_u64_u32 v[252:253], vcc, %[m4], %[p13], v[252:253]\n\tv_mad_u64_u32 v[252:253], vcc, %[m5], %[p12], v[252:253]\n\tv_mad_u64_u32 v[252:253], vcc, %[m6], %[p11], v[252:253]\n\tv_mad_u64_u32 v[252:253], vcc, %[m7], %[p10], v[252:253]\n\t"
+      "v_mad_u64_u32 v[252:253], vcc, %[m8], %[p9], v[252:253]\n\tv_mad_u64_u32 v[252:253], vcc, %[m9], %[p8], v[252:253]\n\tv_mad_u64_u32 v[252:253], vcc, %[m10], %[p7], v[252:253]\n\tv_mad_u64_u32 v[252:253], vcc, %[m11], %[p6], v[252:253]\n\tv_mad_u64_u32 v[252:253], vcc, %[m12], %[p5], v[252:253]\n\tv_mad_u64_u32 v[252:253], vcc, %[m13], %[p4], v[252:253]\n\tv_and_b32_e32 %[t3], %[mask], v252\n\tv_lshrrev_b64 v[252:253], 28, v[252:253]\n\t"
+      "v_mad_u64_u32 v[252:253], vcc, %[x5], %[y13], v[252:253]\n\tv_mad_u64_u32 v[252:253], vcc, %[x6], %[y12], v[252:253]\n\tv_mad_u64_u32 v[252:253], vcc, %[x7], %[y11], v[252:253]\n\tv_mad_u64_u32 v[252:253], vcc, %[x8], %[y10], v[252:253]\n\tv_mad_u64_u32 v[252:253], vcc, %[x9], %[y9], v[252:253]\n\tv_mad_u64_u32 v[252:253], vcc, %[x10], %[y8], v[252:253]\n\tv_mad_u64_u32 v[252:253], vcc, %[x11], %[y7], v[252:253]\n\tv_mad_u64_u32 v[252:253], vcc, %[x12], %[y6], v[252:253]\n\t"
+      "v_mad_u64_u32 v[252:253], vcc, %[x13], %[y5], v[252:253]\n\tv_mad_u64_u32 v[252:253], vcc, %[m5], %[p13], v[252:253]\n\tv_mad_u64_u32 v[252:253], vcc, %[m6], %[p12], v[252:253]\n\tv_mad_u64_u32 v[252:253], vcc, %[m7], %[p11], v[252:253]\n\tv_mad_u64_u32 v[252:253], vcc, %[m8], %[p10], v[252:253]\n\tv_mad_u64_u32 v[252:253], vcc, %[m9], %[p9], v[252:253]\n\tv_mad_u64_u32 v[252:253], vcc, %[m10], %[p8], v[252:253]\n\tv_mad_u64_u32 v[252:253], vcc, %[m11], %[p7], v[252:253]\n\t"
+      "v_mad_u64_u32 v[252:253], vcc, %[m12], %[p6], v[252:253]\n\tv_mad_u64_u32 v[252:253], vcc, %[m13], %[p5], v[252:253]\n\tv_and_b32_e32 %[t4], %[mask], v252\n\tv_lshrrev_b64 v[252:253], 28, v[252:253]\n\tv_mad_u64_u32 v[252:253], vcc, %[x6], %[y13], v[252:253]\n\tv_mad_u64_u32 v[252:253], vcc, %[x7], %[y12], v[252:253]\n\tv_mad_u64_u32 v[252:253], vcc, %[x8], %[y11], v[252:253]\n\tv_mad_u64_u32 v[252:253], vcc, %[x9], %[y10], v[252:253]\n\t"
+      "v_mad_u64_u32 v[252:253], vcc, %[x10], %[y9], v[252:253]\n\tv_mad_u64_u32 v[252:253], vcc, %[x11], %[y8], v[252:253]\n\tv_mad_u64_u32 v[252:253], vcc, %[x12], %[y7], v[252:253]\n\tv_mad_u64_u32 v[252:253], vcc, %[x13], %[y6], v[252:253]\n\tv_mad_u64_u32 v[252:253], vcc, %[m6], %[p13], v[252:253]\n\tv_mad_u64_u32 v[252:253], vcc, %[m7], %[p12], v[252:253]\n\tv_mad_u64_u32 v[252:253], vcc, %[m8], %[p11], v[252:253]\n\tv_mad_u64_u32 v[252:253], vcc, %[m9], %[p10], v[252:253]\n\t"
+      "v_mad_u64_u32 v[252:253], vcc, %[m10], %[p9], v[252:253]\n\tv_mad_u64_u32 v[252:253], vcc, %[m11], %[p8], v[252:253]\n\tv_mad_u64_u32 v[252:253], vcc, %[m12], %[p7], v[252:253]\n\tv_mad_u64_u32 v[252:253], vcc, %[m13], %[p6], v[252:253]\n\tv_and_b32_e32 %[t5], %[mask], v252\n\tv_lshrrev_b64 v[252:253], 28, v[252:253]\n\tv_mad_u64_u32 v[252:253], vcc, %[x7], %[y13], v[252:253]\n\tv_mad_u64_u32 v[252:253], vcc, %[x8], %[y12], v[252:253]\n\t"
+      "v_mad_u64_u32 v[252:253], vcc, %[x9], %[y11], v[252:253]\n\tv_mad_u64_u32 v[252:253], vcc, %[x10], %[y10], v[252:253]\n\tv_mad_u64_u32 v[252:253], vcc, %[x11], %[y9], v[252:253]\n\tv_mad_u64_u32 v[252:253], vcc, %[x12], %[y8], v[252:253]\n\tv_mad_u64_u32 v[252:253], vcc, %[x13], %[y7], v[252:253]\n\tv_mad_u64_u32 v[252:253], vcc, %[m7], %[p13], v[252:253]\n\tv_mad_u64_u32 v[252:253], vcc, %[m8], %[p12], v[252:253]\n\tv_mad_u64_u32 v[252:253], vcc, %[m9], %[p11], v[252:253]\n\t"
+      "v_mad_u64_u32 v[252:253], vcc, %[m10], %[p10], v[252:253]\n\tv_mad_u64_u32 v[252:253], vcc, %[m11], %[p9], v[252:253]\n\tv_mad_u64_u32 v[252:253], vcc, %[m12], %[p8], v[252:253]\n\tv_mad_u64_u32 v[252:253], vcc, %[m13], %[p7], v[252:253]\n\tv_and_b32_e32 %[t6], %[mask], v252\n\tv_lshrrev_b64 v[252:253], 28, v[252:253]\n\tv_mad_u64_u32 v[252:253], vcc, %[x8], %[y13], v[252:253]\n\tv_mad_u64_u32 v[252:253], vcc, %[x9], %[y12], v[252:253]\n\t"
+      "v_mad_u64_u32 v[252:253], vcc, %[x10], %[y11], v[252:253]\n\tv_mad_u64_u32 v[252:253], vcc, %[x11], %[y10], v[252:253]\n\tv_mad_u64_u32 v[252:253], vcc, %[x12], %[y9], v[252:253]\n\tv_mad_u64_u32 v[252:253], vcc, %[x13], %[y8], v[252:253]\n\tv_mad_u64_u32 v[252:253], vcc, %[m8], %[p13], v[252:253]\n\tv_mad_u64_u32 v[252:253], vcc, %[m9], %[p12], v[252:253]\n\tv_mad_u64_u32 v[252:253], vcc, %[m10], %[p11], v[252:253]\n\tv_mad_u64_u32 v[252:253], vcc, %[m11], %[p10], v[252:253]\n\t"
+      "v_mad_u64_u32 v[252:253], vcc, %[m12], %[p9], v[252:253]\n\tv_mad_u64_u32 v[252:253], vcc, %[m13], %[p8], v[252:253]\n\tv_and_b32_e32 %[t7], %[mask], v252\n\tv_lshrrev_b64 v[252:253], 28, v[252:253]\n\tv_mad_u64_u32 v[252:253], vcc, %[x9], %[y13], v[252:253]\n\tv_mad_u64_u32 v[252:253], vcc, %[x10], %[y12], v[252:253]\n\tv_mad_u64_u32 v[252:253], vcc, %[x11], %[y11], v[252:253]\n\tv_mad_u64_u32 v[252:253], vcc, %[x12], %[y10], v[252:253]\n\t"
+      "v_mad_u64_u32 v[252:253], vcc, %[x13], %[y9], v[252:253]\n\tv_mad_u64_u32 v[252:253], vcc, %[m9], %[p13], v[252:253]\n\tv_mad_u64_u32 v[252:253], vcc, %[m10], %[p12], v[252:253]\n\tv_mad_u64_u32 v[252:253], vcc, %[m11], %[p11], v[252:253]\n\tv_mad_u64_u32 v[252:253], vcc, %[m12], %[p10], v[252:253]\n\tv_mad_u64_u32 v[252:253], vcc, %[m13], %[p9], v[252:253]\n\tv_and_b32_e32 %[t8], %[mask], v252\n\tv_lshrrev_b64 v[252:253], 28, v[252:253]\n\t"
+      "v_mad_u64_u32 v[252:253], vcc, %[x10], %[y13], v[252:253]\n\tv_mad_u64_u32 v[252:253], vcc, %[x11], %[y12], v[252:253]\n\tv_mad_u64_u32 v[252:253], vcc, %[x12], %[y11], v[252:253]\n\tv_mad_u64_u32 v[252:253], vcc, %[x13], %[y10], v[252:253]\n\tv_mad_u64_u32 v[252:253], vcc, %[m10], %[p13], v[252:253]\n\tv_mad_u64_u32 v[252:253], vcc, %[m11], %[p12], v[252:253]\n\tv_mad_u64_u32 v[252:253], vcc, %[m12], %[p11], v[252:253]\n\tv_mad_u64_u32 v[252:253], vcc, %[m13], %[p10], v[252:253]\n\t"
+      "v_and_b32_e32 %[t9], %[mask], v252\n\tv_lshrrev_b64 v[252:253], 28, v[252:253]\n\tv_mad_u64_u32 v[252:253], vcc, %[x11], %[y13], v[252:253]\n\tv_mad_u64_u32 v[252:253], vcc, %[x12], %[y12], v[252:253]\n\tv_mad_u64_u32 v[252:253], vcc, %[x13], %[y11], v[252:253]\n\tv_mad_u64_u32 v[252:253], vcc, %[m11], %[p13], v[252:253]\n\tv_mad_u64_u32 v[252:253], vcc, %[m12], %[p12], v[252:253]\n\tv_mad_u64_u32 v[252:253], vcc, %[m13], %[p11], v[252:253]\n\t"
+      "v_and_b32_e32 %[t10], %[mask], v252\n\tv_lshrrev_b64 v[252:253], 28, v[252:253]\n\tv_mad_u64_u32 v[252:253], vcc, %[x12], %[y13], v[252:253]\n\tv_mad_u64_u32 v[252:253], vcc, %[x13], %[y12], v[252:253]\n\tv_mad_u64_u32 v[252:253], vcc, %[m12], %[p13], v[252:253]\n\tv_mad_u64_u32 v[252:253], vcc, %[m13], %[p12], v[252:253]\n\tv_and_b32_e32 %[t11], %[mask], v252\n\tv_lshrrev_b64 v[252:253], 28, v[252:253]\n\t"
+      "v_mad_u64_u32 v[252:253], vcc, %[x13], %[y13], v[252:253]\n\tv_mad_u64_u32 v[252:253], vcc, %[m13], %[p13], v[252:253]\n\tv_and_b32_e32 %[t12], %[mask], v252\n\tv_lshrrev_b64 v[252:253], 28, v[252:253]\n\tv_mov_b32 %[t13], v252\n\t"
+      : [m0] "=&v"(m[0]), [m1] "=&v"(m[1]), [m2] "=&v"(m[2]), [m3] "=&v"(m[3]), [m4] "=&v"(m[4]), [m5] "=&v"(m[5]), [m6] "=&v"(m[6]), [m7] "=&v"(m[7]), [m8] "=&v"(m[8]), [m9] "=&v"(m[9]), [m10] "=&v"(m[10]), [m11] "=&v"(m[11]), [m12] "=&v"(m[12]), [m13] "=&v"(m[13]), [t0] "=&v"(t[0]), [t1] "=&v"(t[1]), [t2] "=&v"(t[2]), [t3] "=&v"(t[3]), [t4] "=&v"(t[4]), [t5] "=&v"(t[5]), [t6] "=&v"(t[6]), [t7] "=&v"(t[7]), [t8] "=&v"(t[8]), [t9] "=&v"(t[9]), [t10] "=&v"(t[10]), [t11] "=&v"(t[11]), [t12] "=&v"(t[12]), [t13] "=&v"(t[13])
+      : [x0] "v"(x[0]), [x1] "v"(x[1]), [x2] "v"(x[2]), [x3] "v"(x[3]), [x4] "v"(x[4]), [x5] "v"(x[5]), [x6] "v"(x[6]), [x7] "v"(x[7]), [x8] "v"(x[8]), [x9] "v"(x[9]), [x10] "v"(x[10]), [x11] "v"(x[11]), [x12] "v"(x[12]), [x13] "v"(x[13]), [y0] "v"(y[0]), [y1] "v"(y[1]), [y2] "v"(y[2]), [y3] "v"(y[3]), [y4] "v"(y[4]), [y5] "v"(y[5]), [y6] "v"(y[6]), [y7] "v"(y[7]), [y8] "v"(y[8]), [y9] "v"(y[9]), [y10] "v"(y[10]), [y11] "v"(y[11]), [y12] "v"(y[12]), [y13] "v"(y[13]), [p0] "s"(P28[0]), [p1] "s"(P28[1]), [p2] "s"(P28[2]), [p3] "s"(P28[3]), [p4] "s"(P28[4]), [p5] "s"(P28[5]), [p6] "s"(P28[6]), [p7] "s"(P28[7]), [p8] "s"(P28[8]), [p9] "s"(P28[9]), [p10] "s"(P28[10]), [p11] "s"(P28[11]), [p12] "s"(P28[12]), [p13] "s"(P28[13]), [pinv] "s"(PINV28), [mask] "v"(M28)
+      : "vcc", "v252", "v253");
+  (void)m;
+  join28(r, t);
+}
 #if defined(OVH_FPMUL28_2ACC)
 __device__ __forceinline__ void fp_mul28_gfx950(uint32_t* r, const uint32_t* a, const uint32_t* b) {
   fp_mul28_gfx950_2acc(r, a, b);
diff --git a/consensus_overlord_amd/csrc/fpvm.hpp b/consensus_overlord_amd/csrc/fpvm.hpp
--- a/consensus_overlord_amd/csrc/fpvm.hpp
+++ b/consensus_overlord_amd/csrc/fpvm.hpp
@@ -211,6 +211,11 @@
   }
 }
 
+constexpr uint32_t W_WIDE = 1u << 25;
+#ifndef OVH_VM_RADIX
+#define OVH_VM_RADIX 0
+#endif
+
 constexpr uint32_t H_MUL = 1u << 22, H_MULNEG = 1u << 23, H_FLAG = 1u << 24, H_LIN = 1u << 25,
                    H_LINNEG = 1u << 26, H_ACC = 1u << 27, H_RARE = 1u << 28, H_SELB = 1u << 29,
                    H_LINNEG2 = 1u << 30, H_LINNEG3 = 1u << 31;
@@ -275,7 +280,7 @@
 VM_FN uint32_t sign_mask(uint32_t w, int bit) { return (uint32_t)((int32_t)(w << (31 - bit)) >> 31); }
 VM_FN int coef5(uint32_t w, int lo) { return ((int)(w << (27 - lo))) >> 27; }
 
-template <bool INV = true>
+template <bool INV = true, int RADIX = OVH_VM_RADIX>
 VM_FN void exec(const uint4 in, bool active, uint32_t* __restrict__ slots, const uint32_t* __restrict__ cst,
                 uint64_t scalar, const Out& out) {
   const uint32_t hdr = uniform(in.x);
@@ -301,13 +306,28 @@
     const bool is_mul = op == OP_MULS || op == OP_SGN0 || op == OP_LEX || op == OP_EQ;
     Fp x, y, m;
     pre_add2(x, A, B, y, C, D, sign_mask(in.w, 19) != 0, (hdr & H_MULNEG) != 0);
-    fp_mul(m, x, y);
+    static_assert(RADIX == 0 || RADIX == 384 || RADIX == 392, "Fp-VM radix: 2^384, 2^392 or per phase (0)");
+    const bool wide = RADIX == 392 || (RADIX == 0 && (uniform(in.w) & W_WIDE) != 0);
+    if constexpr (RADIX == 384) {
+      fp_mul(m, x, y);
+    } else if constexpr (RADIX == 392) {
+      fp_mul_wide(m, x, y);
+    } else {
+      if (wide) fp_mul_wide(m, x, y);
+      else fp_mul(m, x, y);
+    }
     if (hdr & H_FLAG) {
       const bool flag = is_mul && op != OP_MULS;
       uint32_t f = 0;
       if (op == OP_SGN0) f = m.v[0] & 1u;
       if (op == OP_LEX) f = limbs_gt(m.v, HALF_P) ? 1u : 0u;
       if (op == OP_EQ) f = fp_is_zero(m) ? 1u : 0u;
+      if (wide) {
+        uint32_t d = 0;
+#pragma unroll
+        for (int j = 0; j < 12; ++j) d |= m.v[j] ^ P_LIMBS[j];
+        if (d == 0) f = op == OP_EQ ? 1u : 0u;
+      }
 #pragma unroll
       for (int j = 0; j < 12; ++j) m.v[j] = flag ? (j == 0 ? f : 0u) : m.v[j];
     }
@@ -370,7 +390,7 @@
 #define OVH_VM_UNROLL 1
 #endif
 
-template <bool SIDE = false, bool INV = true, int UNROLL = OVH_VM_UNROLL>
+template <bool SIDE = false, bool INV = true, int UNROLL = OVH_VM_UNROLL, int RADIX = OVH_VM_RADIX>
 __device__ __forceinline__ void run(const uint4* __restrict__ code, uint32_t nphases, uint32_t W, uint32_t lane,
                                     bool active, uint32_t* __restrict__ slots, const uint32_t* __restrict__ cst,
                                     uint64_t scalar, const Out& out, uint64_t* __restrict__ trace = nullptr,
@@ -396,7 +416,7 @@
       }
       q2 = code[(size_t)(ph + QD) * W + lane];
       s2 = active ? side[(size_t)(ph + 2) * W + lane] : 0u;
-      exec<INV>(q, active, slots, cst, scalar, out);
+      exec<INV, RADIX>(q, active, slots, cst, scalar, out);
       side_spill(s, slots, scr);
       if (fill) {
         u32x4* d = reinterpret_cast<u32x4*>(slots + (sn & 0x7FF) * 12);
@@ -430,7 +450,7 @@
   __builtin_amdgcn_s_waitcnt(0x0F70);
   auto step = [&](const uint4& q, uint4& q2, const uint32_t ph) __attribute__((always_inline)) {
     q2 = code[(size_t)(ph + (UNROLL == 3 ? 2 : 1)) * W + lane];
-    exec<INV>(q, active, slots, cst, scalar, out);
+    exec<INV, RADIX>(q, active, slots, cst, scalar, out);
     if (trace && ph < nphases) {
       __asm__ volatile("s_waitcnt lgkmcnt(0)" ::: "memory");
       if (threadIdx.x == 0) trace[ph + 1] = wall_clock64();
diff --git a/consensus_overlord_amd/csrc/ovhip.hip b/consensus_overlord_amd/csrc/ovhip.hip
--- a/consensus_overlord_amd/csrc/ovhip.hip
+++ b/consensus_overlord_amd/csrc/ovhip.hip
@@ -17,7 +17,9 @@
 
 #include "../../include/ovhip.h"
 #include "bls/verify.hpp"
+#define OVH_VM_RADIX 384
 #include "fpvm.hpp"
+#include "ovhip/pool_remap.hpp"
 #include "keygen.hpp"
 #include "proof.hpp"
 #include "qc_round_groups.hpp"
@@ -31,8 +33,16 @@
 #include <vm_progs.inc>
 #endif
 static_assert(VM_KZERO == ovh::vm::KZERO && VM_KTAB == ovh::vm::KTAB, "fixed constants (tools/fpvm/gen.py)");
-#define VM_ASSERT_NO_INV(P) static_assert(!VM_##P##_HAS_INV, #P " has an inv op: it needs vm::run<SIDE, true>")
-#define VM_ASSERT_INV(P) static_assert(VM_##P##_HAS_INV, #P " has no inv op: bind it to vm::run<SIDE, false>")
+#define VM_ASSERT_RADIX(P, R) static_assert(VM_##P##_RADIX == (R), #P ": bind it to vm::run<.., RADIX> of its own radix")
+#define VM_ASSERT_NO_INV_ANY_RADIX(P) \
+  static_assert(!VM_##P##_HAS_INV, #P " has an inv op: it needs vm::run<SIDE, true>")
+#define VM_ASSERT_NO_INV(P)      \
+  VM_ASSERT_NO_INV_ANY_RADIX(P); \
+  VM_ASSERT_RADIX(P, OVH_VM_RADIX)
+#define VM_ASSERT_INV(P)                                                                             \
+  static_assert(VM_##P##_HAS_INV, #P " has no inv op: bind it to vm::run<SIDE, false>"); \
+  VM_ASSERT_RADIX(P, OVH_VM_RADIX)
+static_assert(VM_POOL_NCONST <= VM_NCONST, "the pool's constant table fits where the 384 prefix does (SLOT_BASE_W)");
 VM_ASSERT_NO_INV(MADD); VM_ASSERT_NO_INV(PADD); VM_ASSERT_NO_INV(G1PADD);
 VM_ASSERT_NO_INV(HDBL1); VM_ASSERT_NO_INV(HDBL2); VM_ASSERT_NO_INV(HDBL4); VM_ASSERT_NO_INV(HDBL8); VM_ASSERT_NO_INV(HDBL16);
 VM_ASSERT_NO_INV(VOTE1); VM_ASSERT_NO_INV(VOTE_T1); VM_ASSERT_NO_INV(VOTE1H); VM_ASSERT_NO_INV(VOTE_T1H);
@@ -1500,11 +1510,12 @@
   uint8_t* mg = nullptr;
   std::deque<HostBatch> hq;
   uint64_t hb_k = 0;
-  VmDev vm_vote{}, vm_vote_t{}, vm_fold{}, vm_final{}, vm_rs{}, vm_sigchk{}, vm_pkchk{}, vm_vote1{}, vm_vote_t1{},
+  VmDev vm_vote{}, vm_vote_t{}, vm_fold{}, vm_pfold{}, vm_final{}, vm_rs{}, vm_sigchk{}, vm_pkchk{}, vm_vote1{}, vm_vote_t1{},
       vm_signg0{}, vm_signg1{}, vm_pkgen{}, vm_vote1h{}, vm_vote_t1h{}, vm_qcpre{}, vm_qcmil{}, vm_votew{}, vm_votew_t{},
       vm_votewh{}, vm_votewh_t{}, vm_signg0h{}, vm_final1{}, vm_vsame{}, vm_vsame_t{}, vm_vsame8{}, vm_vsame8_t{},
       vm_h2g{}, vm_gfin{}, vm_g1grp{}, vm_pkdec{}, vm_gmil{}, vm_g1padd{}, vm_madd{}, vm_padd{}, vm_hdbl[5]{};
   uint32_t* vm_consts = nullptr;
+  uint32_t* vm_pool_consts = nullptr;
   std::vector<void*> vm_bufs;
   uint32_t* gslab[OVH_BATCH_SLOTS] = {};
   uint32_t gcap[OVH_BATCH_SLOTS] = {};
@@ -1628,6 +1639,7 @@
   uint32_t nphases, W, NW;
   const uint16_t* in; uint32_t nin; const uint16_t* out; uint32_t nout;
   const uint32_t* side;
+  bool pool = false;
 };
 #define VM_PROG(P, ...) \
   VmProg { VM_##P##_CODE, VM_##P##_NPHASES, VM_##P##_W, VM_##P##_NW, VM_##P##_IN, VM_##P##_NIN, VM_##P##_OUT, VM_##P##_NOUT, __VA_ARGS__ }
@@ -1644,9 +1656,10 @@
 #define VM_ROW(member, ...) \
   VmRow { [](ovh_ctx* c) { return &c->member; }, VM_PROG(__VA_ARGS__) }
 static const VmRow VM_TABLE[] = {
-    VM_ROW(vm_vote, VOTE, VM_VOTE_SIDE),
-    VM_ROW(vm_vote_t, VOTE_T, VM_VOTE_T_SIDE),
+    VM_ROW(vm_vote, VOTE, VM_VOTE_SIDE, true),
+    VM_ROW(vm_vote_t, VOTE_T, VM_VOTE_T_SIDE, true),
     VM_ROW(vm_fold, FOLD),
+    VM_ROW(vm_pfold, FOLD, nullptr, true),
     VM_ROW(vm_final, FINAL),
     VM_ROW(vm_rs, RS),
     VM_ROW(vm_sigchk, SIGCHK),
@@ -1691,7 +1704,13 @@
   void *dc = nullptr, *di = nullptr, *dout = nullptr;
   HIPCHK(hipMalloc(&dc, (words + pad) * 4));
   c->vm_bufs.push_back(dc);
-  HIPCHK(hipMemcpy(dc, p.code, words * 4, hipMemcpyHostToDevice));
+  if (p.pool) {
+    std::vector<uint32_t> pc(words);
+    if (pool::pool_remap_code(pc.data(), p.code, words, VM_POOL_CONST_IDX, VM_POOL_NCONST)) return OVH_ERR_DEVICE;
+    HIPCHK(hipMemcpy(dc, pc.data(), words * 4, hipMemcpyHostToDevice));
+  } else {
+    HIPCHK(hipMemcpy(dc, p.code, words * 4, hipMemcpyHostToDevice));
+  }
   HIPCHK(hipMemset((uint32_t*)dc + words, 0, pad * 4));
   HIPCHK(hipMalloc(&di, p.nin * 2 + 2));
   c->vm_bufs.push_back(di);
@@ -1733,8 +1752,14 @@
 }
 
 static int vm_init(ovh_ctx* c) {
-  HIPCHK(hipMalloc(&c->vm_consts, sizeof(VM_CONST_WORDS)));
+  HIPCHK(hipMalloc(&c->vm_consts, sizeof(VM_CONST_WORDS) + (size_t)VM_POOL_NCONST * 48));
   HIPCHK(hipMemcpy(c->vm_consts, VM_CONST_WORDS, sizeof(VM_CONST_WORDS), hipMemcpyHostToDevice));
+  {
+    std::vector<uint32_t> pw((size_t)VM_POOL_NCONST * 12);
+    pool::pool_const_words(pw.data(), VM_CONST_WORDS, VM_POOL_CONST_IDX, VM_POOL_NCONST);
+    c->vm_pool_consts = c->vm_consts + sizeof(VM_CONST_WORDS) / 4;
+    HIPCHK(hipMemcpy(c->vm_pool_consts, pw.data(), pw.size() * 4, hipMemcpyHostToDevice));
+  }
   for (const VmRow& r : VM_TABLE) CHK(vm_upload(c, *r.dev(c), r.prog));
   HIPCHK(hipFuncSetAttribute((const void*)k_vm_pool, hipFuncAttributeMaxDynamicSharedMemorySize, (int)LDS_POOL));
   HIPCHK(hipFuncSetAttribute((const void*)k_vm_signg, hipFuncAttributeMaxDynamicSharedMemorySize, (int)LDS_SIGNG));
@@ -2031,8 +2056,8 @@
   pa.pv_side = c->vm_vote.side;
   pa.pt_code = c->vm_vote_t.code;
   pa.pt_side = c->vm_vote_t.side;
-  pa.fold_code = c->vm_fold.code;
-  pa.cst = c->vm_consts;
+  pa.fold_code = c->vm_pfold.code;
+  pa.cst = c->vm_pool_consts;
   for (uint32_t par = 0; launch && par < (shard ? c->shard_streams : 2u); ++par) {
     if (shard && par != (uint32_t)(seq % c->shard_streams)) continue;
     if (shard) pa.only = seq + c->shard_span;
diff --git a/consensus_overlord_amd/csrc/ovhip/pool.hpp b/consensus_overlord_amd/csrc/ovhip/pool.hpp
--- a/consensus_overlord_amd/csrc/ovhip/pool.hpp
+++ b/consensus_overlord_amd/csrc/ovhip/pool.hpp
@@ -245,8 +245,10 @@
 #endif
 __device__ __forceinline__ void vote_quad(const PoolArgs& a, uint32_t slot_in, uint32_t quad_in, uint32_t* lds,
                                           const bool TABLE) {
-  VM_ASSERT_NO_INV(VOTE);
-  VM_ASSERT_NO_INV(VOTE_T);
+  VM_ASSERT_NO_INV_ANY_RADIX(VOTE);
+  VM_ASSERT_NO_INV_ANY_RADIX(VOTE_T);
+  VM_ASSERT_RADIX(VOTE, 392);
+  VM_ASSERT_RADIX(VOTE_T, 392);
   const uint32_t NSLOTS = TABLE ? VM_VOTE_T_NSLOTS : VM_VOTE_NSLOTS;
   const uint32_t STRIDE = TABLE ? VOTE_T_STRIDE_W : VOTE_STRIDE_W;
   const uint32_t NPH = TABLE ? VM_VOTE_T_NPHASES : VM_VOTE_NPHASES;
@@ -321,7 +323,7 @@
     }
     __syncthreads();
     const uint64_t scalar = vote_scalar(uni64(dget(&bd->seed)), uni64(dget(&bd->base)), i);
-    vm::run<true, false, OVH_POOL_UNROLL>(
+    vm::run<true, false, OVH_POOL_UNROLL, 392>(
         TABLE ? a.pt_code : a.pv_code, NPH, VM_VOTE_W, lane, active, slots, cst, scalar, vm::Out{s.p, s.cap, i},
         nullptr, TABLE ? a.pt_side : a.pv_side,
         a.scr + (size_t)blockIdx.x * VM_SLICES * VOTE_NSCR * 12 + slice * VOTE_NSCR * 12);
@@ -399,7 +401,7 @@
   extern __shared__ uint4 lds4[];
   if (a.skip_cu && ((simd_key() >> 2) & 0x7Fu) < a.skip_cu) return;
   uint32_t* lds = reinterpret_cast<uint32_t*>(lds4);
-  load_consts(lds, a.cst, VM_NCONST);
+  load_consts(lds, a.cst, VM_POOL_NCONST);
   const uint64_t t_in = __builtin_amdgcn_s_memrealtime();
   vote_stagger();
   uint32_t nquads = 0, why = 0;
diff --git a/consensus_overlord_amd/csrc/ovhip/pool_remap.hpp b/consensus_overlord_amd/csrc/ovhip/pool_remap.hpp
--- /dev/null
+++ b/consensus_overlord_amd/csrc/ovhip/pool_remap.hpp
@@ -0,0 +1,38 @@
+#pragma once
+#include <stdint.h>
+
+namespace ovh {
+namespace pool {
+
+constexpr uint32_t REF_CONST = 0x800;
+
+inline void pool_const_words(uint32_t* out, const uint32_t* table, const uint16_t* idx, uint32_t npool) {
+  for (uint32_t k = 0; k < npool; ++k)
+    for (uint32_t j = 0; j < 12; ++j) out[12 * k + j] = table[12 * (uint32_t)idx[k] + j];
+}
+
+inline uint32_t pool_remap_code(uint32_t* out, const uint32_t* code, size_t nwords, const uint16_t* idx,
+                                uint32_t npool) {
+  auto map = [&](uint32_t h, bool& bad) -> uint32_t {
+    if (!(h & REF_CONST)) return h;
+    const uint32_t c = h & (REF_CONST - 1);
+    for (uint32_t k = 0; k < npool; ++k)
+      if (idx[k] == c) return (h & ~(REF_CONST - 1)) | k;
+    bad = true;
+    return h;
+  };
+  for (size_t w = 0; w < nwords; ++w) {
+    const uint32_t v = code[w];
+    if ((w & 3) == 1 || (w & 3) == 2) {
+      bool bad = false;
+      out[w] = map(v & 0xFFFF, bad) | map(v >> 16, bad) << 16;
+      if (bad) return (uint32_t)w + 1;
+    } else {
+      out[w] = v;
+    }
+  }
+  return 0;
+}
+
+}
+}
```

Result: faster. 1.841 million verifications/s, median of 6 (+2.1%).
